# uta-smile/Adaptive-Graph-Convolutional-Network

Hardware: NVIDIA B200
Metric: sgc_ll_train_graphs_per_s (higher is better)
Workload: dtype f32

## Files before the change

adaptive-graph-convolutional-network_b200/_lib.py:

```python
import ctypes
import os

HERE = os.path.dirname(os.path.abspath(__file__))
LIB_PATH = os.path.join(HERE, "libagcn_sm100.so")

AGCN_OK = 0
VARIANT = {"SGC_LL": 0, "SGC_LL_Reslap": 1}
LAPLACIAN = {"reference_literal": 0, "paper": 1}
METRIC_GRAD = {"reference": 0, "full": 1}
ACT = {"linear": 0, "relu": 1}
LOSS = {"sigmoid_ce": 0, "softmax_ce": 1, "weighted_l2": 2}
ADJ_RULE = {"mean_distance": 0, "cutoff": 1}
NODE = {"sgcll": 0, "block_end": 1}
NOTIFY_FN = ctypes.CFUNCTYPE(None, ctypes.c_void_p, ctypes.c_int32, ctypes.c_void_p)
OUT_RES_L, OUT_RES_W, OUT_L_ALL, SAVE_FOR_BACKWARD = 1, 2, 4, 8


class AgcnError(RuntimeError):
    pass


class Desc(ctypes.Structure):
    _fields_ = [("F", ctypes.c_int32), ("Fo", ctypes.c_int32), ("K", ctypes.c_int32), ("variant", ctypes.c_int32),
                ("laplacian_mode", ctypes.c_int32), ("metric_grad", ctypes.c_int32), ("activation", ctypes.c_int32),
                ("flags", ctypes.c_uint32)]


class StackNode(ctypes.Structure):
    _fields_ = [("kind", ctypes.c_int32), ("desc", Desc), ("src", ctypes.c_int32)]


_P = ctypes.c_void_p
_SIGNATURES = {
    "agcn_version": (ctypes.c_int, []),
    "agcn_last_error": (ctypes.c_char_p, []),
    "agcn_launch_count": (ctypes.c_uint64, []),
    "agcn_plan_create": (ctypes.c_int, [_P, ctypes.c_int32, ctypes.c_int32, _P, ctypes.POINTER(_P)]),
    "agcn_plan_destroy": (ctypes.c_int, [_P]),
    "agcn_plan_total_nodes": (ctypes.c_int64, [_P]),
    "agcn_plan_total_lap": (ctypes.c_int64, [_P]),
    "agcn_plan_node_off_host": (_P, [_P]),
    "agcn_plan_lap_off_host": (_P, [_P]),
    "agcn_fused_tiles_host": (ctypes.c_int, [_P, ctypes.c_int32, _P, ctypes.c_int32, _P, ctypes.c_int32, _P, _P]),
    "agcn_fused_debug_set": (ctypes.c_int, [_P]),
    "agcn_fused_profile": (ctypes.c_int, [ctypes.c_int]),
    "agcn_fused_profile_read": (ctypes.c_int, [ctypes.POINTER(ctypes.c_float), ctypes.POINTER(ctypes.c_int)]),
    "agcn_profile_enable": (ctypes.c_int, [ctypes.c_int]),
    "agcn_profile_read": (ctypes.c_int, [ctypes.c_char_p, ctypes.c_size_t, ctypes.POINTER(ctypes.c_size_t)]),
    "agcn_profile_timeline": (ctypes.c_int, [ctypes.c_char_p, ctypes.c_size_t, ctypes.POINTER(ctypes.c_size_t)]),
    "agcn_probe_fp32_fma": (ctypes.c_int, [_P, ctypes.c_int32, _P]),
    "agcn_pack_nodes": (ctypes.c_int, [_P, _P, _P, ctypes.c_int32, _P]),
    "agcn_unpack_nodes": (ctypes.c_int, [_P, _P, _P, ctypes.c_int32, _P]),
    "agcn_pack_lap": (ctypes.c_int, [_P, _P, _P, _P]),
    "agcn_capture_begin": (ctypes.c_int, [_P]),
    "agcn_capture_end_launch": (ctypes.c_int, [_P, ctypes.POINTER(ctypes.c_void_p), ctypes.POINTER(ctypes.c_int32)]),
    "agcn_capture_abort": (ctypes.c_int, [_P]),
    "agcn_step_graph_destroy": (ctypes.c_int, [_P]),
    "agcn_unpack_lap": (ctypes.c_int, [_P, _P, _P, _P]),
    "agcn_debug_grouped_product": (ctypes.c_int, [_P, _P, _P, _P, ctypes.c_int32, ctypes.c_int32, ctypes.c_int32,
                                                  ctypes.c_float, ctypes.c_int32, _P]),
    "agcn_debug_grouped_timeline": (ctypes.c_int, [_P]),
    "agcn_pack_lap_csr": (ctypes.c_int, [_P, _P, _P, _P, _P, _P]),
    "agcn_point_laplacian_workspace_bytes": (ctypes.c_int, [_P, ctypes.POINTER(ctypes.c_size_t)]),
    "agcn_point_laplacian": (ctypes.c_int, [_P, _P, ctypes.c_int32, ctypes.c_int32, ctypes.c_float, _P, _P,
                                            ctypes.c_size_t, _P]),
    "agcn_graph_pool": (ctypes.c_int, [_P, _P, _P, _P, _P, ctypes.c_int32, _P]),
    "agcn_graph_pool_backward": (ctypes.c_int, [_P, _P, _P, _P, ctypes.c_int32, _P]),
    "agcn_sgcll_workspace_bytes": (ctypes.c_int, [ctypes.POINTER(Desc), _P, ctypes.POINTER(ctypes.c_size_t),
                                                  ctypes.POINTER(ctypes.c_size_t)]),
    "agcn_sgcll_forward": (ctypes.c_int, [ctypes.POINTER(Desc), _P] + [_P] * 14 + [ctypes.c_size_t, _P]),
    "agcn_sgcll_backward": (ctypes.c_int, [ctypes.POINTER(Desc), _P] + [_P] * 19 + [ctypes.c_size_t, _P]),
    "agcn_gemm_tn_scratch_bytes": (ctypes.c_size_t, [ctypes.c_int32] * 4),
    "agcn_gemm_tn": (ctypes.c_int, [_P, _P, _P, _P, ctypes.c_int32, ctypes.c_int32, ctypes.c_int32, ctypes.c_int32,
                                    _P, ctypes.c_int32, _P]),
    "agcn_node_gemm_scratch_bytes": (ctypes.c_size_t, [ctypes.c_int32, ctypes.c_int32]),
    "agcn_node_gemm": (ctypes.c_int, [_P, ctypes.c_int32, _P, ctypes.c_int32, ctypes.c_int32, _P, ctypes.c_int32,
                                      ctypes.c_int32, ctypes.c_int32, ctypes.c_int32, _P, _P, ctypes.c_int32,
                                      ctypes.c_int32, _P, _P]),
    "agcn_dropout": (ctypes.c_int, [_P, _P, ctypes.c_int64, ctypes.c_float, ctypes.c_uint64, _P]),
    "agcn_expand_labels": (ctypes.c_int, [_P, _P, ctypes.c_int32, ctypes.c_int32, _P, _P, _P]),
    "agcn_head_workspace_bytes": (ctypes.c_int, [_P, ctypes.c_int32, ctypes.c_int32, ctypes.c_int32,
                                                  ctypes.POINTER(ctypes.c_size_t)]),
    "agcn_head_loss_grad": (ctypes.c_int, [_P] * 8 + [ctypes.c_float, ctypes.c_int32, ctypes.c_int32, ctypes.c_int32] +
                            [_P] * 7 + [ctypes.c_size_t, _P]),
    "agcn_head_loss_grad_ex": (ctypes.c_int, [_P] * 8 + [ctypes.c_float, ctypes.c_int32, ctypes.c_int32, ctypes.c_int32,
                                                     ctypes.c_int32] + [_P] * 7 + [ctypes.c_size_t, _P]),
    "agcn_head_predict_workspace_bytes": (ctypes.c_int, [_P, ctypes.c_int32, ctypes.c_int32, ctypes.c_int32,
                                                          ctypes.POINTER(ctypes.c_size_t)]),
    "agcn_head_predict": (ctypes.c_int, [_P] * 8 + [ctypes.c_float, ctypes.c_int32, ctypes.c_int32, ctypes.c_int32,
                                                ctypes.c_int32] + [_P] * 3 + [ctypes.c_size_t, _P]),
    "agcn_stack_create": (ctypes.c_int, [_P, ctypes.c_int32, ctypes.c_int32, ctypes.c_int32, ctypes.c_int32, _P,
                                         ctypes.POINTER(_P)]),
    "agcn_stack_create_nodes": (ctypes.c_int, [_P, ctypes.c_int32, ctypes.c_int32, ctypes.c_int32, ctypes.c_int32, _P,
                                               ctypes.POINTER(_P)]),
    "agcn_stack_destroy": (ctypes.c_int, [_P]),
    "agcn_stack_workspace_bytes": (ctypes.c_int, [_P, _P, ctypes.POINTER(ctypes.c_size_t)]),
    "agcn_stack_loss_grad": (ctypes.c_int, [_P] * 6 + [ctypes.c_float] + [_P] * 4 + [ctypes.c_size_t, _P, _P, _P]),
    "agcn_stack_predict_workspace_bytes": (ctypes.c_int, [_P, _P, ctypes.POINTER(ctypes.c_size_t)]),
    "agcn_stack_predict": (ctypes.c_int, [_P] * 6 + [ctypes.c_float] + [_P] * 4 + [ctypes.c_size_t, _P]),
    "agcn_adam_step": (ctypes.c_int, [_P] * 5 + [ctypes.c_int64] + [ctypes.c_float] * 4 + [_P]),
    "agcn_sgcll_host_scratch_bytes": (ctypes.c_int, [ctypes.POINTER(Desc), _P, ctypes.POINTER(ctypes.c_size_t)]),
    "agcn_sgcll_forward_host": (ctypes.c_int, [ctypes.POINTER(Desc), _P] + [_P] * 8 + [ctypes.c_size_t, _P]),
}
EXPORTED_SYMBOLS = tuple(_SIGNATURES)

_lib = None


def lib():
    global _lib
    if _lib is None:
        if not os.path.exists(LIB_PATH):
            raise AgcnError("libagcn_sm100.so is missing: run `python %s` (no CPU fallback exists)"
                            % os.path.join(HERE, "build_ext.py"))
        handle = ctypes.CDLL(LIB_PATH)
        for name, (res, args) in _SIGNATURES.items():
            fn = getattr(handle, name)
            fn.restype, fn.argtypes = res, args
        _lib = handle
    return _lib


def check(rc):
    if rc != AGCN_OK:
        raise AgcnError("libagcn_sm100 error %d: %s" % (rc, lib().agcn_last_error().decode()))


def launch_count():
    return int(lib().agcn_launch_count())


def profile_enable(on):
    check(lib().agcn_profile_enable(1 if on else 0))


def profile_timeline():
    buf = ctypes.create_string_buffer(1 << 18)
    check(lib().agcn_profile_timeline(buf, len(buf), None))
    out = []
    for line in buf.value.decode().splitlines():
        name, t0, t1 = line.split("\t")
        out.append((name, float(t0), float(t1)))
    return out


def profile_read():
    buf = ctypes.create_string_buffer(1 << 16)
    check(lib().agcn_profile_read(buf, len(buf), None))
    out = {}
    for line in buf.value.decode().splitlines():
        name, n, ms = line.split("\t")
        out[name] = (int(n), float(ms))
    return out
```

adaptive-graph-convolutional-network_b200/csrc/agcn_capi.cu:

```cuda
#include <algorithm>

#include "agcn_internal.cuh"

using namespace agcn;

namespace {

inline size_t align256(size_t x) { return (x + 255) & ~(size_t)255; }

int node_gemm_tn(const GemmTNArgs& t, cudaStream_t st) {
  if (tc_gemm_tn_supported(t)) return tc_gemm_tn(t, st);
  return gemm_tn(t, st);
}

int node_gemm(const GemmArgs& g, float* tc_scratch, cudaStream_t st, bool presplit = false) {
  if (tc_gemm_supported(g)) {
    if (!presplit) {
      int rc = tc_gemm_split_b(g, tc_scratch, st);
      if (rc) return rc;
    }
    return tc_gemm(g, tc_scratch, st);
  }
  return gemm_rows(g, st);
}
// ... 65 lines not shown
  return s;
}

inline int64_t dl_stride(const agcn_plan* p) { return (p->LL + 63) & ~(int64_t)63; }
inline int dl_parts(const agcn_sgcll_desc* d, const agcn_plan* p) {
  if (d->K < 2) return 1;
  int parts = std::min(8, (d->F + 31) / 32);
  while (parts > 1 && (int64_t)parts * dl_stride(p) * 4 > ((int64_t)1 << 30)) --parts;
  return std::max(1, parts);
}

struct Work {
  float *XW, *dYp, *G, *V, *tn_part, *act_part, *dL, *dXW, *dalpha_part, *dbeta_part, *tcY, *tcM, *big, *ftY;
  size_t bytes;
};

Work carve_work(const agcn_sgcll_desc* d, const agcn_plan* p, void* base) {
  const Modes m = modes_of(d);
  Carver c(base);
  Work w{};
  w.XW = c.take((size_t)p->R * d->F);
  w.dYp = c.take((size_t)p->R * d->Fo);
  w.G = c.take((size_t)d->K * p->R * d->F);
  w.V = c.take((size_t)(d->K > 1 ? d->K - 1 : 0) * p->R * d->Fo);
  size_t tn = gemm_tn_partial_floats((int)p->R, d->F, d->Fo, d->K);
  if (m.full) tn = std::max(tn, gemm_tn_partial_floats((int)p->R, d->F, d->F, 1));
  {
    GemmTNArgs t;
    t.M = (int)p->R; t.Kd = d->F; t.N = d->Fo; t.S = d->K;
    tn = std::max(tn, tc_gemm_tn_partial_floats(t));
    t.N = d->F; t.S = 1;
    tn = std::max(tn, tc_gemm_tn_partial_floats(t));
  }
  w.tn_part = c.take(tn);
  w.act_part = c.take(act_bwd_partial_floats(p->R, d->Fo));
  w.dL = m.need_dL ? c.take((size_t)dl_parts(d, p) * dl_stride(p)) : nullptr;
  w.dXW = m.full ? c.take((size_t)p->R * d->F) : nullptr;
  w.dalpha_part = c.take((size_t)p->B);
  w.dbeta_part = c.take((size_t)p->B);
  w.tcY = c.take(tc_gemm_scratch_floats(d->Fo, d->F, d->K, 1));
  w.tcM = c.take(tc_gemm_scratch_floats(d->F, d->F, 1, 1));
  w.big = c.take(big_work_floats(p, m.full));
  w.ftY = c.take(fused_w_floats(d->Fo, d->F, d->K));
  w.bytes = c.off;
  return w;
}

int check_desc(const agcn_sgcll_desc* d, const agcn_plan* p) {
  AGCN_REQUIRE(d && p, "null desc or plan");
  AGCN_REQUIRE(d->F >= 1 && d->Fo >= 1 && d->K >= 1, "F, Fo, K must be >= 1");
  AGCN_REQUIRE(d->variant == AGCN_VARIANT_SGC_LL || d->variant == AGCN_VARIANT_SGC_LL_RESLAP, "unknown variant");
  AGCN_REQUIRE(d->laplacian_mode == AGCN_LAP_REFERENCE_LITERAL || d->laplacian_mode == AGCN_LAP_PAPER,
               "unknown laplacian_mode");
  AGCN_REQUIRE(d->metric_grad == AGCN_METRIC_GRAD_REFERENCE || d->metric_grad == AGCN_METRIC_GRAD_FULL,
               "unknown metric_grad");
  AGCN_REQUIRE(d->activation == AGCN_ACT_LINEAR || d->activation == AGCN_ACT_RELU, "unknown activation");
  AGCN_REQUIRE(p->R < (1ll << 31) / std::max(d->F, d->Fo), "batch too large for 32-bit row indexing");
  return AGCN_OK;
}

}

namespace {

int padded_features(const agcn_sgcll_desc* d, const agcn_plan* p) {
  const int F = d->F;
  if (F < 33 || F % 32 == 0) return F;
  if (!literal_shortcut(d->variant, d->laplacian_mode)) return F;
  if (d->flags & (AGCN_OUT_RES_L | AGCN_OUT_RES_W | AGCN_OUT_L_ALL)) return F;
  const int Fp = (F + 31) & ~31;
  if (!fused_fwd_supported(p, Fp, d->Fo, d->K)) return F;
  return Fp;
}

struct PadSaved {
  float *Xp, *Wp;
  void* inner;
  size_t bytes;
};
PadSaved carve_pad_saved(const agcn_sgcll_desc* d2, const agcn_plan* p, void* base) {
  Carver c(base);
  PadSaved s{};
  s.Xp = c.take((size_t)p->R * d2->F);
  s.Wp = c.take((size_t)d2->F * d2->K * d2->Fo);
  s.inner = base ? reinterpret_cast<char*>(base) + c.off : nullptr;
  s.bytes = c.off + carve_saved(d2, p, nullptr).bytes + 256;
  return s;
}
struct PadWork {
  float *dXp, *dWp, *dMp;
  void* inner;
  size_t inner_bytes, bytes;
};
PadWork carve_pad_work(const agcn_sgcll_desc* d2, const agcn_plan* p, void* base) {
  Carver c(base);
  PadWork w{};
  w.dXp = c.take((size_t)p->R * d2->F);
  w.dWp = c.take((size_t)d2->F * d2->K * d2->Fo);
  w.dMp = c.take((size_t)d2->F * d2->F);
  w.inner = base ? reinterpret_cast<char*>(base) + c.off : nullptr;
  w.inner_bytes = carve_work(d2, p, nullptr).bytes + 256;
  w.bytes = c.off + w.inner_bytes;
  return w;
}

__global__ void pad_cols_kernel(const float* __restrict__ src, int Fs, float* __restrict__ dst, int Fd, long long rows) {
  const long long total = rows * Fd;
  for (long long e = (long long)blockIdx.x * blockDim.x + threadIdx.x; e < total; e += (long long)gridDim.x * blockDim.x) {
    const long long r = e / Fd;
    const int c = (int)(e - r * Fd);
    dst[e] = c < Fs ? src[r * Fs + c] : 0.f;
  }
}
__global__ void unpad_cols_kernel(const float* __restrict__ src, int Fs, float* __restrict__ dst, int Fd, long long rows) {
  const long long total = rows * Fd;
  for (long long e = (long long)blockIdx.x * blockDim.x + threadIdx.x; e < total; e += (long long)gridDim.x * blockDim.x) {
    const long long r = e / Fd;
    const int c = (int)(e - r * Fd);
    dst[e] = src[r * Fs + c];
  }
}
__global__ void copy_then_zero_kernel(const float* __restrict__ src, float* __restrict__ dst, long long n_copy, long long n_total) {
  for (long long e = (long long)blockIdx.x * blockDim.x + threadIdx.x; e < n_total; e += (long long)gridDim.x * blockDim.x)
    dst[e] = e < n_copy ? src[e] : 0.f;
}
inline unsigned grid_for(long long total) { return (unsigned)std::max<long long>(1, std::min<long long>((total + 255) / 256, 1184)); }

int forward_impl(const agcn_sgcll_desc* desc, const agcn_plan* plan, const float* d_X, const float* d_Lint,
                 const float* d_Lprev, const float* d_M_L, const float* d_weight, const float* d_bias,
                 const float* d_alpha, const float* d_beta, float* d_Y, float* d_resL, float* d_resW, float* d_Lall,
                 void* d_saved, void* d_work, size_t work_bytes, void* stream);
int backward_impl(const agcn_sgcll_desc* desc, const agcn_plan* plan, const float* d_X, const float* d_Lint,
                  const float* d_Lprev, const float* d_M_L, const float* d_weight, const float* d_alpha,
                  const float* d_beta, const float* d_Y, const float* d_dY, const float* d_dLall_in, const void* d_saved,
                  float* d_dX, float* d_dM_L, float* d_dweight, float* d_dbias, float* d_dalpha, float* d_dbeta,
                  float* d_dLprev, void* d_work, size_t work_bytes, void* stream);

}

extern "C" {

int agcn_sgcll_workspace_bytes(const agcn_sgcll_desc* desc, const agcn_plan* plan, size_t* saved_bytes,
                               size_t* work_bytes) {
  AGCN_REQUIRE(desc && plan, "null desc or plan");
  const int Fp = padded_features(desc, plan);
  if (Fp != desc->F) {
    agcn_sgcll_desc d2 = *desc;
    d2.F = Fp;
    if (saved_bytes) *saved_bytes = carve_pad_saved(&d2, plan, nullptr).bytes + 256;
    if (work_bytes) *work_bytes = carve_pad_work(&d2, plan, nullptr).bytes + 256;
    return AGCN_OK;
  }
  if (saved_bytes) *saved_bytes = carve_saved(desc, plan, nullptr).bytes + 256;
  if (work_bytes) *work_bytes = carve_work(desc, plan, nullptr).bytes + 256;
  return AGCN_OK;
}

int agcn_sgcll_forward(const agcn_sgcll_desc* desc, const agcn_plan* plan, const float* d_X, const float* d_Lint,
                       const float* d_Lprev, const float* d_M_L, const float* d_weight, const float* d_bias,
                       const float* d_alpha, const float* d_beta, float* d_Y, float* d_resL, float* d_resW,
                       float* d_Lall, void* d_saved, void* d_work, size_t work_bytes, void* stream) {
  int rc = check_desc(desc, plan);
  if (rc) return rc;
  const int Fp = padded_features(desc, plan);
  if (Fp == desc->F)
    return forward_impl(desc, plan, d_X, d_Lint, d_Lprev, d_M_L, d_weight, d_bias, d_alpha, d_beta, d_Y, d_resL, d_resW,
                        d_Lall, d_saved, d_work, work_bytes, stream);
  AGCN_REQUIRE(d_X && d_weight && d_saved && d_work, "forward: null pointer");
  agcn_sgcll_desc d2 = *desc;
  d2.F = Fp;
  PadSaved ps = carve_pad_saved(&d2, plan, d_saved);
  PadWork pw = carve_pad_work(&d2, plan, d_work);
  if (pw.bytes > work_bytes) {
    set_error("forward: workspace too small");
    return AGCN_ERR_WORKSPACE;
  }
  cudaStream_t st = (cudaStream_t)stream;
  if ((rc = plan_use(plan, st))) return rc;
  pad_cols_kernel<<<grid_for((long long)plan->R * Fp), 256, 0, st>>>(d_X, desc->F, ps.Xp, Fp, plan->R);
  AGCN_LAUNCH_CHECK();
  {
    const long long n_copy = (long long)desc->F * desc->K * desc->Fo, n_total = (long long)Fp * desc->K * desc->Fo;
    copy_then_zero_kernel<<<grid_for(n_total), 256, 0, st>>>(d_weight, ps.Wp, n_copy, n_total);
    AGCN_LAUNCH_CHECK();
  }
  return forward_impl(&d2, plan, ps.Xp, d_Lint, d_Lprev, d_M_L, ps.Wp, d_bias, d_alpha, d_beta, d_Y, d_resL, d_resW, d_Lall,
                      ps.inner, pw.inner, pw.inner_bytes, stream);
}

int agcn_sgcll_backward(const agcn_sgcll_desc* desc, const agcn_plan* plan, const float* d_X, const float* d_Lint,
                        const float* d_Lprev, const float* d_M_L, const float* d_weight, const float* d_alpha,
                        const float* d_beta, const float* d_Y, const float* d_dY, const float* d_dLall_in,
                        const void* d_saved, float* d_dX, float* d_dM_L, float* d_dweight, float* d_dbias,
                        float* d_dalpha, float* d_dbeta, float* d_dLprev, void* d_work, size_t work_bytes,
                        void* stream) {
  int rc = check_desc(desc, plan);
  if (rc) return rc;
  const int Fp = padded_features(desc, plan);
  if (Fp == desc->F)
    return backward_impl(desc, plan, d_X, d_Lint, d_Lprev, d_M_L, d_weight, d_alpha, d_beta, d_Y, d_dY, d_dLall_in, d_saved,
                         d_dX, d_dM_L, d_dweight, d_dbias, d_dalpha, d_dbeta, d_dLprev, d_work, work_bytes, stream);
  AGCN_REQUIRE(d_saved && d_work && d_dM_L && d_dweight, "backward: null pointer");
  agcn_sgcll_desc d2 = *desc;
  d2.F = Fp;
  PadSaved ps = carve_pad_saved(&d2, plan, const_cast<void*>(d_saved));
  PadWork pw = carve_pad_work(&d2, plan, d_work);
  if (pw.bytes > work_bytes) {
    set_error("backward: workspace too small");
    return AGCN_ERR_WORKSPACE;
  }
  cudaStream_t st = (cudaStream_t)stream;
  rc = backward_impl(&d2, plan, ps.Xp, d_Lint, d_Lprev, d_M_L, ps.Wp, d_alpha, d_beta, d_Y, d_dY, d_dLall_in, ps.inner,
                     d_dX ? pw.dXp : nullptr, pw.dMp, pw.dWp, d_dbias, d_dalpha, d_dbeta, d_dLprev, pw.inner, pw.inner_bytes,
                     stream);
  if (rc) return rc;
  {
    const long long n = (long long)desc->F * desc->K * desc->Fo;
    copy_then_zero_kernel<<<grid_for(n), 256, 0, st>>>(pw.dWp, d_dweight, n, n);
    AGCN_LAUNCH_CHECK();
  }
  if ((rc = zero_async(d_dM_L, (size_t)desc->F * desc->F, st))) return rc;
  if (d_dX) {
    unpad_cols_kernel<<<grid_for((long long)plan->R * desc->F), 256, 0, st>>>(pw.dXp, Fp, d_dX, desc->F, plan->R);
    AGCN_LAUNCH_CHECK();
  }
  return AGCN_OK;
}

}

namespace {

int forward_impl(const agcn_sgcll_desc* desc, const agcn_plan* plan, const float* d_X, const float* d_Lint,
                       const float* d_Lprev, const float* d_M_L, const float* d_weight, const float* d_bias,
                       const float* d_alpha, const float* d_beta, float* d_Y, float* d_resL, float* d_resW,
                       float* d_Lall, void* d_saved, void* d_work, size_t work_bytes, void* stream) {
  int rc = check_desc(desc, plan);
  if (rc) return rc;
  AGCN_REQUIRE(d_X && d_Lint && d_M_L && d_weight && d_bias && d_alpha && d_Y && d_saved && d_work,
               "forward: null pointer");
  const Modes m = modes_of(desc);
  AGCN_REQUIRE(!m.reslap || d_beta, "forward: beta required for SGC_LL_Reslap");
  AGCN_REQUIRE(!(desc->flags & AGCN_OUT_RES_L) || d_resL, "forward: d_resL missing");
  AGCN_REQUIRE(!(desc->flags & AGCN_OUT_RES_W) || d_resW, "forward: d_resW missing");
  AGCN_REQUIRE(!(desc->flags & AGCN_OUT_L_ALL) || d_Lall, "forward: d_Lall missing");
  cudaStream_t st = (cudaStream_t)stream;
  if ((rc = plan_use(plan, st))) return rc;
  Saved sv = carve_saved(desc, plan, d_saved);
  Work wk = carve_work(desc, plan, d_work);
  if (wk.bytes > work_bytes) {
    set_error("forward: workspace too small");
    return AGCN_ERR_WORKSPACE;
  }
  const int F = desc->F, Fo = desc->Fo, K = desc->K;
  const int R = (int)plan->R;
  const bool want_resL = desc->flags & AGCN_OUT_RES_L, want_resW = desc->flags & AGCN_OUT_RES_W;
  const bool want_Lall = desc->flags & AGCN_OUT_L_ALL;
  const bool need_W = m.paper || want_resW;
  const bool need_build = !m.shortcut || want_resL || want_resW || want_Lall;
  float* XW = m.full ? sv.XW : wk.XW;

  const bool fuse_f = fused_fwd_supported(plan, F, Fo, K);
  const bool fuse_b = (desc->flags & AGCN_SAVE_FOR_BACKWARD) && !m.need_dL && fused_bwd_supported(plan, F, Fo, K);
  GemmArgs gy = y_gemm_args(desc, R, d_X, sv.T, d_weight, d_bias, d_Y);
  const bool y_tc = !fuse_f && tc_gemm_supported(gy);
  GemmArgs gg = g_gemm_args(desc, R, d_Y , d_weight, wk.G);
  const bool g_tc = !fuse_b && (desc->flags & AGCN_SAVE_FOR_BACKWARD) && tc_gemm_supported(gg);
  if (y_tc || g_tc || fuse_f || fuse_b) {
    AGCN_CUDA(cudaEventRecord(plan->ev_side_fork, st));
    AGCN_CUDA(cudaStreamWaitEvent(plan->side, plan->ev_side_fork, 0));
    if (fuse_f && (rc = fused_fwd_prep(d_weight, F, Fo, K, wk.ftY, plan->side))) return rc;
    if (y_tc && (rc = tc_gemm_split_b(gy, wk.tcY, plan->side))) return rc;
    if (fuse_b && (rc = fused_bwd_prep(d_weight, F, Fo, K, sv.ftG, plan->side))) return rc;
    if (g_tc && (rc = tc_gemm_split_b(gg, sv.tcG, plan->side))) return rc;
    AGCN_CUDA(cudaEventRecord(plan->ev_side_join, plan->side));
  }
  if (need_W) {
    GemmArgs g;
    g.M = R; g.N = F; g.Kd = F;
    g.A0 = d_X; g.lda0 = F;
    g.B = d_M_L; g.ldb = F;
    g.C = XW; g.ldc = F;
    if ((rc = node_gemm(g, wk.tcM, st))) return rc;
  }
  GraphArgs ga;
  ga.plan = plan; ga.F = F; ga.K = K;
  ga.variant = desc->variant; ga.lap_mode = desc->laplacian_mode; ga.metric_full = m.full;
  ga.X = d_X; ga.XW = XW; ga.Lint = d_Lint; ga.Lprev = m.reslap ? d_Lprev : nullptr;
  ga.alpha = d_alpha; ga.beta = d_beta;
  ga.T = sv.T;
  if (need_build) {
    ga.Lall = m.shortcut ? nullptr : sv.Lall;
    ga.Lall_out = want_Lall ? d_Lall : nullptr;
    ga.resL = want_resL ? d_resL : nullptr;
    ga.resW = want_resW ? d_resW : nullptr;
    ga.dist = sv.dist; ga.dis = sv.dis; ga.stats = sv.stats;
    ga.big_work = wk.big;
    if ((rc = graph_build_laplacian(ga, need_W, st))) return rc;
  }
  ga.Lall = m.shortcut ? nullptr : sv.Lall;
  if (fuse_f) {
    const float* Lf = m.shortcut ? d_Lint : sv.Lall;
    const int ident = m.shortcut ? 1 : 0;
    const bool other = cheb_tiles_has_mid(plan) || plan->large_tiles > 0;
    if (other) {
      AGCN_CUDA(cudaEventRecord(plan->ev_big_fork, st));
      AGCN_CUDA(cudaStreamWaitEvent(plan->big, plan->ev_big_fork, 0));
    }
    if ((rc = cheb_tiles_forward(plan, d_X, Lf, ident, F, K, sv.T, st, plan->big))) return rc;
    if (plan->large_tiles > 0 && (rc = graph_chebyshev_fwd(ga, plan->big, AGCN_SMALL_MAX))) return rc;
    if (other) {
      AGCN_CUDA(cudaEventRecord(plan->ev_big_join, plan->big));
      AGCN_CUDA(cudaStreamWaitEvent(st, plan->ev_big_join, 0));
    }
    AGCN_CUDA(cudaStreamWaitEvent(st, plan->ev_side_join, 0));
    return pre_forward(plan, -1, 0, d_X, sv.T, wk.ftY, d_bias, desc->activation, F, Fo, K, d_Y, st);
  }
  if ((rc = graph_chebyshev_fwd(ga, st))) return rc;
  if (y_tc || g_tc || fuse_b) AGCN_CUDA(cudaStreamWaitEvent(st, plan->ev_side_join, 0));
  if ((rc = node_gemm(gy, wk.tcY, st, true))) return rc;
  return AGCN_OK;
}

int backward_impl(const agcn_sgcll_desc* desc, const agcn_plan* plan, const float* d_X, const float* d_Lint,
                  const float* d_Lprev, const float* d_M_L, const float* d_weight, const float* d_alpha,
                  const float* d_beta, const float* d_Y, const float* d_dY, const float* d_dLall_in, const void* d_saved,
                  float* d_dX, float* d_dM_L, float* d_dweight, float* d_dbias, float* d_dalpha, float* d_dbeta,
                  float* d_dLprev, void* d_work, size_t work_bytes, void* stream) {
  int rc = check_desc(desc, plan);
  if (rc) return rc;
  AGCN_REQUIRE(d_X && d_Lint && d_M_L && d_weight && d_alpha && d_Y && d_dY && d_saved && d_work,
               "backward: null input pointer");
  AGCN_REQUIRE(d_dM_L && d_dweight && d_dbias && d_dalpha, "backward: null output pointer");
  const Modes m = modes_of(desc);
  AGCN_REQUIRE(!m.reslap || (d_beta && d_dbeta), "backward: beta / dbeta required for SGC_LL_Reslap");
  cudaStream_t st = (cudaStream_t)stream;
  if ((rc = plan_use(plan, st))) return rc;
  Saved sv = carve_saved(desc, plan, const_cast<void*>(d_saved));
  Work wk = carve_work(desc, plan, d_work);
  if (wk.bytes > work_bytes) {
    set_error("backward: workspace too small");
    return AGCN_ERR_WORKSPACE;
  }
  const int F = desc->F, Fo = desc->Fo, K = desc->K;
  const int R = (int)plan->R;
  const bool has_prev = m.reslap && d_Lprev;

  const bool fuse_b = (desc->flags & AGCN_SAVE_FOR_BACKWARD) && !m.need_dL && d_dX != nullptr &&
                      fused_bwd_supported(plan, F, Fo, K);
  const bool vfirst = fuse_b && plan->large_tiles == 0;
  const bool need_G = !fuse_b && (d_dX != nullptr || (m.need_dL && K >= 2));
  const float* dYp = (desc->activation == AGCN_ACT_RELU) ? wk.dYp : d_dY;
  const bool act_on_side = !vfirst && (fuse_b || (!need_G && !m.need_dL));
  if (!act_on_side && (rc = act_bwd_partials(d_dY, d_Y, wk.dYp, wk.act_part, R, Fo, desc->activation, st))) return rc;
  AGCN_CUDA(cudaEventRecord(plan->ev_side_fork, st));
  AGCN_CUDA(cudaStreamWaitEvent(plan->side, plan->ev_side_fork, 0));
  if (act_on_side && (rc = act_bwd_partials(d_dY, d_Y, wk.dYp, wk.act_part, R, Fo, desc->activation, plan->side)))
    return rc;
  if ((rc = act_bwd_reduce(wk.act_part, d_dbias, R, Fo, plan->side))) return rc;
  float* dXbuf = d_dX ? d_dX : wk.G;
  AGCN_REQUIRE(d_dX || !m.full, "backward: d_dX is required with metric_grad = full");
  if (need_G) {
    GemmArgs g = g_gemm_args(desc, R, dYp, d_weight, (K == 1) ? d_dX : wk.G);
    GemmArgs probe = g_gemm_args(desc, R, d_Y, d_weight, wk.G);
    const bool presplit = (desc->flags & AGCN_SAVE_FOR_BACKWARD) && tc_gemm_supported(probe);
    if ((rc = node_gemm(g, sv.tcG, st, presplit))) return rc;
  }
  GraphArgs ga;
  ga.plan = plan; ga.F = F; ga.K = K;
  ga.variant = desc->variant; ga.lap_mode = desc->laplacian_mode; ga.metric_full = m.full;
  ga.X = d_X; ga.XW = sv.XW; ga.Lint = d_Lint; ga.Lprev = has_prev ? d_Lprev : nullptr;
  ga.alpha = d_alpha; ga.beta = d_beta;
  ga.T = sv.T; ga.Lall = m.shortcut ? nullptr : sv.Lall;
  ga.dist = sv.dist; ga.dis = sv.dis; ga.stats = sv.stats;
  ga.G = wk.G; ga.dLall_in = d_dLall_in; ga.dX = dXbuf; ga.dL = wk.dL;
  ga.dl_parts = (m.need_dL && K >= 2) ? dl_parts(desc, plan) : 1;
  ga.dl_stride = dl_stride(plan);
  ga.dLprev = has_prev ? d_dLprev : nullptr;
  ga.dXW = wk.dXW; ga.dalpha_part = wk.dalpha_part; ga.dbeta_part = m.reslap ? wk.dbeta_part : nullptr;
  ga.big_work = wk.big;
  {
    GemmTNArgs t;
    t.M = R; t.Kd = F; t.N = Fo; t.S = K;
    t.A0 = d_X; t.lda0 = F;
    t.A1 = sv.T; t.lda1 = F; t.sliceA1 = (int64_t)R * F;
    t.D = dYp; t.ldd = Fo;
    t.out = d_dweight; t.partial = wk.tn_part;
    if ((rc = node_gemm_tn(t, plan->side))) return rc;
  }
  AGCN_CUDA(cudaEventRecord(plan->ev_side_join, plan->side));
  if (vfirst) {
    const float* Lf = m.shortcut ? d_Lint : sv.Lall;
    const int ident = m.shortcut ? 1 : 0;
    const bool other = cheb_tiles_has_mid(plan);
    if (other) {
      AGCN_CUDA(cudaEventRecord(plan->ev_big_fork, st));
      AGCN_CUDA(cudaStreamWaitEvent(plan->big, plan->ev_big_fork, 0));
    }
    if ((rc = cheb_tiles_forward(plan, dYp, Lf, ident, Fo, K, wk.V, st, plan->big, 1))) return rc;
    if (other) {
      AGCN_CUDA(cudaEventRecord(plan->ev_big_join, plan->big));
      AGCN_CUDA(cudaStreamWaitEvent(st, plan->ev_big_join, 0));
    }
    if ((rc = pre_forward(plan, -1, 0, dYp, wk.V, sv.ftG, nullptr, AGCN_ACT_LINEAR, Fo, F, K, d_dX, st))) return rc;
  } else if (fuse_b) {
    const float* Lf = m.shortcut ? d_Lint : sv.Lall;
    const int ident = m.shortcut ? 1 : 0;
    if ((rc = pre_backward(plan, -1, 0, d_dY, desc->activation == AGCN_ACT_RELU ? d_Y : nullptr, sv.ftG, F, Fo, K, wk.G, st)))
      return rc;
    const bool other = cheb_tiles_has_mid(plan) || plan->large_tiles > 0;
    if (other) {
      AGCN_CUDA(cudaEventRecord(plan->ev_big_fork, st));
      AGCN_CUDA(cudaStreamWaitEvent(plan->big, plan->ev_big_fork, 0));
    }
    if ((rc = cheb_tiles_backward(plan, wk.G, Lf, ident, F, K, d_dX, st, plan->big))) return rc;
    if (plan->large_tiles > 0 && (rc = graph_recurrence_bwd(ga, false, plan->big, AGCN_SMALL_MAX))) return rc;
    if (other) {
      AGCN_CUDA(cudaEventRecord(plan->ev_big_join, plan->big));
      AGCN_CUDA(cudaStreamWaitEvent(st, plan->ev_big_join, 0));
    }
  } else if (K >= 2) {
    if (need_G && (rc = graph_recurrence_bwd(ga, m.need_dL, st))) return rc;
  } else if (m.need_dL) {
    if (d_dLall_in)
      AGCN_CUDA(cudaMemcpyAsync(wk.dL, d_dLall_in, (size_t)plan->LL * sizeof(float), cudaMemcpyDeviceToDevice, st));
    else
      AGCN_CUDA(cudaMemsetAsync(wk.dL, 0, (size_t)plan->LL * sizeof(float), st));
  }
  AGCN_CUDA(cudaStreamWaitEvent(st, plan->ev_side_join, 0));
  if (m.need_dL) {
    if ((rc = graph_laplacian_bwd(ga, st))) return rc;
    if ((rc = reduce_scalar_parts(wk.dalpha_part, plan->B, d_dalpha, st))) return rc;
    if (m.reslap) {
      if ((rc = reduce_scalar_parts(wk.dbeta_part, plan->B, d_dbeta, st))) return rc;
    }
  } else {
    if ((rc = zero_async(d_dalpha, 1, st))) return rc;
  }
  if (m.full) {
    GemmTNArgs t;
    t.M = R; t.Kd = F; t.N = F; t.S = 1;
    t.A0 = d_X; t.lda0 = F;
    t.D = wk.dXW; t.ldd = F;
    t.out = d_dM_L; t.partial = wk.tn_part;
    if ((rc = node_gemm_tn(t, st))) return rc;
    GemmArgs g;
    g.M = R; g.N = F; g.Kd = F;
    g.A0 = wk.dXW; g.lda0 = F;
    g.B = d_M_L; g.ldb = F; g.transB = 1;
    g.C = d_dX; g.ldc = F; g.accumulate = 1;
    if ((rc = node_gemm(g, wk.tcM, st))) return rc;
  } else {
    if ((rc = zero_async(d_dM_L, (size_t)F * F, st))) return rc;
  }
  return AGCN_OK;
}

}

extern "C" {

size_t agcn_gemm_tn_scratch_bytes(int32_t M, int32_t Kd, int32_t N, int32_t S) {
  GemmTNArgs t;
  t.M = M; t.Kd = Kd; t.N = N; t.S = S;
  return 4 * std::max(gemm_tn_partial_floats(M, Kd, N, S), tc_gemm_tn_partial_floats(t)) + 256;
}

int agcn_gemm_tn(const float* d_A0, const float* d_A1, const float* d_D, float* d_out, int32_t M, int32_t Kd,
                 int32_t N, int32_t S, void* d_scratch, int32_t use_tensor_cores, void* stream) {
  AGCN_REQUIRE(d_A0 && d_D && d_out && d_scratch && M >= 1 && Kd >= 1 && N >= 1 && S >= 1, "gemm_tn: bad arguments");
  GemmTNArgs t;
  t.M = M; t.Kd = Kd; t.N = N; t.S = S;
  t.A0 = d_A0; t.lda0 = Kd;
  t.A1 = d_A1; t.lda1 = Kd; t.sliceA1 = (int64_t)M * Kd;
  t.D = d_D; t.ldd = N;
  t.out = d_out; t.partial = reinterpret_cast<float*>(d_scratch);
  if (use_tensor_cores) {
    if (!tc_gemm_tn_supported(t)) {
      set_error("gemm_tn: shape not supported by the tensor-core kernel");
      return AGCN_ERR_INVALID;
    }
    return tc_gemm_tn(t, (cudaStream_t)stream);
  }
  return gemm_tn(t, (cudaStream_t)stream);
}

size_t agcn_node_gemm_scratch_bytes(int32_t N, int32_t Kd) { return 4 * tc_gemm_scratch_floats(N, Kd, 1, 1) + 256; }

int agcn_node_gemm(const float* d_A, int32_t lda, const float* d_B, int32_t ldb, int32_t transB, float* d_C, int32_t ldc,
                   int32_t M, int32_t N, int32_t Kd, const float* d_bias, const float* d_scale, int32_t accumulate,
                   int32_t activation, void* d_scratch, void* stream) {
  AGCN_REQUIRE(d_A && d_B && d_C && d_scratch && M >= 1 && N >= 1 && Kd >= 1, "node_gemm: bad arguments");
  AGCN_REQUIRE(activation == AGCN_ACT_LINEAR || activation == AGCN_ACT_RELU, "node_gemm: unknown activation");
  GemmArgs g;
  g.M = M; g.N = N; g.Kd = Kd;
  g.A0 = d_A; g.lda0 = lda;
  g.B = d_B; g.ldb = ldb; g.transB = transB;
  g.C = d_C; g.ldc = ldc;
  g.bias = d_bias; g.scale = d_scale; g.accumulate = accumulate; g.act = activation;
  return node_gemm(g, reinterpret_cast<float*>(d_scratch), (cudaStream_t)stream);
}

int agcn_fused_profile(int enable) {
  fused_profile_enable(enable);
  return AGCN_OK;
}
int agcn_fused_profile_read(float* ms_sum, int* launches) { return fused_profile_read(ms_sum, launches); }

int agcn_fused_debug_set(void* d_buf) {
  fused_debug_set(d_buf);
  return AGCN_OK;
}

int agcn_sgcll_host_scratch_bytes(const agcn_sgcll_desc* desc, const agcn_plan* plan, size_t* bytes) {
  AGCN_REQUIRE(desc && plan && bytes, "null pointer");
  size_t saved = 0, work = 0;
  agcn_sgcll_workspace_bytes(desc, plan, &saved, &work);
  const size_t B = plan->B, N = plan->Nmax;
  size_t total = 0;
  total += align256(B * N * desc->F * 4) + align256(B * N * N * 4) + align256(B * N * desc->Fo * 4);
  total += align256((size_t)plan->R * desc->F * 4) + align256((size_t)plan->LL * 4) +
           align256((size_t)plan->R * desc->Fo * 4);
  total += align256(saved) + align256(work);
  *bytes = total;
  return AGCN_OK;
}

int agcn_sgcll_forward_host(const agcn_sgcll_desc* desc, const agcn_plan* plan, const float* h_X_padded,
                            const float* h_L_padded, const float* d_M_L, const float* d_weight, const float* d_bias,
                            const float* d_alpha, float* h_Y_padded, void* d_scratch, size_t scratch_bytes,
                            void* stream) {
  int rc = check_desc(desc, plan);
  if (rc) return rc;
  AGCN_REQUIRE(h_X_padded && h_L_padded && h_Y_padded && d_scratch, "forward_host: null pointer");
  AGCN_REQUIRE(desc->variant == AGCN_VARIANT_SGC_LL, "forward_host: SGC_LL only");
  AGCN_REQUIRE((desc->flags & (AGCN_OUT_RES_L | AGCN_OUT_RES_W | AGCN_OUT_L_ALL)) == 0,
               "forward_host: optional outputs are not supported");
  size_t need = 0, saved = 0, work = 0;
  agcn_sgcll_host_scratch_bytes(desc, plan, &need);
  if (need > scratch_bytes) {
    set_error("forward_host: scratch too small");
    return AGCN_ERR_WORKSPACE;
  }
  agcn_sgcll_workspace_bytes(desc, plan, &saved, &work);
  cudaStream_t st = (cudaStream_t)stream;
  const size_t B = plan->B, N = plan->Nmax;
  char* base = reinterpret_cast<char*>(d_scratch);
  size_t off = 0;
  auto take = [&](size_t bytes) { char* r = base + off; off += align256(bytes); return r; };
  float* dXpad = (float*)take(B * N * desc->F * 4);
  float* dLpad = (float*)take(B * N * N * 4);
  float* dYpad = (float*)take(B * N * desc->Fo * 4);
  float* dX = (float*)take((size_t)plan->R * desc->F * 4);
  float* dL = (float*)take((size_t)plan->LL * 4);
  float* dY = (float*)take((size_t)plan->R * desc->Fo * 4);
  void* dsaved = take(saved);
  void* dwork = take(work);
  auto device_view = [](const float* h) -> const float* {
    cudaPointerAttributes at;
    if (cudaPointerGetAttributes(&at, h) != cudaSuccess) {
      (void)cudaGetLastError();
      return nullptr;
    }
    if ((at.type == cudaMemoryTypeHost || at.type == cudaMemoryTypeManaged) && at.devicePointer)
      return reinterpret_cast<const float*>(at.devicePointer);
    return nullptr;
  };
  const float* xsrc = device_view(h_X_padded);
  const float* lsrc = device_view(h_L_padded);
  if (!xsrc) {
    AGCN_CUDA(cudaMemcpyAsync(dXpad, h_X_padded, B * N * desc->F * 4, cudaMemcpyHostToDevice, st));
    xsrc = dXpad;
  }
  if (!lsrc) {
    AGCN_CUDA(cudaMemcpyAsync(dLpad, h_L_padded, B * N * N * 4, cudaMemcpyHostToDevice, st));
    lsrc = dLpad;
  }
  if ((rc = agcn_pack_nodes(plan, xsrc, dX, desc->F, st))) return rc;
  if ((rc = agcn_pack_lap(plan, lsrc, dL, st))) return rc;
  if ((rc = agcn_sgcll_forward(desc, plan, dX, dL, nullptr, d_M_L, d_weight, d_bias, d_alpha, nullptr, dY, nullptr,
                               nullptr, nullptr, dsaved, dwork, work, st)))
    return rc;
  if ((rc = agcn_unpack_nodes(plan, dY, dYpad, desc->Fo, st))) return rc;
  AGCN_CUDA(cudaMemcpyAsync(h_Y_padded, dYpad, B * N * desc->Fo * 4, cudaMemcpyDeviceToHost, st));
  AGCN_CUDA(cudaStreamSynchronize(st));
  return AGCN_OK;
}

}
```

adaptive-graph-convolutional-network_b200/csrc/agcn_cheb_tile.cu:

```cuda
#include <algorithm>
#include <mutex>

#include "agcn_internal.cuh"

namespace agcn {
namespace ct {

constexpr int CH = 32;
constexpr int CPITCH = 144;

__device__ __forceinline__ uint32_t smem_u32(const void* p) { return (uint32_t)__cvta_generic_to_shared(p); }
__device__ __forceinline__ float4 lds128(uint32_t a) {
  float4 v;
  asm volatile("ld.shared.v4.f32 {%0,%1,%2,%3}, [%4];\n" : "=f"(v.x), "=f"(v.y), "=f"(v.z), "=f"(v.w) : "r"(a) : "memory");
  return v;
}
__device__ __forceinline__ float lds32(uint32_t a) {
  float v;
  asm volatile("ld.shared.f32 %0, [%1];\n" : "=f"(v) : "r"(a) : "memory");
  return v;
}
__device__ __forceinline__ void sts128(uint32_t a, float4 v) {
  asm volatile("st.shared.v4.f32 [%0], {%1,%2,%3,%4};\n" ::"r"(a), "f"(v.x), "f"(v.y), "f"(v.z), "f"(v.w) : "memory");
}
__device__ __forceinline__ void sts32(uint32_t a, float v) {
  asm volatile("st.shared.f32 [%0], %1;\n" ::"r"(a), "f"(v) : "memory");
}
__device__ __forceinline__ void cp_async4(uint32_t sdst, const float* gsrc) {
  asm volatile("cp.async.ca.shared.global [%0], [%1], 4;\n" ::"r"(sdst), "l"(gsrc) : "memory");
}
__device__ __forceinline__ void cp_async16(uint32_t sdst, const float* gsrc) {
  asm volatile("cp.async.cg.shared.global [%0], [%1], 16;\n" ::"r"(sdst), "l"(gsrc) : "memory");
}
__device__ __forceinline__ void cp_async_commit() { asm volatile("cp.async.commit_group;\n" ::: "memory"); }
__device__ __forceinline__ void cp_async_wait_all() { asm volatile("cp.async.wait_group 0;\n" ::: "memory"); }

struct CtArgs {
  const int4* tile_graphs;
  const int32_t* tile_gstart;
  const int32_t* order;
  const int32_t* n_nodes;
  const int32_t* node_off;
  const int64_t* lap_off;
  int order_start;
  int chunks;
  int cpc;
  int groups;
  int rows;
  int lfloats;
  const float* L;
  int add_identity;
  int transL;
  int F, K;
  const float* X;
  float* T;
  long long tslice;
  const float* G;
  long long gslice;
  float* dX;
  unsigned long long* dbg;
};

#define CT_STAMP(slot)                                                                  \
  do {                                                                                  \
    if (p.dbg && threadIdx.x == 0) {                                                    \
      unsigned long long t__;                                                           \
      asm volatile("mov.u64 %0, %%globaltimer;\n" : "=l"(t__));                         \
      p.dbg[(long long)blockIdx.x * 128 + (slot)] = t__;                                \
    }                                                                                   \
  } while (0)

struct Row {
  int grow;
  int n;
  int r0;
  int lbase;
  int i;
  int pitch;
};

__device__ __forceinline__ void copy_matrix(const float* __restrict__ src, uint32_t dst, int n, int pitch) {
  const int warp = threadIdx.x >> 5, lane = threadIdx.x & 31, nw = blockDim.x >> 5;
  for (int i = warp; i < n; i += nw) {
    const float* srow = src + (long long)i * n;
    const uint32_t drow = dst + 4 * (i * pitch);
    for (int j = lane; j < n; j += 32) cp_async4(drow + 4 * j, srow + j);
  }
}

template <bool TILE>
__device__ __forceinline__ Row prologue(const CtArgs& p, int tile, int r, uint32_t s_glist, uint32_t sL) {
  Row t;
  t.grow = -1; t.n = 0; t.r0 = 0; t.lbase = 0; t.i = 0; t.pitch = 1;
  const int tid = threadIdx.x, nthreads = blockDim.x;
  if (TILE) {
    if (tid < 32) {
      int gs = 0, ge = 0;
      if (tid == 0) {
        gs = __ldg(p.tile_gstart + tile);
        ge = __ldg(p.tile_gstart + tile + 1);
      }
      gs = __shfl_sync(0xffffffffu, gs, 0);
      ge = __shfl_sync(0xffffffffu, ge, 0);
      const int ng2 = 2 * (ge - gs);
      for (int e = tid; e < ng2; e += 32) {
        const int4 v = __ldg(p.tile_graphs + 2 * gs + e);
        asm volatile("st.shared.v4.s32 [%0], {%1,%2,%3,%4};\n" ::"r"(s_glist + 16 * e), "r"(v.x), "r"(v.y), "r"(v.z), "r"(v.w) : "memory");
      }
      if (tid == 0) asm volatile("st.shared.s32 [%0], %1;\n" ::"r"(s_glist + 128 * 32), "r"(ge - gs) : "memory");
    }
    __syncthreads();
    int ng;
    asm volatile("ld.shared.s32 %0, [%1];\n" : "=r"(ng) : "r"(s_glist + 128 * 32) : "memory");
    for (int e = 0; e < ng; ++e) {
      int gx, gy, gz, gw, noff, lo, hi, pad;
      asm volatile("ld.shared.v4.s32 {%0,%1,%2,%3}, [%4];\n" : "=r"(gx), "=r"(gy), "=r"(gz), "=r"(gw) : "r"(s_glist + 32 * e) : "memory");
      asm volatile("ld.shared.v4.s32 {%0,%1,%2,%3}, [%4];\n" : "=r"(noff), "=r"(lo), "=r"(hi), "=r"(pad) : "r"(s_glist + 32 * e + 16) : "memory");
      if (r >= gy && r < gy + gz) {
        t.grow = noff + (r - gy);
        t.n = gz; t.r0 = gy; t.lbase = gw; t.i = r - gy; t.pitch = gz | 1;
      }
      const long long loff = (long long)(((unsigned long long)(unsigned)hi << 32) | (unsigned)lo);
      copy_matrix(p.L + loff, sL + 4 * gw, gz, gz | 1);
    }
  } else {
    const int g = p.order[p.order_start + tile];
    const int n = p.n_nodes[g], pitch = n | 1;
    if (r < n) {
      t.grow = p.node_off[g] + r;
      t.n = n; t.i = r; t.pitch = pitch;
    }
    copy_matrix(p.L + p.lap_off[g], sL, n, pitch);
  }
  cp_async_commit();
  return t;
}

template <int MW>
struct Mask {
  uint32_t w[MW];
};

template <int MW>
__device__ __forceinline__ Mask<MW> nonzero_mask(uint32_t laddr, int lstride_bytes, int n) {
  Mask<MW> m;
#pragma unroll
  for (int k = 0; k < MW; ++k) {
    uint32_t bits = 0;
    const int j0 = 32 * k;
    if (j0 < n) {
      const int cnt = min(32, n - j0);
      uint32_t a = laddr + (uint32_t)(j0 * lstride_bytes);
      int j = 0;
      for (; j + 8 <= cnt; j += 8) {
        uint32_t b8 = 0;
#pragma unroll
        for (int u = 0; u < 8; ++u) b8 |= (lds32(a + (uint32_t)(u * lstride_bytes)) != 0.f) ? (1u << u) : 0u;
        bits |= b8 << j;
        a += 8 * lstride_bytes;
      }
      for (; j < cnt; ++j) {
        bits |= (lds32(a) != 0.f) ? (1u << j) : 0u;
        a += lstride_bytes;
      }
    }
    m.w[k] = bits;
  }
  return m;
}
template <int MW>
__device__ __forceinline__ bool prefer_masked(const Mask<MW>& m, int n) {
  int nnz = 0;
#pragma unroll
  for (int k = 0; k < MW; ++k) nnz += __popc(m.w[k]);
  const unsigned dense_cost = __reduce_max_sync(0xffffffffu, (unsigned)(n * 3));
  const unsigned masked_cost = __reduce_max_sync(0xffffffffu, (unsigned)(nnz * 4));
  return masked_cost < dense_cost;
}

__device__ __forceinline__ void fma_row(float a, const float4 b[4], float acc[16]) {
#pragma unroll
  for (int g = 0; g < 4; ++g) {
    acc[4 * g] = fmaf(a, b[g].x, acc[4 * g]);
    acc[4 * g + 1] = fmaf(a, b[g].y, acc[4 * g + 1]);
    acc[4 * g + 2] = fmaf(a, b[g].z, acc[4 * g + 2]);
    acc[4 * g + 3] = fmaf(a, b[g].w, acc[4 * g + 3]);
  }
}
__device__ __forceinline__ void lap_times_rows(uint32_t laddr, int lstride_bytes, uint32_t src, int r0, int n, int h,
                                               float acc[16]) {
  uint32_t ta = src + (uint32_t)(r0 * CPITCH + h * 64);
  uint32_t la = laddr;
  int j = 0;
  for (; j < n; ++j) {
    const float a = lds32(la);
    float4 b[4];
#pragma unroll
    for (int g = 0; g < 4; ++g) b[g] = lds128(ta + 16 * g);
    fma_row(a, b, acc);
    la += lstride_bytes;
    ta += CPITCH;
  }
}
template <int MW>
__device__ __forceinline__ void lap_times_rows_masked(uint32_t laddr, int lstride_bytes, uint32_t src, int r0,
                                                      const Mask<MW>& m, int h, float acc[16]) {
#pragma unroll
  for (int k = 0; k < MW; ++k) {
    uint32_t bits = m.w[k];
    const uint32_t tbase = src + (uint32_t)((r0 + 32 * k) * CPITCH + h * 64);
    const uint32_t lbase = laddr + (uint32_t)(32 * k * lstride_bytes);
    while (bits) {
      const int j = __ffs((int)bits) - 1;
      bits &= bits - 1;
      const float a = lds32(lbase + (uint32_t)(j * lstride_bytes));
      float4 b[4];
#pragma unroll
      for (int g = 0; g < 4; ++g) b[g] = lds128(tbase + (uint32_t)(j * CPITCH + 16 * g));
      fma_row(a, b, acc);
    }
  }
}

__device__ __forceinline__ uint32_t seg_addr(uint32_t buf, int row, int h) { return buf + (uint32_t)(row * CPITCH + h * 64); }
__device__ __forceinline__ void read_seg(uint32_t buf, int row, int h, float v[16]) {
#pragma unroll
  for (int g = 0; g < 4; ++g) {
    const float4 x = lds128(seg_addr(buf, row, h) + 16 * g);
    v[4 * g] = x.x; v[4 * g + 1] = x.y; v[4 * g + 2] = x.z; v[4 * g + 3] = x.w;
  }
}
__device__ __forceinline__ void write_seg(uint32_t buf, int row, int h, const float v[16]) {
#pragma unroll
  for (int g = 0; g < 4; ++g)
    sts128(seg_addr(buf, row, h) + 16 * g, make_float4(v[4 * g], v[4 * g + 1], v[4 * g + 2], v[4 * g + 3]));
}
__device__ __forceinline__ void load_seg(const float* __restrict__ M, int F, int grow, int col0, bool vec, float v[16]) {
  if (grow < 0) {
#pragma unroll
    for (int u = 0; u < 16; ++u) v[u] = 0.f;
    return;
  }
  const float* src = M + (long long)grow * F + col0;
  if (vec) {
#pragma unroll
    for (int g = 0; g < 4; ++g) {
      float4 x = make_float4(0.f, 0.f, 0.f, 0.f);
      if (col0 + 4 * g < F) x = __ldg(reinterpret_cast<const float4*>(src) + g);
      v[4 * g] = x.x; v[4 * g + 1] = x.y; v[4 * g + 2] = x.z; v[4 * g + 3] = x.w;
    }
  } else {
#pragma unroll
    for (int u = 0; u < 16; ++u) v[u] = (col0 + u < F) ? __ldg(src + u) : 0.f;
  }
}
__device__ __forceinline__ void store_seg(float* __restrict__ M, int F, int grow, int col0, bool vec, const float v[16]) {
  if (grow < 0) return;
  float* dst = M + (long long)grow * F + col0;
  if (vec) {
#pragma unroll
    for (int g = 0; g < 4; ++g)
      if (col0 + 4 * g < F)
        reinterpret_cast<float4*>(dst)[g] = make_float4(v[4 * g], v[4 * g + 1], v[4 * g + 2], v[4 * g + 3]);
  } else {
#pragma unroll
    for (int u = 0; u < 16; ++u)
      if (col0 + u < F) dst[u] = v[u];
  }
}

template <bool TILE, int MW>
__global__ void __launch_bounds__(TILE ? 256 : 320, TILE ? 3 : 1) cheb_tile_fwd_kernel(CtArgs p) {
  extern __shared__ __align__(16) uint8_t smem[];
  const uint32_t sbase = smem_u32(smem);
  const int rows = p.rows;
  const uint32_t buf0 = sbase, buf1 = sbase + (uint32_t)(rows * CPITCH), sL = buf1 + (uint32_t)(rows * CPITCH),
                 s_glist = sL + 4u * (uint32_t)p.lfloats;
  const int tile = blockIdx.x / p.groups, grp = blockIdx.x - tile * p.groups;
  const int warp = threadIdx.x >> 5, lane = threadIdx.x & 31, wpr = rows >> 5;
  const int h = warp / wpr, r = (warp - h * wpr) * 32 + lane;
  const int F = p.F, K = p.K;
  CT_STAMP(100);
  const Row me = prologue<TILE>(p, tile, r, s_glist, sL);
  CT_STAMP(101);
  const bool vec = ((F & 3) == 0) && ((reinterpret_cast<uintptr_t>(p.X) & 15) == 0) &&
                   ((reinterpret_cast<uintptr_t>(p.T) & 15) == 0) && ((p.tslice & 3) == 0);
  const uint32_t lrow = p.transL ? sL + 4 * (me.lbase + me.i) : sL + 4 * (me.lbase + me.i * me.pitch);
  const int lstep = p.transL ? 4 * me.pitch : 4;
  Mask<MW> mask;
  bool masked = false;
  const int c_beg = grp * p.cpc, c_end = min(p.chunks, c_beg + p.cpc);
  for (int c = c_beg; c < c_end; ++c) {
    const int col0 = c * CH + 16 * h;
    {
      const uint32_t d = seg_addr(buf0, r, h);
      const float* src = p.X + (long long)(me.grow < 0 ? 0 : me.grow) * F + col0;
      if (vec) {
#pragma unroll
        for (int g = 0; g < 4; ++g) {
          if (me.grow >= 0 && col0 + 4 * g < F)
            cp_async16(d + 16 * g, src + 4 * g);
          else
            sts128(d + 16 * g, make_float4(0.f, 0.f, 0.f, 0.f));
        }
      } else {
#pragma unroll
        for (int u = 0; u < 16; ++u) {
          if (me.grow >= 0 && col0 + u < F)
            cp_async4(d + 4 * u, src + u);
          else
            sts32(d + 4 * u, 0.f);
        }
      }
      cp_async_commit();
    }
    if (c == c_beg) CT_STAMP(102);
    cp_async_wait_all();
    __syncthreads();
    if (c == c_beg) {
      CT_STAMP(103);
      mask = nonzero_mask<MW>(lrow, lstep, me.n);
      masked = prefer_masked<MW>(mask, me.n);
      CT_STAMP(104);
    }
    float tm1[16], tm2[16];
    read_seg(buf0, r, h, tm1);
#pragma unroll
    for (int u = 0; u < 16; ++u) tm2[u] = 0.f;
    uint32_t src = buf0, dst = buf1;
    for (int s = 1; s < K; ++s) {
      float t[16];
#pragma unroll
      for (int u = 0; u < 16; ++u) t[u] = p.add_identity ? tm1[u] : 0.f;
      if (masked)
        lap_times_rows_masked<MW>(lrow, lstep, src, me.r0, mask, h, t);
      else
        lap_times_rows(lrow, lstep, src, me.r0, me.n, h, t);
      if (s >= 2) {
#pragma unroll
        for (int u = 0; u < 16; ++u) t[u] = 2.f * t[u] - tm2[u];
      }
      store_seg(p.T + (long long)(s - 1) * p.tslice, F, me.grow, col0, vec, t);
      if (s + 1 < K) {
        write_seg(dst, r, h, t);
        __syncthreads();
        const uint32_t tmp = src; src = dst; dst = tmp;
      }
#pragma unroll
      for (int u = 0; u < 16; ++u) { tm2[u] = tm1[u]; tm1[u] = t[u]; }
      if (c == c_beg) CT_STAMP(104 + s);
    }
    if (c + 1 < c_end) __syncthreads();
  }
}

template <bool TILE, int MW>
__global__ void __launch_bounds__(TILE ? 256 : 320, TILE ? 3 : 1) cheb_tile_bwd_kernel(CtArgs p) {
  extern __shared__ __align__(16) uint8_t smem[];
  const uint32_t sbase = smem_u32(smem);
  const int rows = p.rows;
  const uint32_t buf0 = sbase, buf1 = sbase + (uint32_t)(rows * CPITCH), sL = buf1 + (uint32_t)(rows * CPITCH),
                 s_glist = sL + 4u * (uint32_t)p.lfloats;
  const int tile = blockIdx.x / p.groups, grp = blockIdx.x - tile * p.groups;
  const int warp = threadIdx.x >> 5, lane = threadIdx.x & 31, wpr = rows >> 5;
  const int h = warp / wpr, r = (warp - h * wpr) * 32 + lane;
  const int F = p.F, K = p.K;
  const Row me = prologue<TILE>(p, tile, r, s_glist, sL);
  const bool vec = ((F & 3) == 0) && ((reinterpret_cast<uintptr_t>(p.G) & 15) == 0) &&
                   ((reinterpret_cast<uintptr_t>(p.dX) & 15) == 0) && ((p.gslice & 3) == 0);
  cp_async_wait_all();
  __syncthreads();
  const uint32_t lcol = sL + 4 * (me.lbase + me.i);
  const Mask<MW> mask = nonzero_mask<MW>(lcol, 4 * me.pitch, me.n);
  const bool masked = prefer_masked<MW>(mask, me.n);
  const uint32_t ub[2] = {buf0, buf1};
  const int c_beg = grp * p.cpc, c_end = min(p.chunks, c_beg + p.cpc);
  for (int c = c_beg; c < c_end; ++c) {
    const int col0 = c * CH + 16 * h;
    float u1[16], u2[16];
    load_seg(p.G + (long long)(K - 1) * p.gslice, F, me.grow, col0, vec, u1);
#pragma unroll
    for (int u = 0; u < 16; ++u) u2[u] = 0.f;
    int cur = 0;
    for (int j = K - 2; j >= 0; --j) {
      write_seg(ub[cur], r, h, u1);
      __syncthreads();
      float acc[16];
#pragma unroll
      for (int u = 0; u < 16; ++u) acc[u] = p.add_identity ? u1[u] : 0.f;
      if (masked)
        lap_times_rows_masked<MW>(lcol, 4 * me.pitch, ub[cur], me.r0, mask, h, acc);
      else
        lap_times_rows(lcol, 4 * me.pitch, ub[cur], me.r0, me.n, h, acc);
      const float cmul = (j + 1 >= 2) ? 2.f : 1.f;
#pragma unroll
      for (int u = 0; u < 16; ++u) acc[u] = cmul * acc[u] - u2[u];
      float g[16];
      load_seg(p.G + (long long)j * p.gslice, F, me.grow, col0, vec, g);
#pragma unroll
      for (int u = 0; u < 16; ++u) {
        const float o = g[u] + acc[u];
        u2[u] = u1[u];
        u1[u] = o;
      }
      cur ^= 1;
    }
    store_seg(p.dX, F, me.grow, col0, vec, u1);
    if (c + 1 < c_end) __syncthreads();
  }
}

static unsigned long long* g_dbg = nullptr;

static size_t smem_bytes(int rows, int lfloats, bool tile) {
  return (size_t)2 * rows * CPITCH + (size_t)lfloats * 4 + (tile ? 128 * 32 + 16 : 0) + 64;
}

template <typename Kern>
static int opt_in(Kern k, size_t bytes) {
  cudaError_t e = cudaFuncSetAttribute(k, cudaFuncAttributeMaxDynamicSharedMemorySize, (int)bytes);
  if (e != cudaSuccess) return cuda_fail(e, "cudaFuncSetAttribute(cheb_tile)", __FILE__, __LINE__);
  return AGCN_OK;
}

static CtArgs base_args(const agcn_plan* plan, const float* L, int add_identity, int F, int K) {
  CtArgs a{};
  a.order = plan->d_order; a.n_nodes = plan->d_n; a.node_off = plan->d_node_off; a.lap_off = plan->d_lap_off;
  a.chunks = (F + CH - 1) / CH;
  a.L = L; a.add_identity = add_identity; a.F = F; a.K = K;
  a.dbg = g_dbg;
  return a;
}

static const Bucket* mid_bucket(const agcn_plan* plan) {
  for (const Bucket& b : plan->buckets)
    if (b.limit > AGCN_FUSE_MAX_N && b.max_n <= plan->cheb_small_max) return &b;
  return nullptr;
}

static int launch(const agcn_plan* plan, CtArgs a, bool forward, cudaStream_t st_small, cudaStream_t st_mid) {
  static std::once_flag once;
  static int once_rc = AGCN_OK;
  const size_t smem_tile = smem_bytes(128, AGCN_FUSE_LCAP, true);
  const int mid_rows = (AGCN_SMALL_MAX + 31) / 32 * 32;
  const size_t smem_mid = smem_bytes(mid_rows, AGCN_SMALL_MAX * (AGCN_SMALL_MAX | 1), false);
  std::call_once(once, [&] {
    int rc;
    if ((rc = opt_in(cheb_tile_fwd_kernel<true, 2>, smem_tile))) once_rc = rc;
    if ((rc = opt_in(cheb_tile_bwd_kernel<true, 2>, smem_tile))) once_rc = rc;
    if ((rc = opt_in(cheb_tile_fwd_kernel<false, 5>, smem_mid))) once_rc = rc;
    if ((rc = opt_in(cheb_tile_bwd_kernel<false, 5>, smem_mid))) once_rc = rc;
  });
  if (once_rc) return once_rc;
  if (const Bucket* b = mid_bucket(plan)) {
    CtArgs t = a;
    t.tile_graphs = nullptr;
    t.order_start = b->start;
    t.rows = mid_rows;
    t.lfloats = AGCN_SMALL_MAX * (AGCN_SMALL_MAX | 1);
    t.cpc = 1;
    t.groups = t.chunks;
    const unsigned grid = (unsigned)(b->count * t.chunks);
    {
      ProfScope prof(forward ? "ct::cheb_tile_fwd_kernel(mid)" : "ct::cheb_tile_bwd_kernel(mid)", st_mid);
      if (forward)
        cheb_tile_fwd_kernel<false, 5><<<grid, 2 * mid_rows, smem_mid, st_mid>>>(t);
      else
        cheb_tile_bwd_kernel<false, 5><<<grid, 2 * mid_rows, smem_mid, st_mid>>>(t);
    }
    AGCN_LAUNCH_CHECK();
  }
  if (plan->ft_small_tiles > 0) {
    CtArgs t = a;
    t.tile_graphs = reinterpret_cast<const int4*>(plan->d_ft_entries);
    t.tile_gstart = plan->d_ft_gstart;
    t.rows = 128;
    t.lfloats = AGCN_FUSE_LCAP;
    int sms = 148, dev = 0;
    if (cudaGetDevice(&dev) == cudaSuccess) cudaDeviceGetAttribute(&sms, cudaDevAttrMultiProcessorCount, dev);
    t.cpc = 1;
    while (t.cpc < t.chunks && plan->ft_small_tiles * ((t.chunks + t.cpc - 1) / t.cpc) > 3 * sms) ++t.cpc;
    t.groups = (t.chunks + t.cpc - 1) / t.cpc;
    const unsigned grid = (unsigned)(plan->ft_small_tiles * t.groups);
    ProfScope prof(forward ? "ct::cheb_tile_fwd_kernel" : "ct::cheb_tile_bwd_kernel", st_small);
    if (forward)
      cheb_tile_fwd_kernel<true, 2><<<grid, 256, smem_tile, st_small>>>(t);
    else
      cheb_tile_bwd_kernel<true, 2><<<grid, 256, smem_tile, st_small>>>(t);
  }
  if (plan->ft_small_tiles > 0) AGCN_LAUNCH_CHECK();
  return AGCN_OK;
}

}

void cheb_debug_set(void* d_buf) { ct::g_dbg = reinterpret_cast<unsigned long long*>(d_buf); }

bool cheb_tiles_has_mid(const agcn_plan* plan) { return ct::mid_bucket(plan) != nullptr; }

int cheb_tiles_forward(const agcn_plan* plan, const float* X, const float* L, int add_identity, int F, int K, float* T,
                       cudaStream_t st_small, cudaStream_t st_mid, int transL) {
  if (K < 2) return AGCN_OK;
  ct::CtArgs a = ct::base_args(plan, L, add_identity, F, K);
  a.transL = transL;
  a.X = X; a.T = T; a.tslice = (long long)plan->R * F;
  return ct::launch(plan, a, true, st_small, st_mid);
}

int cheb_tiles_backward(const agcn_plan* plan, const float* G, const float* L, int add_identity, int F, int K, float* dX,
                        cudaStream_t st_small, cudaStream_t st_mid) {
  if (K < 2) return AGCN_OK;
  ct::CtArgs a = ct::base_args(plan, L, add_identity, F, K);
  a.G = G; a.gslice = (long long)plan->R * F; a.dX = dX;
  return ct::launch(plan, a, false, st_small, st_mid);
}

}
```

adaptive-graph-convolutional-network_b200/csrc/agcn_internal.cuh:

```cuda
#pragma once
#include <cuda_runtime.h>
#include <stdint.h>

#include <atomic>
#include <string>
#include <vector>

#include "agcn_sgcll.h"

#define AGCN_SMALL_MAX 144
#define AGCN_CHEB_SMALL_MAX 144
#define AGCN_FUSE_MAX_N 64
#define AGCN_FUSE_LCAP 8320
#define AGCN_MID_TILED_MIN 32
#define AGCN_DEGREE_FLOOR 8.271806125530277e-25f

namespace agcn {

#ifdef __CUDACC__
__device__ __forceinline__ float tf32_rn(float x) {
  uint32_t r;
  asm("cvt.rna.tf32.f32 %0, %1;\n" : "=r"(r) : "f"(x));
  return __uint_as_float(r);
}

__device__ __forceinline__ void mbar_wait_shared(uint32_t addr, uint32_t parity) {
  uint32_t done = 0, spins = 0;
  unsigned long long t0 = 0;
  while (true) {
    asm volatile(
        "{\n.reg .pred p;\nmbarrier.try_wait.parity.shared::cta.b64 p, [%1], %2;\nselp.u32 %0, 1, 0, p;\n}\n"
        : "=r"(done)
        : "r"(addr), "r"(parity)
        : "memory");
    if (done) break;
    if ((++spins & 0xFFFFu) == 0) {
      unsigned long long t;
      asm volatile("mov.u64 %0, %%globaltimer;\n" : "=l"(t));
      if (t0 == 0) t0 = t;
      else if (t - t0 > 10000000000ull) __trap();
    }
  }
}
#endif

struct Bucket {
  int start;
  int count;
  int max_n;
  int limit;
};

#ifdef AGCN_AB_SWITCHES
#include <cstdlib>
inline const char* ab_env(const char* name) { return getenv(name); }
#else
inline const char* ab_env(const char*) { return nullptr; }
#endif

void set_error(const std::string& msg);
int cuda_fail(cudaError_t e, const char* what, const char* file, int line);
extern std::atomic<uint64_t> g_launches;

#define AGCN_CUDA(call)                                                        \
  do {                                                                         \
    cudaError_t e__ = (call);                                                  \
    if (e__ != cudaSuccess) return agcn::cuda_fail(e__, #call, __FILE__, __LINE__); \
  } while (0)

#define AGCN_LAUNCH_CHECK()                                                    \
  do {                                                                         \
    agcn::g_launches.fetch_add(1, std::memory_order_relaxed);                  \
    cudaError_t e__ = cudaGetLastError();                                      \
    if (e__ != cudaSuccess) return agcn::cuda_fail(e__, "kernel launch", __FILE__, __LINE__); \
  } while (0)

#define AGCN_REQUIRE(cond, msg)                                                \
  do {                                                                         \
    if (!(cond)) {                                                             \
      agcn::set_error(std::string("invalid argument: ") + msg);               \
      return AGCN_ERR_INVALID;                                                 \
    }                                                                          \
  } while (0)

}

struct agcn_plan {
  int32_t B = 0, Nmax = 0, max_n = 0;
  int32_t uniform_n = 0;
  int32_t cheb_small_max = AGCN_CHEB_SMALL_MAX;
  int64_t R = 0;
  int64_t LL = 0;
  std::vector<int32_t> n, node_off, order;
  std::vector<int64_t> lap_off;
  std::vector<agcn::Bucket> buckets;
  int large_count = 0;
  std::vector<int32_t> tile_graph, tile_row;
  int large_tiles = 0;
  int big_tiles = 0;
  std::vector<int32_t> big_tile_start;
  void* d_block = nullptr;
  int32_t* d_n = nullptr;
  int32_t* d_node_off = nullptr;
  int32_t* d_order = nullptr;
  int64_t* d_lap_off = nullptr;
  int32_t* d_tile_graph = nullptr;
  int32_t* d_tile_row = nullptr;
  int32_t* d_big_tile_start = nullptr;
  int ft_tiles = 0;
  int ft_small_tiles = 0;
  std::vector<int32_t> ft_gstart, ft_entries;
  int32_t* d_ft_gstart = nullptr;
  int32_t* d_ft_entries = nullptr;
  cudaStream_t aux[3] = {nullptr, nullptr, nullptr};
  cudaEvent_t ev_fork = nullptr;
  cudaEvent_t ev_join[3] = {nullptr, nullptr, nullptr};
  cudaStream_t side = nullptr;
  cudaEvent_t ev_side_fork = nullptr, ev_side_join = nullptr;
  cudaStream_t big = nullptr;
  cudaEvent_t ev_big_fork = nullptr, ev_big_join = nullptr;
  cudaEvent_t ev_ready = nullptr;
  cudaStream_t create_stream = nullptr, last_stream = nullptr;
  bool ready_done = false;
  int res_device = -1;
  void* staging_host = nullptr;
  size_t staging_bytes = 0;
  cudaEvent_t staging_done = nullptr;
};

namespace agcn {

struct GemmArgs {
  int M = 0, N = 0, Kd = 0;
  int S = 1;
  int Z = 1;
  const float* A0 = nullptr;
  int lda0 = 0;
  const float* A1 = nullptr;
  int lda1 = 0;
  int64_t sliceA1 = 0;
  const float* B = nullptr;
  int ldb = 0;
  int64_t sliceB = 0;
  int transB = 0;
  float* C = nullptr;
  int ldc = 0;
  int64_t sliceC = 0;
  const float* bias = nullptr;
  const float* scale = nullptr;
  int act = AGCN_ACT_LINEAR;
  int accumulate = 0;
  const float* bce_y = nullptr;
  const float* bce_w = nullptr;
  int bce_ld = 0;
  float bce_scale = 1.f;
  float* loss_part = nullptr;
  int prob = 0;
  int l2 = 0;
  float* split_k_partial = nullptr;
};
int tc_gemm_loss_parts(const GemmArgs& a);
int gemm_rows(const GemmArgs& a, cudaStream_t st);
bool tc_gemm_supported(const GemmArgs& a);
size_t tc_gemm_scratch_floats(int N, int Kd, int S, int Z);
int tc_gemm_split_b(const GemmArgs& a, float* scratch, cudaStream_t st);
int tc_gemm(const GemmArgs& a, const float* scratch, cudaStream_t st);

struct GemmTNArgs {
  int M = 0;
  int Kd = 0;
  int N = 0;
  int S = 1;
  const float* A0 = nullptr;
  int lda0 = 0;
  const float* A1 = nullptr;
  int lda1 = 0;
  int64_t sliceA1 = 0;
  const float* D = nullptr;
  int ldd = 0;
  float* out = nullptr;
  float* partial = nullptr;
};
size_t gemm_tn_partial_floats(int M, int Kd, int N, int S);
int gemm_tn(const GemmTNArgs& a, cudaStream_t st);
bool tc_gemm_tn_supported(const GemmTNArgs& a);
size_t tc_gemm_tn_partial_floats(const GemmTNArgs& a);
int tc_gemm_tn(const GemmTNArgs& a, cudaStream_t st);

size_t act_bwd_partial_floats(int64_t R, int Fo);
int act_bwd_partials(const float* dY, const float* Y, float* dYp, float* partial, int64_t R, int Fo, int act,
                     cudaStream_t st);
int act_bwd_reduce(const float* partial, float* dbias, int64_t R, int Fo, cudaStream_t st);

struct GraphArgs {
  const agcn_plan* plan = nullptr;
  int F = 0, K = 0;
  int variant = 0, lap_mode = 0, metric_full = 0;
  const float* X = nullptr;
  const float* XW = nullptr;
  const float* Lint = nullptr;
  const float* Lprev = nullptr;
  const float* alpha = nullptr;
  const float* beta = nullptr;
  float* T = nullptr;
  float* Lall = nullptr;
  float* Lall_out = nullptr;
  float* resL = nullptr;
  float* resW = nullptr;
  float* dist = nullptr;
  float* dis = nullptr;
  float* stats = nullptr;
  const float* G = nullptr;
  const float* dLall_in = nullptr;
  float* dX = nullptr;
  float* dL = nullptr;
  int dl_parts = 1;
  int64_t dl_stride = 0;
  float* dLprev = nullptr;
  float* dXW = nullptr;
  float* dalpha_part = nullptr;
  float* dbeta_part = nullptr;
  float* big_work = nullptr;
};
bool literal_shortcut(int variant, int lap_mode);
int graph_build_laplacian(const GraphArgs& a, bool need_W, cudaStream_t st);
int graph_chebyshev_fwd(const GraphArgs& a, cudaStream_t st, int above_n = 0);
int graph_recurrence_bwd(const GraphArgs& a, bool need_dL, cudaStream_t st, int above_n = 0);
int graph_laplacian_bwd(const GraphArgs& a, cudaStream_t st);
int reduce_scalar_parts(const float* parts, int B, float* out, cudaStream_t st);
int large_chebyshev_fwd(const GraphArgs& a, cudaStream_t st);
int large_recurrence_bwd(const GraphArgs& a, float* G, bool big_only, cudaStream_t st);
size_t big_work_floats(const agcn_plan* plan, bool full);
int big_build_laplacian(const GraphArgs& a, bool need_W, float* big_work, cudaStream_t st);
int big_dL(const GraphArgs& a, const float* U, cudaStream_t st);
int big_laplacian_bwd(const GraphArgs& a, float* big_work, cudaStream_t st);

struct GroupedArgs {
  const int32_t* n_nodes;
  const int32_t* node_off;
  const int64_t* lap_off;
  const int32_t* tile_graph;
  const int32_t* tile_row;
  const float* L;
  int add_identity, transL;
  const float* In;
  const float* Sub;
  const float* Add;
  float* Out;
  float* Out2;
  float cmul;
  int F;
  const float* RowScale;
  const float* ScaleIn;
  unsigned long long* dbg;
  int force_uniform;
};
int grouped_launch(const agcn_plan* plan, int tiles, const GroupedArgs& g, cudaStream_t st);
int grouped_simt(int tiles, const GroupedArgs& g, cudaStream_t st);
bool grouped_tc_supported(const GroupedArgs& g);
int grouped_tc(const agcn_plan* plan, int tiles, const GroupedArgs& g, cudaStream_t st);
bool pair_tc_supported(const agcn_plan* plan, int F);
int pair_tc_similarity(const agcn_plan* plan, const float* XW, int F, float* norms, float* dist, float* resW, float* rowpart,
                       int ncb, cudaStream_t st);
int pair_tc_dL(const agcn_plan* plan, const float* U, const float* X, const float* T, int F, int K, const float* dL_in,
               float* dL, cudaStream_t st);
bool grouped_thin_supported(const GroupedArgs& g);
int grouped_thin(int tiles, const GroupedArgs& g, cudaStream_t st);

void fused_profile_enable(int on);
int fused_profile_read(float* ms_sum, int* launches);
void prof_enable(int on);
void fused_debug_set(void* d_buf);
bool fused_fwd_supported(const agcn_plan* plan, int F, int Fo, int K);
bool fused_bwd_supported(const agcn_plan* plan, int F, int Fo, int K);
size_t fused_w_floats(int Nv, int Kv, int Z);
int fused_fwd_prep(const float* weight, int F, int Fo, int K, float* scratch, cudaStream_t st);
int fused_bwd_prep(const float* weight, int F, int Fo, int K, float* scratch, cudaStream_t st);

int pre_forward(const agcn_plan* plan, int tile0, int ntiles, const float* X, const float* T, const float* wsplit,
                const float* bias, int act, int F, int Fo, int K, float* Y, cudaStream_t st);
int pre_backward(const agcn_plan* plan, int tile0, int ntiles, const float* dY, const float* Y, const float* wsplit, int F,
                 int Fo, int K, float* G, cudaStream_t st);

bool cheb_tiles_has_mid(const agcn_plan* plan);
int cheb_tiles_forward(const agcn_plan* plan, const float* X, const float* L, int add_identity, int F, int K, float* T,
                       cudaStream_t st_small, cudaStream_t st_mid, int transL = 0);
int cheb_tiles_backward(const agcn_plan* plan, const float* G, const float* L, int add_identity, int F, int K, float* dX,
                        cudaStream_t st_small, cudaStream_t st_mid);

class ProfScope {
 public:
  ProfScope(const char* name, cudaStream_t st);
  ~ProfScope();
  ProfScope(const ProfScope&) = delete;
  ProfScope& operator=(const ProfScope&) = delete;

 private:
  const char* name_;
  cudaStream_t st_;
  cudaEvent_t e0_;
};

int zero_async(float* dst, size_t floats, cudaStream_t st);
int plan_use(const agcn_plan* plan, cudaStream_t st);
int fork_streams(const agcn_plan* plan, cudaStream_t main, int n_aux);
int join_streams(const agcn_plan* plan, cudaStream_t main, int n_aux);

}
```

adaptive-graph-convolutional-network_b200/csrc/agcn_plan.cu:

```cuda
#include <algorithm>
#include <cstdlib>
#include <cstring>
#include <mutex>
#include <numeric>

#include "agcn_internal.cuh"

namespace agcn {

static thread_local std::string t_error;
std::atomic<uint64_t> g_launches{0};

void set_error(const std::string& msg) { t_error = msg; }

int cuda_fail(cudaError_t e, const char* what, const char* file, int line) {
  t_error = std::string(what) + " failed: " + cudaGetErrorString(e) + " (" + file + ":" + std::to_string(line) + ")";
  return (e == cudaErrorNoDevice || e == cudaErrorNoKernelImageForDevice || e == cudaErrorInsufficientDriver)
             ? AGCN_ERR_NO_DEVICE
             : AGCN_ERR_CUDA;
}

int fork_streams(const agcn_plan* plan, cudaStream_t main, int n_aux) {
  if (n_aux <= 0) return AGCN_OK;
  AGCN_CUDA(cudaEventRecord(plan->ev_fork, main));
// ... 125 lines not shown
      const int nl = len ? (int)((s0 - a0 + len + 31) >> 5) : 0;
      for (int l = 0; __any_sync(0xffffffffu, l < nl); l += PACK_U) {
        float4 v[PACK_U];
#pragma unroll
        for (int u = 0; u < PACK_U; ++u) v[u] = load_line(a0, l + u, l + u < nl);
#pragma unroll
        for (int u = 0; u < PACK_U; ++u) store_line(a0, l + u, s0, len, d0, v[u], l + u < nl);
      }
    }
  }
}

__global__ void __launch_bounds__(1024) pack_rows_kernel(const float* __restrict__ padded, float* __restrict__ packed,
                                                        const int32_t* __restrict__ n_nodes,
                                                        const int32_t* __restrict__ node_off,
                                                        const int64_t* __restrict__ lap_off, int B, int Nmax, int F,
                                                        int R, int lap) {
  const int lane = threadIdx.x & 31;
  const int warps = (gridDim.x * blockDim.x) >> 5;
  for (int r = (blockIdx.x * blockDim.x + threadIdx.x) >> 5; r < R; r += warps) {
    const int g = graph_of_row(node_off, B, r);
    const int i = r - node_off[g];
    const float* __restrict__ src;
    float* __restrict__ dst;
    int len;
    if (lap) {
      const int n = n_nodes[g];
      src = padded + ((int64_t)g * Nmax + i) * Nmax;
      dst = packed + lap_off[g] + (int64_t)i * n;
      len = n;
    } else {
      src = padded + ((int64_t)g * Nmax + i) * F;
      dst = packed + (int64_t)r * F;
      len = F;
    }
    for (int c = lane; c < len; c += 32) dst[c] = __ldg(src + c);
  }
}

constexpr int PACK_CTAS = 2, PACK_THREADS = 1024;
static void pack_shape(int64_t warp_items, unsigned* ctas, unsigned* threads) {
  static const int c = ab_env("AGCN_PACK_CTAS") ? atoi(ab_env("AGCN_PACK_CTAS")) : PACK_CTAS;
  static const int t = ab_env("AGCN_PACK_THREADS") ? atoi(ab_env("AGCN_PACK_THREADS")) : PACK_THREADS;
  *threads = (unsigned)t;
  *ctas = (unsigned)std::max<int64_t>(1, std::min<int64_t>((std::max<int64_t>(1, warp_items) * 32 + t - 1) / t, c));
}

static void launch_pack(const agcn_plan* plan, const float* padded, float* packed, int F, int lap, cudaStream_t st) {
  unsigned ctas, threads;
  if ((reinterpret_cast<uintptr_t>(padded) & 15) != 0) {
    pack_shape(plan->R, &ctas, &threads);
    pack_rows_kernel<<<ctas, threads, 0, st>>>(padded, packed, plan->d_n, plan->d_node_off, plan->d_lap_off, plan->B,
                                              plan->Nmax, F, (int)plan->R, lap);
  } else if (lap) {
    pack_shape((plan->R + 3) / 4, &ctas, &threads);
    pack_lines_kernel<true><<<ctas, threads, 0, st>>>(padded, packed, plan->d_n, plan->d_node_off, plan->d_lap_off, plan->B,
                                                     plan->Nmax, F, (int)plan->R,
                                                     (int64_t)plan->B * plan->Nmax * plan->Nmax);
  } else {
    pack_shape(plan->B, &ctas, &threads);
    pack_lines_kernel<false><<<ctas, threads, 0, st>>>(padded, packed, plan->d_n, plan->d_node_off, plan->d_lap_off, plan->B,
                                                      plan->Nmax, F, (int)plan->R, (int64_t)plan->B * plan->Nmax * F);
  }
}

static void build_fused_tiles(const std::vector<int32_t>& n, const std::vector<int32_t>& order,
                              std::vector<int32_t>* gstart, std::vector<int32_t>* entries, int* n_small_tiles) {
  const int B = (int)n.size();
  gstart->clear();
  entries->clear();
  auto push = [&](int g, int a, int b, int c) {
    entries->push_back(g); entries->push_back(a); entries->push_back(b); entries->push_back(c);
  };
  int i = 0;
  while (i < B && n[order[i]] > AGCN_FUSE_MAX_N) ++i;
  const int n_big = i;
  struct Open { int rows, lused; std::vector<int32_t> e; };
  std::vector<Open> open;
  size_t first_open = 0;
  const int min_n = n[order[B - 1]];
  for (; i < B; ++i) {
    const int g = order[i], ng = n[g], need = ng * (ng | 1);
    size_t t = first_open;
    for (; t < open.size(); ++t)
      if (open[t].rows + ng <= 128 && open[t].lused + need <= AGCN_FUSE_LCAP) break;
    if (t == open.size()) open.push_back(Open{0, 0, {}});
    Open& o = open[t];
    o.e.push_back(g); o.e.push_back(o.rows); o.e.push_back(ng); o.e.push_back(o.lused);
    o.rows += ng;
    o.lused += need;
    while (first_open < open.size() && open[first_open].rows + min_n > 128) ++first_open;
  }
  for (const Open& o : open) {
    gstart->push_back((int32_t)(entries->size() / 4));
    entries->insert(entries->end(), o.e.begin(), o.e.end());
  }
  if (n_small_tiles) *n_small_tiles = (int)gstart->size();
  for (int b = 0; b < n_big; ++b) {
    const int g = order[b];
    for (int r = 0; r < n[g]; r += 128) {
      gstart->push_back((int32_t)(entries->size() / 4));
      push(g, r, std::min(128, n[g] - r), -1);
    }
  }
  gstart->push_back((int32_t)(entries->size() / 4));
}


__global__ void upload_tables_kernel(const int4* __restrict__ src, int4* __restrict__ dst, size_t n16) {
  for (size_t i = (size_t)blockIdx.x * blockDim.x + threadIdx.x; i < n16; i += (size_t)gridDim.x * blockDim.x)
    dst[i] = src[i];
}

__global__ void zero_fill_kernel(float* __restrict__ dst, size_t n) {
  for (size_t i = (size_t)blockIdx.x * blockDim.x + threadIdx.x; i < n; i += (size_t)gridDim.x * blockDim.x) dst[i] = 0.f;
}
int zero_async(float* dst, size_t floats, cudaStream_t st) {
  if (floats == 0) return AGCN_OK;
  zero_fill_kernel<<<(unsigned)std::min<size_t>((floats + 255) / 256, 592), 256, 0, st>>>(dst, floats);
  AGCN_LAUNCH_CHECK();
  return AGCN_OK;
}

struct PlanRes {
  cudaStream_t aux[3] = {nullptr, nullptr, nullptr}, side = nullptr, big = nullptr;
  cudaEvent_t ev_fork = nullptr, ev_join[3] = {nullptr, nullptr, nullptr}, ev_side_fork = nullptr, ev_side_join = nullptr,
              ev_big_fork = nullptr, ev_big_join = nullptr, ev_ready = nullptr;
  int device = -1;
};
struct Staging {
  void* host = nullptr;
  size_t bytes = 0;
  cudaEvent_t done = nullptr;
  int device = -1;
};
static std::mutex g_pool_mu;
static std::vector<PlanRes> g_res_pool;
static std::vector<Staging> g_staging_pool;

static cudaError_t acquire_res(PlanRes* out) {
  int dev = 0;
  cudaError_t e = cudaGetDevice(&dev);
  if (e != cudaSuccess) return e;
  {
    std::lock_guard<std::mutex> lock(g_pool_mu);
    for (size_t i = 0; i < g_res_pool.size(); ++i)
      if (g_res_pool[i].device == dev) {
        *out = g_res_pool[i];
        g_res_pool.erase(g_res_pool.begin() + i);
        return cudaSuccess;
      }
  }
  PlanRes r;
  r.device = dev;
  for (int i = 0; i < 3 && e == cudaSuccess; ++i) {
    e = cudaStreamCreateWithFlags(&r.aux[i], cudaStreamNonBlocking);
    if (e == cudaSuccess) e = cudaEventCreateWithFlags(&r.ev_join[i], cudaEventDisableTiming);
  }
  if (e == cudaSuccess) e = cudaEventCreateWithFlags(&r.ev_fork, cudaEventDisableTiming);
  if (e == cudaSuccess) e = cudaStreamCreateWithFlags(&r.side, cudaStreamNonBlocking);
  if (e == cudaSuccess) e = cudaEventCreateWithFlags(&r.ev_side_fork, cudaEventDisableTiming);
  if (e == cudaSuccess) e = cudaEventCreateWithFlags(&r.ev_side_join, cudaEventDisableTiming);
  if (e == cudaSuccess) {
    int lo = 0, hi = 0;
    if (cudaDeviceGetStreamPriorityRange(&lo, &hi) != cudaSuccess) { lo = hi = 0; (void)cudaGetLastError(); }
    e = cudaStreamCreateWithPriority(&r.big, cudaStreamNonBlocking, hi);
  }
  if (e == cudaSuccess) e = cudaEventCreateWithFlags(&r.ev_big_fork, cudaEventDisableTiming);
  if (e == cudaSuccess) e = cudaEventCreateWithFlags(&r.ev_big_join, cudaEventDisableTiming);
  if (e == cudaSuccess) e = cudaEventCreateWithFlags(&r.ev_ready, cudaEventDisableTiming);
  *out = r;
  return e;
}

static void release_res(const PlanRes& r) {
  std::lock_guard<std::mutex> lock(g_pool_mu);
  g_res_pool.push_back(r);
}

static cudaError_t acquire_staging(size_t bytes, Staging* out) {
  int dev = 0;
  cudaError_t e = cudaGetDevice(&dev);
  if (e != cudaSuccess) return e;
  {
    std::lock_guard<std::mutex> lock(g_pool_mu);
    for (size_t i = 0; i < g_staging_pool.size(); ++i) {
      Staging& s = g_staging_pool[i];
      if (s.device != dev || s.bytes < bytes) continue;
      const cudaError_t q = cudaEventQuery(s.done);
      if (q == cudaSuccess) {
        *out = s;
        g_staging_pool.erase(g_staging_pool.begin() + i);
        return cudaSuccess;
      }
      (void)cudaGetLastError();
    }
  }
  Staging s;
  s.device = dev;
  s.bytes = std::max<size_t>((bytes + 65535) & ~(size_t)65535, (size_t)1 << 18);
  e = cudaMallocHost(&s.host, s.bytes);
  if (e == cudaSuccess) e = cudaEventCreateWithFlags(&s.done, cudaEventDisableTiming);
  *out = s;
  return e;
}

static void release_staging(const Staging& s) {
  if (!s.host) return;
  std::lock_guard<std::mutex> lock(g_pool_mu);
  g_staging_pool.push_back(s);
}

int plan_use(const agcn_plan* plan, cudaStream_t st) {
  agcn_plan* p = const_cast<agcn_plan*>(plan);
  if (!p->ready_done && st != p->create_stream) {
    cudaStreamCaptureStatus cs = cudaStreamCaptureStatusNone;
    AGCN_CUDA(cudaStreamIsCapturing(st, &cs));
    if (cs == cudaStreamCaptureStatusNone) {
      const cudaError_t q = cudaEventQuery(p->ev_ready);
      if (q == cudaSuccess) {
        p->ready_done = true;
      } else {
        (void)cudaGetLastError();
        AGCN_CUDA(cudaStreamWaitEvent(st, p->ev_ready, 0));
      }
    }
  }
  p->last_stream = st;
  return AGCN_OK;
}

}

using namespace agcn;

extern "C" {

int agcn_version(void) { return 100; }
const char* agcn_last_error(void) { return t_error.c_str(); }
uint64_t agcn_launch_count(void) { return g_launches.load(); }

int agcn_plan_create(const int32_t* n_nodes_host, int32_t B, int32_t Nmax, void* stream, agcn_plan** out) {
  AGCN_REQUIRE(n_nodes_host && out, "null pointer");
  AGCN_REQUIRE(B >= 1 && Nmax >= 1, "B and Nmax must be positive");
  agcn_plan* p = new agcn_plan();
  p->B = B;
  p->Nmax = Nmax;
  p->n.assign(n_nodes_host, n_nodes_host + B);
  p->node_off.resize(B + 1);
  p->lap_off.resize(B + 1);
  p->node_off[0] = 0;
  p->lap_off[0] = 0;
  for (int g = 0; g < B; ++g) {
    const int n = p->n[g];
    if (n < 1 || n > Nmax) {
      delete p;
      set_error("invalid argument: n_nodes[g] must be in [1, Nmax]");
      return AGCN_ERR_INVALID;
    }
    p->node_off[g + 1] = p->node_off[g] + n;
    p->lap_off[g + 1] = p->lap_off[g] + (int64_t)n * n;
    p->max_n = std::max(p->max_n, n);
  }
  p->R = p->node_off[B];
  p->LL = p->lap_off[B];
  p->uniform_n = p->max_n;
  for (int g = 0; g < B; ++g)
    if (p->n[g] != p->max_n) p->uniform_n = 0;
  p->order.resize(B);
  std::iota(p->order.begin(), p->order.end(), 0);
  std::stable_sort(p->order.begin(), p->order.end(), [&](int a, int b) { return p->n[a] > p->n[b]; });
  int pos = 0;
  while (pos < B && p->n[p->order[pos]] > AGCN_SMALL_MAX) ++pos;
  p->large_count = pos;
  {
    int mid = 0;
    for (int i = pos; i < B && p->n[p->order[i]] > AGCN_FUSE_MAX_N; ++i) ++mid;
    if (mid >= AGCN_MID_TILED_MIN) p->cheb_small_max = AGCN_FUSE_MAX_N;
  }
  if (const char* e = ab_env("AGCN_CHEB_SMALL_MAX")) p->cheb_small_max = std::min(AGCN_SMALL_MAX, std::max(16, atoi(e)));
  for (int i = 0; i < B && p->n[p->order[i]] > p->cheb_small_max; ++i) {
    const int g = p->order[i];
    if (i <= p->large_count) p->big_tile_start.push_back((int32_t)p->tile_graph.size());
    if (i == p->large_count) p->big_tiles = (int)p->tile_graph.size();
    for (int r = 0; r < p->n[g]; r += 64) {
      p->tile_graph.push_back(g);
      p->tile_row.push_back(r);
    }
  }
  p->large_tiles = (int)p->tile_graph.size();
  if ((int)p->big_tile_start.size() <= p->large_count) {
    p->big_tile_start.push_back(p->large_tiles);
    p->big_tiles = p->large_tiles;
  }
  static const int limits[] = {AGCN_SMALL_MAX, AGCN_FUSE_MAX_N, 32, 16};
  for (int b = 0; b < 4 && pos < B; ++b) {
    const int lo = (b + 1 < 4) ? limits[b + 1] : 0;
    const int start = pos;
    while (pos < B && p->n[p->order[pos]] > lo) ++pos;
    if (pos > start) p->buckets.push_back(Bucket{start, pos - start, p->n[p->order[start]], limits[b]});
  }
  build_fused_tiles(p->n, p->order, &p->ft_gstart, &p->ft_entries, &p->ft_small_tiles);
  p->ft_tiles = (int)p->ft_gstart.size() - 1;
  const size_t T = (size_t)p->large_tiles;
  const size_t NB = p->big_tile_start.size();
  const size_t n32 = (size_t)B + (B + 1) + B + 2 * T + NB + p->ft_gstart.size();
  const size_t off64 = (n32 * 4 + 15) / 16 * 16;
  const size_t off_ft = (off64 + (size_t)(B + 1) * 8 + 15) / 16 * 16;
  const size_t bytes = off_ft + p->ft_entries.size() * 8;
  cudaStream_t st = (cudaStream_t)stream;
  PlanRes res;
  Staging stg;
  cudaError_t e = acquire_res(&res);
  if (e == cudaSuccess) e = acquire_staging(bytes, &stg);
  if (e != cudaSuccess) {
    int rc = cuda_fail(e, "agcn_plan_create (resources)", __FILE__, __LINE__);
    delete p;
    return rc;
  }
  char* host = reinterpret_cast<char*>(stg.host);
  std::memset(host, 0, bytes);
  int32_t* h32 = reinterpret_cast<int32_t*>(host);
  std::memcpy(h32, p->n.data(), (size_t)B * 4);
  std::memcpy(h32 + B, p->node_off.data(), (size_t)(B + 1) * 4);
  std::memcpy(h32 + 2 * B + 1, p->order.data(), (size_t)B * 4);
  if (T) {
    std::memcpy(h32 + 3 * B + 1, p->tile_graph.data(), T * 4);
    std::memcpy(h32 + 3 * B + 1 + T, p->tile_row.data(), T * 4);
  }
  std::memcpy(h32 + 3 * B + 1 + 2 * T, p->big_tile_start.data(), NB * 4);
  std::memcpy(h32 + 3 * B + 1 + 2 * T + NB, p->ft_gstart.data(), p->ft_gstart.size() * 4);
  std::memcpy(host + off64, p->lap_off.data(), (size_t)(B + 1) * 8);
  {
    int32_t* de = reinterpret_cast<int32_t*>(host + off_ft);
    for (size_t en = 0; en < p->ft_entries.size() / 4; ++en) {
      const int32_t* src = &p->ft_entries[4 * en];
      const int64_t lo = p->lap_off[src[0]];
      de[8 * en + 0] = src[0]; de[8 * en + 1] = src[1]; de[8 * en + 2] = src[2]; de[8 * en + 3] = src[3];
      de[8 * en + 4] = p->node_off[src[0]];
      de[8 * en + 5] = (int32_t)(uint32_t)(lo & 0xffffffffll);
      de[8 * en + 6] = (int32_t)(uint32_t)((uint64_t)lo >> 32);
      de[8 * en + 7] = 0;
    }
  }
  for (int i = 0; i < 3; ++i) { p->aux[i] = res.aux[i]; p->ev_join[i] = res.ev_join[i]; }
  p->ev_fork = res.ev_fork; p->side = res.side; p->ev_side_fork = res.ev_side_fork; p->ev_side_join = res.ev_side_join;
  p->big = res.big; p->ev_big_fork = res.ev_big_fork; p->ev_big_join = res.ev_big_join; p->ev_ready = res.ev_ready;
  p->res_device = res.device;
  p->staging_host = stg.host; p->staging_bytes = stg.bytes; p->staging_done = stg.done;
  p->create_stream = st;
  p->last_stream = st;
  const size_t n16 = (bytes + 15) / 16;
  e = cudaMallocAsync(&p->d_block, n16 * 16, st);
  if (e == cudaSuccess) {
    upload_tables_kernel<<<(unsigned)std::min<size_t>((n16 + 255) / 256, 64), 256, 0, st>>>(
        reinterpret_cast<const int4*>(host), reinterpret_cast<int4*>(p->d_block), n16);
    g_launches.fetch_add(1, std::memory_order_relaxed);
    e = cudaGetLastError();
  }
  if (e == cudaSuccess) e = cudaEventRecord(stg.done, st);
  if (e == cudaSuccess) e = cudaEventRecord(p->ev_ready, st);
  if (e != cudaSuccess) {
    int rc = cuda_fail(e, "agcn_plan_create", __FILE__, __LINE__);
    agcn_plan_destroy(p);
    return rc;
  }
  int32_t* d32 = reinterpret_cast<int32_t*>(p->d_block);
  p->d_n = d32;
  p->d_node_off = d32 + B;
  p->d_order = d32 + 2 * B + 1;
  p->d_tile_graph = d32 + 3 * B + 1;
  p->d_tile_row = d32 + 3 * B + 1 + T;
  p->d_big_tile_start = d32 + 3 * B + 1 + 2 * T;
  p->d_ft_gstart = d32 + 3 * B + 1 + 2 * T + NB;
  p->d_lap_off = reinterpret_cast<int64_t*>(reinterpret_cast<char*>(p->d_block) + off64);
  p->d_ft_entries = reinterpret_cast<int32_t*>(reinterpret_cast<char*>(p->d_block) + off_ft);
  *out = p;
  return AGCN_OK;
}

int agcn_fused_tiles_host(const int32_t* n_nodes_host, int32_t B, int32_t* gstart_out, int32_t gstart_cap,
                          int32_t* entries_out, int32_t entries_cap, int32_t* tiles_out, int32_t* n_entries_out) {
  AGCN_REQUIRE(n_nodes_host && B >= 1 && tiles_out && n_entries_out, "fused_tiles_host: bad arguments");
  std::vector<int32_t> n(n_nodes_host, n_nodes_host + B), order(B), gs, en;
  for (int g = 0; g < B; ++g) AGCN_REQUIRE(n[g] >= 1, "n_nodes[g] must be >= 1");
  std::iota(order.begin(), order.end(), 0);
  std::stable_sort(order.begin(), order.end(), [&](int a, int b) { return n[a] > n[b]; });
  build_fused_tiles(n, order, &gs, &en, nullptr);
  *tiles_out = (int32_t)gs.size() - 1;
  *n_entries_out = (int32_t)(en.size() / 4);
  if (gstart_out && entries_out) {
    AGCN_REQUIRE(gstart_cap >= (int32_t)gs.size() && entries_cap >= (int32_t)en.size(), "fused_tiles_host: buffers too small");
    std::memcpy(gstart_out, gs.data(), gs.size() * 4);
    std::memcpy(entries_out, en.data(), en.size() * 4);
  }
  return AGCN_OK;
}

int agcn_plan_destroy(agcn_plan* p) {
  if (!p) return AGCN_OK;
  if (p->d_block) cudaFreeAsync(p->d_block, p->last_stream);
  if (p->ev_ready) {
    PlanRes r;
    for (int i = 0; i < 3; ++i) { r.aux[i] = p->aux[i]; r.ev_join[i] = p->ev_join[i]; }
    r.ev_fork = p->ev_fork; r.side = p->side; r.ev_side_fork = p->ev_side_fork; r.ev_side_join = p->ev_side_join;
    r.big = p->big; r.ev_big_fork = p->ev_big_fork; r.ev_big_join = p->ev_big_join; r.ev_ready = p->ev_ready;
    r.device = p->res_device;
    release_res(r);
  }
  if (p->staging_host) {
    Staging sg;
    sg.host = p->staging_host; sg.bytes = p->staging_bytes; sg.done = p->staging_done; sg.device = p->res_device;
    release_staging(sg);
  }
  delete p;
  return AGCN_OK;
}

int64_t agcn_plan_total_nodes(const agcn_plan* p) { return p ? p->R : -1; }
int64_t agcn_plan_total_lap(const agcn_plan* p) { return p ? p->LL : -1; }
const int32_t* agcn_plan_node_off_host(const agcn_plan* p) { return p ? p->node_off.data() : nullptr; }
const int64_t* agcn_plan_lap_off_host(const agcn_plan* p) { return p ? p->lap_off.data() : nullptr; }

static int pack_nodes_impl(const agcn_plan* plan, const float* padded, float* packed, int32_t F, void* stream,
                           int to_padded) {
  AGCN_REQUIRE(plan && padded && packed && F >= 1, "null pointer or F < 1");
  if (int rc = plan_use(plan, (cudaStream_t)stream)) return rc;
  if (!to_padded) {
    launch_pack(plan, padded, packed, F, 0, (cudaStream_t)stream);
    AGCN_LAUNCH_CHECK();
    return AGCN_OK;
  }
  const int64_t rows = (int64_t)plan->B * plan->Nmax;
  const int wpb = 8;
  pack_nodes_kernel<<<(unsigned)((rows + wpb - 1) / wpb), wpb * 32, 0, (cudaStream_t)stream>>>(
      padded, packed, plan->d_n, plan->d_node_off, plan->B, plan->Nmax, F, to_padded);
  AGCN_LAUNCH_CHECK();
  return AGCN_OK;
}

int agcn_pack_nodes(const agcn_plan* plan, const float* d_padded, float* d_packed, int32_t F, void* stream) {
  return pack_nodes_impl(plan, d_padded, d_packed, F, stream, 0);
}
int agcn_unpack_nodes(const agcn_plan* plan, const float* d_packed, float* d_padded, int32_t F, void* stream) {
  return pack_nodes_impl(plan, d_padded, const_cast<float*>(d_packed), F, stream, 1);
}

static int pack_lap_impl(const agcn_plan* plan, const float* padded, float* packed, void* stream, int to_padded) {
  AGCN_REQUIRE(plan && padded && packed, "null pointer");
  if (int rc = plan_use(plan, (cudaStream_t)stream)) return rc;
  if (!to_padded) {
    launch_pack(plan, padded, packed, 0, 1, (cudaStream_t)stream);
    AGCN_LAUNCH_CHECK();
    return AGCN_OK;
  }
  const int64_t rows = (int64_t)plan->B * plan->Nmax;
  const int wpb = 8;
  pack_lap_kernel<<<(unsigned)((rows + wpb - 1) / wpb), wpb * 32, 0, (cudaStream_t)stream>>>(
      padded, packed, plan->d_n, plan->d_lap_off, plan->B, plan->Nmax, to_padded);
  AGCN_LAUNCH_CHECK();
  return AGCN_OK;
}

int agcn_pack_lap(const agcn_plan* plan, const float* d_padded, float* d_packed, void* stream) {
  return pack_lap_impl(plan, d_padded, d_packed, stream, 0);
}
int agcn_unpack_lap(const agcn_plan* plan, const float* d_packed, float* d_padded, void* stream) {
  return pack_lap_impl(plan, d_padded, const_cast<float*>(d_packed), stream, 1);
}

}
```

adaptive-graph-convolutional-network_b200/csrc/agcn_pre_tile.cu:

```cuda
#include <cuda.h>

#include <algorithm>
#include <mutex>

#include "agcn_internal.cuh"

namespace agcn {
namespace pt {

constexpr int TM = 128;
constexpr int CH = 32;
constexpr int UMMA_K = 8;
constexpr int A_BYTES = TM * CH * 4;
constexpr int WORKERS = 256;
constexpr int THREADS = 64 + WORKERS;
constexpr int SLOTS = 3;

__device__ __forceinline__ uint32_t smem_u32(const void* p) { return (uint32_t)__cvta_generic_to_shared(p); }
__device__ __forceinline__ void mbar_init(uint64_t* bar, uint32_t count) {
  asm volatile("mbarrier.init.shared::cta.b64 [%0], %1;\n" ::"r"(smem_u32(bar)), "r"(count) : "memory");
}
__device__ __forceinline__ void mbar_expect_tx(uint64_t* bar, uint32_t bytes) {
  asm volatile("mbarrier.arrive.expect_tx.shared::cta.b64 _, [%0], %1;\n" ::"r"(smem_u32(bar)), "r"(bytes) : "memory");
}
__device__ __forceinline__ void mbar_arrive(uint64_t* bar) {
  asm volatile("mbarrier.arrive.shared::cta.b64 _, [%0];\n" ::"r"(smem_u32(bar)) : "memory");
}
__device__ __forceinline__ void mbar_wait(uint64_t* bar, uint32_t parity) { mbar_wait_shared(smem_u32(bar), parity); }
__device__ __forceinline__ void tma_load_2d(uint32_t dst, const CUtensorMap* map, uint64_t* bar, int c0, int c1) {
  asm volatile(
      "cp.async.bulk.tensor.2d.shared::cluster.global.mbarrier::complete_tx::bytes [%0], [%1, {%3, %4}], [%2];\n" ::"r"(dst),
      "l"(reinterpret_cast<uint64_t>(map)), "r"(smem_u32(bar)), "r"(c0), "r"(c1)
      : "memory");
}
__device__ __forceinline__ void tc_fence_before() { asm volatile("tcgen05.fence::before_thread_sync;\n" ::: "memory"); }
__device__ __forceinline__ void tc_fence_after() { asm volatile("tcgen05.fence::after_thread_sync;\n" ::: "memory"); }

__device__ __forceinline__ uint64_t make_desc(uint32_t saddr) {
  uint64_t d = 0;
  d |= (uint64_t)((saddr & 0x3FFFF) >> 4);
  d |= (uint64_t)1 << 16;
  d |= (uint64_t)(1024 >> 4) << 32;
  d |= (uint64_t)1 << 46;
  d |= (uint64_t)2 << 61;
  return d;
}
__device__ __forceinline__ void umma_ss(uint32_t tmem_d, uint64_t adesc, uint64_t bdesc, uint32_t idesc, uint32_t acc) {
  asm volatile(
      "{\n.reg .pred p;\nsetp.ne.b32 p, %4, 0;\ntcgen05.mma.cta_group::1.kind::tf32 [%0], %1, %2, %3, p;\n}\n" ::"r"(tmem_d),
      "l"(adesc), "l"(bdesc), "r"(idesc), "r"(acc)
      : "memory");
}
__device__ __forceinline__ void umma_commit(uint64_t* bar) {
  asm volatile("tcgen05.commit.cta_group::1.mbarrier::arrive::one.shared::cluster.b64 [%0];\n" ::"r"(smem_u32(bar))
               : "memory");
}
__device__ __forceinline__ void tmem_ld16(uint32_t taddr, float v[16]) {
  uint32_t u[16];
  asm volatile(
      "tcgen05.ld.sync.aligned.32x32b.x16.b32 {%0,%1,%2,%3,%4,%5,%6,%7,%8,%9,%10,%11,%12,%13,%14,%15}, [%16];\n"
      : "=r"(u[0]), "=r"(u[1]), "=r"(u[2]), "=r"(u[3]), "=r"(u[4]), "=r"(u[5]), "=r"(u[6]), "=r"(u[7]), "=r"(u[8]),
        "=r"(u[9]), "=r"(u[10]), "=r"(u[11]), "=r"(u[12]), "=r"(u[13]), "=r"(u[14]), "=r"(u[15])
      : "r"(taddr));
  asm volatile("tcgen05.wait::ld.sync.aligned;\n" ::: "memory");
#pragma unroll
  for (int i = 0; i < 16; ++i) v[i] = __uint_as_float(u[i]);
}
__device__ __forceinline__ void sts128(uint32_t a, float4 v) {
  asm volatile("st.shared.v4.f32 [%0], {%1,%2,%3,%4};\n" ::"r"(a), "f"(v.x), "f"(v.y), "f"(v.z), "f"(v.w) : "memory");
}
__device__ __forceinline__ int ldsi32(uint32_t a) {
  int v;
  asm volatile("ld.shared.s32 %0, [%1];\n" : "=r"(v) : "r"(a) : "memory");
  return v;
}
__device__ __forceinline__ void worker_sync() { asm volatile("bar.sync 1, 256;\n" ::: "memory"); }

__device__ __forceinline__ void write_rows_operand(uint32_t a_hi, uint32_t a_lo, int row, int h, const float v[16]) {
#pragma unroll
  for (int g = 0; g < 4; ++g) {
    float4 hi, lo;
    hi.x = tf32_rn(v[4 * g]);     hi.y = tf32_rn(v[4 * g + 1]);
    hi.z = tf32_rn(v[4 * g + 2]); hi.w = tf32_rn(v[4 * g + 3]);
    lo.x = tf32_rn(v[4 * g] - hi.x);     lo.y = tf32_rn(v[4 * g + 1] - hi.y);
    lo.z = tf32_rn(v[4 * g + 2] - hi.z); lo.w = tf32_rn(v[4 * g + 3] - hi.w);
    const uint32_t off = (uint32_t)(row * 128 + (((4 * h + g) ^ (row & 7)) << 4));
    sts128(a_hi + off, hi);
    sts128(a_lo + off, lo);
  }
}

struct SmemPlan {
  int w_bytes;
  int slot_bytes;
  int off_bars;
  int total;
};
__host__ __device__ inline SmemPlan smem_plan(int N) {
  SmemPlan s;
  s.w_bytes = N * 128;
  s.slot_bytes = 2 * A_BYTES + 2 * s.w_bytes;
  s.off_bars = SLOTS * s.slot_bytes;
  s.total = s.off_bars + 256 + 1024;
  return s;
}

struct PreArgs {
  const int4* tile_graphs;
  const int32_t* tile_gstart;
  int tile0;
  int R;
  int Fin;
  int Fout;
  int K;
  int N;
  int nchunks;
  int tmem_cols;
  int acc_stride;
  const float* In;
  const float* Mask;
  const float* T;
  long long t_slice;
  const float* bias;
  int act;
  float* Out;
  long long out_slice;
  int forward;
};

__global__ void __launch_bounds__(THREADS, 1)
pre_tile_kernel(const __grid_constant__ CUtensorMap tmBhi, const __grid_constant__ CUtensorMap tmBlo, PreArgs p) {
  extern __shared__ uint8_t smem_raw[];
  uint8_t* base = reinterpret_cast<uint8_t*>((reinterpret_cast<uintptr_t>(smem_raw) + 1023) & ~(uintptr_t)1023);
  const uint32_t sbase = smem_u32(base);
  const SmemPlan sp = smem_plan(p.N);
  uint64_t* bars = reinterpret_cast<uint64_t*>(base + sp.off_bars);
  uint64_t* full_bar = bars;
  uint64_t* ops_bar = bars + SLOTS;
  uint64_t* done_bar = bars + 2 * SLOTS;
  uint64_t* out_bar = bars + 3 * SLOTS;
  uint64_t* outfree_bar = bars + 3 * SLOTS + 1;
  uint32_t* tmem_slot = reinterpret_cast<uint32_t*>(bars + 3 * SLOTS + 2);

  const int warp = threadIdx.x >> 5, lane = threadIdx.x & 31;
  const int tile = p.tile0 + blockIdx.x;
  const int K = p.K, N = p.N, nc = p.nchunks, Fin = p.Fin, Fout = p.Fout;
  const int passes = p.forward ? 1 : K;
  const int per_pass = p.forward ? nc * K : nc;

  if (threadIdx.x == 0) {
    for (int s = 0; s < SLOTS; ++s) {
      mbar_init(&full_bar[s], 1);
      mbar_init(&ops_bar[s], WORKERS / 32);
      mbar_init(&done_bar[s], 1);
    }
    mbar_init(out_bar, 1);
    mbar_init(outfree_bar, WORKERS / 32);
    asm volatile("fence.mbarrier_init.release.cluster;\n" ::: "memory");
  }
  if (warp == 1) {
    const uint32_t s = smem_u32(tmem_slot);
    switch (p.tmem_cols) {
      case 32: asm volatile("tcgen05.alloc.cta_group::1.sync.aligned.shared::cta.b32 [%0], 32;\n" ::"r"(s) : "memory"); break;
      case 64: asm volatile("tcgen05.alloc.cta_group::1.sync.aligned.shared::cta.b32 [%0], 64;\n" ::"r"(s) : "memory"); break;
      case 128: asm volatile("tcgen05.alloc.cta_group::1.sync.aligned.shared::cta.b32 [%0], 128;\n" ::"r"(s) : "memory"); break;
      default: asm volatile("tcgen05.alloc.cta_group::1.sync.aligned.shared::cta.b32 [%0], 256;\n" ::"r"(s) : "memory"); break;
    }
    asm volatile("tcgen05.relinquish_alloc_permit.cta_group::1.sync.aligned;\n" ::: "memory");
  }
  tc_fence_before();
  __syncthreads();
  tc_fence_after();
  const uint32_t tmem_base = *tmem_slot;

  if (warp == 0) {
    if (lane == 0) {
      int t_all = 0;
      for (int z = 0; z < passes; ++z)
        for (int t = 0; t < per_pass; ++t, ++t_all) {
          const int slot = t_all % SLOTS, u = t_all / SLOTS;
          if (u > 0) mbar_wait(&done_bar[slot], (uint32_t)((u - 1) & 1));
          const int cc = p.forward ? t / K : t, sl = p.forward ? t % K : z;
          const uint32_t dst = sbase + slot * sp.slot_bytes + 2 * A_BYTES;
          mbar_expect_tx(&full_bar[slot], 2 * sp.w_bytes);
          tma_load_2d(dst, &tmBhi, &full_bar[slot], cc * CH, sl * N);
          tma_load_2d(dst + sp.w_bytes, &tmBlo, &full_bar[slot], cc * CH, sl * N);
        }
    }
  } else if (warp == 1) {
    if (lane == 0) {
      const uint32_t idesc = (1u << 4) | (2u << 7) | (2u << 10) | ((uint32_t)(N >> 3) << 17) | ((uint32_t)(TM >> 4) << 24);
      int t_all = 0;
      for (int z = 0; z < passes; ++z) {
        if (z > 1) {
          mbar_wait(outfree_bar, (uint32_t)((z - 2) & 1));
          tc_fence_after();
        }
        const uint32_t acc = tmem_base + (uint32_t)((z & 1) * p.acc_stride);
        for (int t = 0; t < per_pass; ++t, ++t_all) {
          const int slot = t_all % SLOTS, u = t_all / SLOTS;
          mbar_wait(&full_bar[slot], (uint32_t)(u & 1));
          mbar_wait(&ops_bar[slot], (uint32_t)(u & 1));
          tc_fence_after();
          const uint32_t sa = sbase + slot * sp.slot_bytes, sa_lo = sa + A_BYTES;
          const uint32_t sw = sa + 2 * A_BYTES, sw_lo = sw + sp.w_bytes;
#pragma unroll
          for (int k = 0; k < CH / UMMA_K; ++k) {
            const uint32_t koff = k * UMMA_K * 4;
            const uint64_t a_hi = make_desc(sa + koff), a_lo = make_desc(sa_lo + koff);
            const uint64_t b_hi = make_desc(sw + koff), b_lo = make_desc(sw_lo + koff);
            umma_ss(acc, a_lo, b_hi, idesc, (t | k) != 0);
            umma_ss(acc, a_hi, b_lo, idesc, 1);
            umma_ss(acc, a_hi, b_hi, idesc, 1);
          }
          umma_commit(&done_bar[slot]);
        }
        umma_commit(out_bar);
      }
    }
  } else {
    const int q = warp & 3;
    const int h = (warp - 2) >> 2;
    const int r = q * 32 + lane;
    int grow = -1;
    if (p.tile_graphs) {
      const int4 e0 = __ldg(p.tile_graphs + 2 * p.tile_gstart[tile]);
      const int4 e1 = __ldg(p.tile_graphs + 2 * p.tile_gstart[tile] + 1);
      if (r < e0.z) grow = e1.x + e0.y + r;
    } else if (tile * TM + r < p.R) {
      grow = tile * TM + r;
    }
    const bool vecIn = ((Fin & 3) == 0) && ((reinterpret_cast<uintptr_t>(p.In) & 15) == 0) &&
                       (!p.Mask || (reinterpret_cast<uintptr_t>(p.Mask) & 15) == 0) &&
                       (!p.T || (((reinterpret_cast<uintptr_t>(p.T) & 15) == 0) && ((p.t_slice & 3) == 0)));
    auto load_item = [&](int cc, int sl, float v[16], float m[16]) {
      const int c0 = cc * CH + 16 * h;
      const float* src = (p.forward && sl > 0) ? p.T + (long long)(sl - 1) * p.t_slice : p.In;
      const float* msk = p.forward ? nullptr : p.Mask;
#pragma unroll
      for (int g = 0; g < 4; ++g) {
        const int col = c0 + 4 * g;
        float4 x = make_float4(0.f, 0.f, 0.f, 0.f), y = make_float4(1.f, 1.f, 1.f, 1.f);
        if (grow >= 0 && col < Fin) {
          const long long o = (long long)grow * Fin + col;
          if (vecIn) {
            x = __ldg(reinterpret_cast<const float4*>(src + o));
            if (msk) y = __ldg(reinterpret_cast<const float4*>(msk + o));
          } else {
            float t[4] = {0.f, 0.f, 0.f, 0.f}, ty[4] = {1.f, 1.f, 1.f, 1.f};
#pragma unroll
            for (int e = 0; e < 4; ++e)
              if (col + e < Fin) {
                t[e] = __ldg(src + o + e);
                if (msk) ty[e] = __ldg(msk + o + e);
              }
            x = make_float4(t[0], t[1], t[2], t[3]);
            y = make_float4(ty[0], ty[1], ty[2], ty[3]);
          }
        }
        v[4 * g] = x.x; v[4 * g + 1] = x.y; v[4 * g + 2] = x.z; v[4 * g + 3] = x.w;
        m[4 * g] = y.x; m[4 * g + 1] = y.y; m[4 * g + 2] = y.z; m[4 * g + 3] = y.w;
      }
    };
    auto coords = [&](int z, int t, int& cc, int& sl) {
      cc = p.forward ? t / K : t;
      sl = p.forward ? t % K : z;
    };
    auto drain_out = [&](float* dstm, uint32_t acc_col) {
      const bool vecO = ((Fout & 3) == 0) && ((reinterpret_cast<uintptr_t>(dstm) & 15) == 0);
      for (int c0 = 16 * h; c0 < N && c0 < Fout; c0 += 32) {
        float v[16];
        tmem_ld16(tmem_base + ((uint32_t)(q * 32) << 16) + acc_col + (uint32_t)c0, v);
        if (grow < 0) continue;
        if (p.forward) {
#pragma unroll
          for (int u = 0; u < 16; ++u) {
            float o = v[u] + ((p.bias && c0 + u < Fout) ? __ldg(p.bias + c0 + u) : 0.f);
            if (p.act == AGCN_ACT_RELU) o = fmaxf(o, 0.f);
            v[u] = o;
          }
        }
        float* dst = dstm + (long long)grow * Fout + c0;
#pragma unroll
        for (int g = 0; g < 4; ++g) {
          if (c0 + 4 * g >= Fout) continue;
          if (vecO && c0 + 4 * g + 3 < Fout) {
            *reinterpret_cast<float4*>(dst + 4 * g) = make_float4(v[4 * g], v[4 * g + 1], v[4 * g + 2], v[4 * g + 3]);
          } else {
#pragma unroll
            for (int e = 0; e < 4; ++e)
              if (c0 + 4 * g + e < Fout) dst[4 * g + e] = v[4 * g + e];
          }
        }
      }
    };

    const int total = passes * per_pass;
    auto fetch = [&](int idx, float (&buf)[16], float (&mk)[16]) {
      if (idx >= total) return;
      const int z = idx / per_pass, t = idx - z * per_pass;
      int cc, sl;
      coords(z, t, cc, sl);
      load_item(cc, sl, buf, mk);
    };
    auto process = [&](int idx, float (&buf)[16], float (&mk)[16]) {
      if (idx >= total) return;
      float v[16];
#pragma unroll
      for (int e = 0; e < 16; ++e) v[e] = (mk[e] > 0.f) ? buf[e] : 0.f;
      fetch(idx + 2, buf, mk);
      const int slot = idx % SLOTS, u = idx / SLOTS;
      if (u > 0) {
        if (lane == 0) mbar_wait(&done_bar[slot], (uint32_t)((u - 1) & 1));
        __syncwarp();
      }
      const uint32_t st = sbase + slot * sp.slot_bytes;
      write_rows_operand(st, st + A_BYTES, r, h, v);
      asm volatile("fence.proxy.async.shared::cta;\n" ::: "memory");
      __syncwarp();
      if (lane == 0) mbar_arrive(&ops_bar[slot]);
      const int z = idx / per_pass;
      if (idx - z * per_pass == per_pass - 1) {
        for (int zd = (z > 0 ? z - 1 : z); zd <= z; ++zd) {
          if (zd == z && z != passes - 1) break;
          if (lane == 0) mbar_wait(out_bar, (uint32_t)(zd & 1));
          __syncwarp();
          tc_fence_after();
          drain_out(p.forward ? p.Out : p.Out + (long long)zd * p.out_slice, (uint32_t)((zd & 1) * p.acc_stride));
          tc_fence_before();
          __syncwarp();
          if (lane == 0 && zd + 2 < passes) mbar_arrive(outfree_bar);
        }
      }
    };
    float b0[16], m0[16], b1[16], m1[16];
    fetch(0, b0, m0);
    fetch(1, b1, m1);
    for (int idx = 0; idx < total; idx += 2) {
      process(idx, b0, m0);
      process(idx + 1, b1, m1);
    }
  }
  tc_fence_before();
  __syncthreads();
  if (warp == 1) {
    switch (p.tmem_cols) {
      case 32: asm volatile("tcgen05.dealloc.cta_group::1.sync.aligned.b32 %0, 32;\n" ::"r"(tmem_base) : "memory"); break;
      case 64: asm volatile("tcgen05.dealloc.cta_group::1.sync.aligned.b32 %0, 64;\n" ::"r"(tmem_base) : "memory"); break;
      case 128: asm volatile("tcgen05.dealloc.cta_group::1.sync.aligned.b32 %0, 128;\n" ::"r"(tmem_base) : "memory"); break;
      default: asm volatile("tcgen05.dealloc.cta_group::1.sync.aligned.b32 %0, 256;\n" ::"r"(tmem_base) : "memory"); break;
    }
  }
}

constexpr int RG_THREADS = 96 + WORKERS;

struct RowsArgs {
  int R, Fin, Fout, K, N, nchunks;
  int NS, NA, NB;
  int acc_stride, tmem_cols;
  int full_tiles;
  int a_col0;
  int has_mask;
  const float* bias;
  int act;
  float* Out;
  long long out_slice;
  unsigned long long* dbg;
};

#define RG_STAMP(slot)                                                                  \
  do {                                                                                  \
    if (p.dbg) {                                                                        \
      unsigned long long t__;                                                           \
      asm volatile("mov.u64 %0, %%globaltimer;\n" : "=l"(t__));                         \
      p.dbg[(long long)blockIdx.x * 128 + (slot)] = t__;                                \
    }                                                                                   \
  } while (0)

__device__ __forceinline__ void umma_ts(uint32_t tmem_d, uint32_t tmem_a, uint64_t bdesc, uint32_t idesc, uint32_t acc) {
  asm volatile(
      "{\n.reg .pred p;\nsetp.ne.b32 p, %4, 0;\ntcgen05.mma.cta_group::1.kind::tf32 [%0], [%1], %2, %3, p;\n}\n" ::"r"(tmem_d),
      "r"(tmem_a), "l"(bdesc), "r"(idesc), "r"(acc)
      : "memory");
}
__device__ __forceinline__ void tmem_st16(uint32_t taddr, const float v[16]) {
  asm volatile(
      "tcgen05.st.sync.aligned.32x32b.x16.b32 [%0], {%1,%2,%3,%4,%5,%6,%7,%8,%9,%10,%11,%12,%13,%14,%15,%16};\n" ::"r"(taddr),
      "r"(__float_as_uint(v[0])), "r"(__float_as_uint(v[1])), "r"(__float_as_uint(v[2])), "r"(__float_as_uint(v[3])),
      "r"(__float_as_uint(v[4])), "r"(__float_as_uint(v[5])), "r"(__float_as_uint(v[6])), "r"(__float_as_uint(v[7])),
      "r"(__float_as_uint(v[8])), "r"(__float_as_uint(v[9])), "r"(__float_as_uint(v[10])), "r"(__float_as_uint(v[11])),
      "r"(__float_as_uint(v[12])), "r"(__float_as_uint(v[13])), "r"(__float_as_uint(v[14])), "r"(__float_as_uint(v[15]))
      : "memory");
}
__device__ __forceinline__ void tmem_st_wait() { asm volatile("tcgen05.wait::st.sync.aligned;\n" ::: "memory"); }

__device__ __forceinline__ float4 lds128(uint32_t a) {
  float4 v;
  asm volatile("ld.shared.v4.f32 {%0,%1,%2,%3}, [%4];\n" : "=f"(v.x), "=f"(v.y), "=f"(v.z), "=f"(v.w) : "r"(a) : "memory");
  return v;
}

template <bool FWD>
__global__ void __launch_bounds__(RG_THREADS, FWD ? 2 : 1)
rows_gemm_kernel(const __grid_constant__ CUtensorMap tmBhi, const __grid_constant__ CUtensorMap tmBlo,
                 const __grid_constant__ CUtensorMap tmIn, const __grid_constant__ CUtensorMap tmAux, RowsArgs p) {
  extern __shared__ uint8_t smem_raw[];
  uint8_t* base = reinterpret_cast<uint8_t*>((reinterpret_cast<uintptr_t>(smem_raw) + 1023) & ~(uintptr_t)1023);
  const uint32_t sbase = smem_u32(base);
  const int NS = p.NS, NA = p.NA, NB = p.NB, N = p.N, K = p.K, nc = p.nchunks;
  const int w_bytes = N * 128;
  const int stage_bytes = (!FWD && p.has_mask) ? 2 * A_BYTES : A_BYTES;
  const uint32_t b_ring = sbase, s_ring = b_ring + (uint32_t)(NB * 2 * w_bytes);
  uint64_t* bars = reinterpret_cast<uint64_t*>(base + NB * 2 * w_bytes + NS * stage_bytes);
  uint64_t* a_full = bars;
  uint64_t* a_empty = bars + 4;
  uint64_t* b_full = bars + 8;
  uint64_t* b_empty = bars + 12;
  uint64_t* s_full = bars + 16;
  uint64_t* s_empty = bars + 20;
  uint64_t* out_bar = bars + 24;
  uint32_t* tmem_slot = reinterpret_cast<uint32_t*>(bars + 25);

  const int warp = threadIdx.x >> 5, lane = threadIdx.x & 31;
  const bool split = !FWD && (int)blockIdx.x >= p.full_tiles;
  const int tile = split ? p.full_tiles + ((int)blockIdx.x - p.full_tiles) / K : (int)blockIdx.x;
  const int z0 = split ? ((int)blockIdx.x - p.full_tiles) % K : 0;
  const int items = FWD ? nc * K : nc;
  const int nb = FWD ? 1 : (split ? 1 : K);

  if (threadIdx.x == 0) {
    RG_STAMP(0);
    for (int s = 0; s < 4; ++s) {
      mbar_init(&a_full[s], WORKERS / 32);
      mbar_init(&a_empty[s], 1);
      mbar_init(&b_full[s], 1);
      mbar_init(&b_empty[s], 1);
      mbar_init(&s_full[s], 1);
      mbar_init(&s_empty[s], WORKERS / 32);
    }
    mbar_init(out_bar, 1);
    asm volatile("fence.mbarrier_init.release.cluster;\n" ::: "memory");
  }
  if (warp == 1) {
    const uint32_t s = smem_u32(tmem_slot);
    switch (p.tmem_cols) {
      case 32: asm volatile("tcgen05.alloc.cta_group::1.sync.aligned.shared::cta.b32 [%0], 32;\n" ::"r"(s) : "memory"); break;
      case 64: asm volatile("tcgen05.alloc.cta_group::1.sync.aligned.shared::cta.b32 [%0], 64;\n" ::"r"(s) : "memory"); break;
      case 128: asm volatile("tcgen05.alloc.cta_group::1.sync.aligned.shared::cta.b32 [%0], 128;\n" ::"r"(s) : "memory"); break;
      case 256: asm volatile("tcgen05.alloc.cta_group::1.sync.aligned.shared::cta.b32 [%0], 256;\n" ::"r"(s) : "memory"); break;
      default: asm volatile("tcgen05.alloc.cta_group::1.sync.aligned.shared::cta.b32 [%0], 512;\n" ::"r"(s) : "memory"); break;
    }
    asm volatile("tcgen05.relinquish_alloc_permit.cta_group::1.sync.aligned;\n" ::: "memory");
  }
  tc_fence_before();
  __syncthreads();
  tc_fence_after();
  const uint32_t tmem_base = *tmem_slot;
  if (threadIdx.x == 0) RG_STAMP(1);

  if (warp == 0) {
    if (lane == 0) {
      int bi = 0, cc = 0, sl = 0;
      for (int i = 0; i < items; ++i) {
        for (int j = 0; j < nb; ++j, ++bi) {
          const int slot = bi % NB, u = bi / NB;
          if (u > 0) mbar_wait(&b_empty[slot], (uint32_t)((u - 1) & 1));
          const uint32_t dst = b_ring + (uint32_t)(slot * 2 * w_bytes);
          const int z = FWD ? sl : z0 + j;
          mbar_expect_tx(&b_full[slot], 2 * w_bytes);
          tma_load_2d(dst, &tmBhi, &b_full[slot], cc * CH, z * N);
          tma_load_2d(dst + w_bytes, &tmBlo, &b_full[slot], cc * CH, z * N);
        }
        if (FWD) {
          if (++sl == K) { sl = 0; ++cc; }
        } else {
          ++cc;
        }
      }
    }
  } else if (warp == 2) {
    if (lane == 0) {
      int cc = 0, sl = 0;
      for (int i = 0; i < items; ++i) {
        const int slot = i % NS, u = i / NS;
        if (u > 0) mbar_wait(&s_empty[slot], (uint32_t)((u - 1) & 1));
        const uint32_t dst = s_ring + (uint32_t)(slot * stage_bytes);
        mbar_expect_tx(&s_full[slot], stage_bytes);
        if (FWD) {
          if (sl == 0)
            tma_load_2d(dst, &tmIn, &s_full[slot], cc * CH, tile * TM);
          else
            tma_load_2d(dst, &tmAux, &s_full[slot], cc * CH, (sl - 1) * p.R + tile * TM);
          if (++sl == K) { sl = 0; ++cc; }
        } else {
          tma_load_2d(dst, &tmIn, &s_full[slot], cc * CH, tile * TM);
          if (p.has_mask) tma_load_2d(dst + A_BYTES, &tmAux, &s_full[slot], cc * CH, tile * TM);
          ++cc;
        }
      }
    }
  } else if (warp == 1) {
    if (lane == 0) {
      const uint32_t idesc = (1u << 4) | (2u << 7) | (2u << 10) | ((uint32_t)(N >> 3) << 17) | ((uint32_t)(TM >> 4) << 24);
      int bi = 0;
      for (int i = 0; i < items; ++i) {
        const int aslot = i % NA;
        mbar_wait(&a_full[aslot], (uint32_t)((i / NA) & 1));
        if (i < 12) RG_STAMP(40 + 3 * i);
        tc_fence_after();
        const uint32_t ta_hi = tmem_base + (uint32_t)(p.a_col0 + aslot * 2 * CH), ta_lo = ta_hi + CH;
        for (int j = 0; j < nb; ++j, ++bi) {
          const int slot = bi % NB;
          mbar_wait(&b_full[slot], (uint32_t)((bi / NB) & 1));
          if (i < 12 && j == 0) RG_STAMP(41 + 3 * i);
          tc_fence_after();
          const uint32_t sw = b_ring + (uint32_t)(slot * 2 * w_bytes), sw_lo = sw + w_bytes;
          const uint32_t acc = tmem_base + (uint32_t)(FWD ? 0 : (z0 + j) * p.acc_stride);
#pragma unroll
          for (int k = 0; k < CH / UMMA_K; ++k) {
            const uint32_t koff = k * UMMA_K * 4;
            const uint64_t b_hi = make_desc(sw + koff), b_lo = make_desc(sw_lo + koff);
            umma_ts(acc, ta_lo + k * UMMA_K, b_hi, idesc, (i | k) != 0);
            umma_ts(acc, ta_hi + k * UMMA_K, b_lo, idesc, 1);
            umma_ts(acc, ta_hi + k * UMMA_K, b_hi, idesc, 1);
          }
          umma_commit(&b_empty[slot]);
        }
        umma_commit(&a_empty[aslot]);
        if (i < 12) RG_STAMP(42 + 3 * i);
      }
      umma_commit(out_bar);
    }
  } else {
    const int wi = warp - 3, q = warp & 3, h = wi >> 2, r = q * 32 + lane;
    const long long grow = (long long)tile * TM + r;
    const bool valid = grow < p.R;
    uint32_t soff[4];
#pragma unroll
    for (int g = 0; g < 4; ++g) soff[g] = (uint32_t)(r * 128 + (((4 * h + g) ^ (r & 7)) << 4));
    const bool masked = !FWD && p.has_mask;
    for (int i = 0; i < items; ++i) {
      const int sslot = i % NS, aslot = i % NA;
      if (lane == 0) {
        mbar_wait(&s_full[sslot], (uint32_t)((i / NS) & 1));
        if (wi == 0 && i < 12) RG_STAMP(4 + 3 * i);
        if (i >= NA) mbar_wait(&a_empty[aslot], (uint32_t)((i / NA - 1) & 1));
        if (wi == 0 && i < 12) RG_STAMP(5 + 3 * i);
      }
      __syncwarp();
      const uint32_t st = s_ring + (uint32_t)(sslot * stage_bytes);
      float4 x[4];
#pragma unroll
      for (int g = 0; g < 4; ++g) x[g] = lds128(st + soff[g]);
      if (masked) {
#pragma unroll
        for (int g = 0; g < 4; ++g) {
          const float4 m = lds128(st + A_BYTES + soff[g]);
          x[g].x = m.x > 0.f ? x[g].x : 0.f; x[g].y = m.y > 0.f ? x[g].y : 0.f;
          x[g].z = m.z > 0.f ? x[g].z : 0.f; x[g].w = m.w > 0.f ? x[g].w : 0.f;
        }
      }
      float hi[16], lo[16];
#pragma unroll
      for (int g = 0; g < 4; ++g) {
        hi[4 * g] = tf32_rn(x[g].x); hi[4 * g + 1] = tf32_rn(x[g].y);
        hi[4 * g + 2] = tf32_rn(x[g].z); hi[4 * g + 3] = tf32_rn(x[g].w);
        lo[4 * g] = tf32_rn(x[g].x - hi[4 * g]); lo[4 * g + 1] = tf32_rn(x[g].y - hi[4 * g + 1]);
        lo[4 * g + 2] = tf32_rn(x[g].z - hi[4 * g + 2]); lo[4 * g + 3] = tf32_rn(x[g].w - hi[4 * g + 3]);
      }
      const uint32_t ta = tmem_base + ((uint32_t)(q * 32) << 16) + (uint32_t)(p.a_col0 + aslot * 2 * CH + 16 * h);
      tmem_st16(ta, hi);
      tmem_st16(ta + CH, lo);
      tmem_st_wait();
      tc_fence_before();
      __syncwarp();
      if (lane == 0) {
        mbar_arrive(&s_empty[sslot]);
        mbar_arrive(&a_full[aslot]);
        if (wi == 0 && i < 12) RG_STAMP(6 + 3 * i);
      }
    }
    if (lane == 0) mbar_wait(out_bar, 0);
    if (wi == 0 && lane == 0) RG_STAMP(2);
    __syncwarp();
    tc_fence_after();
    const int Fout = p.Fout;
    const int zbeg = FWD ? 0 : z0, zend = FWD ? 1 : (split ? z0 + 1 : K);
    for (int z = zbeg; z < zend; ++z) {
      float* dstm = p.Out + (long long)z * p.out_slice;
      const bool vecO = ((Fout & 3) == 0) && ((reinterpret_cast<uintptr_t>(dstm) & 15) == 0);
      for (int c0 = 16 * h; c0 < N && c0 < Fout; c0 += 32) {
        float v[16];
        tmem_ld16(tmem_base + ((uint32_t)(q * 32) << 16) + (uint32_t)(z * p.acc_stride + c0), v);
        if (!valid) continue;
        if (FWD) {
#pragma unroll
          for (int u = 0; u < 16; ++u) {
            float o = v[u] + ((p.bias && c0 + u < Fout) ? __ldg(p.bias + c0 + u) : 0.f);
            if (p.act == AGCN_ACT_RELU) o = fmaxf(o, 0.f);
            v[u] = o;
          }
        }
        float* dst = dstm + grow * Fout + c0;
#pragma unroll
        for (int g = 0; g < 4; ++g) {
          if (c0 + 4 * g >= Fout) continue;
          if (vecO && c0 + 4 * g + 3 < Fout) {
            *reinterpret_cast<float4*>(dst + 4 * g) = make_float4(v[4 * g], v[4 * g + 1], v[4 * g + 2], v[4 * g + 3]);
          } else {
#pragma unroll
            for (int e = 0; e < 4; ++e)
              if (c0 + 4 * g + e < Fout) dst[4 * g + e] = v[4 * g + e];
          }
        }
      }
    }
  }
  tc_fence_before();
  __syncthreads();
  if (threadIdx.x == 0) RG_STAMP(3);
  if (warp == 1) {
    switch (p.tmem_cols) {
      case 32: asm volatile("tcgen05.dealloc.cta_group::1.sync.aligned.b32 %0, 32;\n" ::"r"(tmem_base) : "memory"); break;
      case 64: asm volatile("tcgen05.dealloc.cta_group::1.sync.aligned.b32 %0, 64;\n" ::"r"(tmem_base) : "memory"); break;
      case 128: asm volatile("tcgen05.dealloc.cta_group::1.sync.aligned.b32 %0, 128;\n" ::"r"(tmem_base) : "memory"); break;
      case 256: asm volatile("tcgen05.dealloc.cta_group::1.sync.aligned.b32 %0, 256;\n" ::"r"(tmem_base) : "memory"); break;
      default: asm volatile("tcgen05.dealloc.cta_group::1.sync.aligned.b32 %0, 512;\n" ::"r"(tmem_base) : "memory"); break;
    }
  }
}

typedef CUresult (*EncodeTiledFn)(CUtensorMap*, CUtensorMapDataType, cuuint32_t, void*, const cuuint64_t*,
                                  const cuuint64_t*, const cuuint32_t*, const cuuint32_t*, CUtensorMapInterleave,
                                  CUtensorMapSwizzle, CUtensorMapL2promotion, CUtensorMapFloatOOBfill);

static EncodeTiledFn encode_fn() {
  static EncodeTiledFn fn = nullptr;
  static std::once_flag once;
  std::call_once(once, [] {
    void* p = nullptr;
    cudaDriverEntryPointQueryResult q;
    if (cudaGetDriverEntryPoint("cuTensorMapEncodeTiled", &p, cudaEnableDefault, &q) == cudaSuccess &&
        q == cudaDriverEntryPointSuccess)
      fn = reinterpret_cast<EncodeTiledFn>(p);
  });
  return fn;
}

static int make_map(CUtensorMap* map, const float* ptr, uint64_t rows, uint64_t cols, uint32_t box_rows) {
  EncodeTiledFn fn = encode_fn();
  if (!fn) {
    set_error("cuTensorMapEncodeTiled is not available from the driver");
    return AGCN_ERR_CUDA;
  }
  cuuint64_t gdim[2] = {cols, rows};
  cuuint64_t gstride[1] = {cols * sizeof(float)};
  cuuint32_t box[2] = {(cuuint32_t)CH, box_rows};
  cuuint32_t estr[2] = {1, 1};
  CUresult r = fn(map, CU_TENSOR_MAP_DATA_TYPE_FLOAT32, 2, const_cast<float*>(ptr), gdim, gstride, box, estr,
                  CU_TENSOR_MAP_INTERLEAVE_NONE, CU_TENSOR_MAP_SWIZZLE_128B, CU_TENSOR_MAP_L2_PROMOTION_L2_256B,
                  CU_TENSOR_MAP_FLOAT_OOB_FILL_NONE);
  if (r != CUDA_SUCCESS) {
    set_error("cuTensorMapEncodeTiled failed with code " + std::to_string((int)r));
    return AGCN_ERR_CUDA;
  }
  return AGCN_OK;
}


static int pad16(int x) { return (x + 15) & ~15; }
static int pad32(int x) { return (x + 31) & ~31; }

static void* g_rows_dbg = nullptr;
static void* rows_debug_buffer() { return g_rows_dbg; }

static bool rows_fast(const PreArgs& a) {
  auto al = [](const void* q) { return (reinterpret_cast<uintptr_t>(q) & 15) == 0; };
  if (a.Fin % CH != 0 || !al(a.In) || (a.Mask && !al(a.Mask)) || (a.T && (!al(a.T) || (a.t_slice & 3)))) return false;
  const int stride = a.N <= 32 ? 32 : (a.N <= 64 ? 64 : 128);
  return a.N <= 128 && (a.forward ? stride : a.K * stride) + 2 * CH <= 512;
}

static int launch_rows(const agcn_plan* plan, const PreArgs& a, const CUtensorMap& mhi, const CUtensorMap& mlo, const char* name,
                       cudaStream_t st) {
  RowsArgs r{};
  r.R = (int)plan->R; r.Fin = a.Fin; r.Fout = a.Fout; r.K = a.K; r.N = a.N; r.nchunks = a.Fin / CH;
  r.acc_stride = a.N <= 32 ? 32 : (a.N <= 64 ? 64 : 128);
  r.a_col0 = a.forward ? r.acc_stride : a.K * r.acc_stride;
  const int tmem_budget = a.forward ? 256 : 512;
  r.NA = std::max(1, std::min(3, (tmem_budget - r.a_col0) / (2 * CH)));
  int cols = r.a_col0 + r.NA * 2 * CH, tm = 32;
  while (tm < cols) tm <<= 1;
  r.tmem_cols = tm;
  r.has_mask = (!a.forward && a.Mask) ? 1 : 0;
  r.bias = a.bias; r.act = a.act; r.Out = a.Out; r.out_slice = a.out_slice;
  r.dbg = reinterpret_cast<unsigned long long*>(rows_debug_buffer());
  CUtensorMap min, maux;
  int rc;
  if ((rc = make_map(&min, a.In, (uint64_t)plan->R, (uint64_t)a.Fin, (uint32_t)TM))) return rc;
  if (a.forward) {
    const float* aux = (a.K > 1) ? a.T : a.In;
    const uint64_t rows = (a.K > 1) ? (uint64_t)(a.K - 1) * plan->R : (uint64_t)plan->R;
    if ((rc = make_map(&maux, aux, rows, (uint64_t)a.Fin, (uint32_t)TM))) return rc;
  } else {
    if ((rc = make_map(&maux, a.Mask ? a.Mask : a.In, (uint64_t)plan->R, (uint64_t)a.Fin, (uint32_t)TM))) return rc;
  }
  const int w2 = 2 * a.N * 128, budget = (a.forward ? 112 : 227) * 1024 - 1024 - 256;
  const int stage_bytes = r.has_mask ? 2 * A_BYTES : A_BYTES;
  r.NS = a.forward ? 2 : std::min(4, 65536 / stage_bytes);
  r.NB = std::max(1, std::min(4, (budget - r.NS * stage_bytes) / w2));
  const int smem = r.NB * w2 + r.NS * stage_bytes + 256 + 1024;
  int ntiles = (int)((plan->R + TM - 1) / TM);
  r.full_tiles = ntiles;
  if (!a.forward && a.K > 1) {
    int sms = 148;
    int dev = 0;
    if (cudaGetDevice(&dev) == cudaSuccess) cudaDeviceGetAttribute(&sms, cudaDevAttrMultiProcessorCount, dev);
    const int rem = ntiles % sms;
    if (ntiles > sms && rem > 0 && rem * a.K <= sms) {
      r.full_tiles = ntiles - rem;
      ntiles = r.full_tiles + rem * a.K;
    }
  }
  static std::once_flag once;
  std::call_once(once, [] {
    cudaFuncSetAttribute(rows_gemm_kernel<true>, cudaFuncAttributeMaxDynamicSharedMemorySize, 227 * 1024);
    cudaFuncSetAttribute(rows_gemm_kernel<false>, cudaFuncAttributeMaxDynamicSharedMemorySize, 227 * 1024);
  });
  {
    ProfScope prof(name, st);
    if (a.forward)
      rows_gemm_kernel<true><<<ntiles, RG_THREADS, smem, st>>>(mhi, mlo, min, maux, r);
    else
      rows_gemm_kernel<false><<<ntiles, RG_THREADS, smem, st>>>(mhi, mlo, min, maux, r);
  }
  AGCN_LAUNCH_CHECK();
  return AGCN_OK;
}

static int launch(const agcn_plan* plan, int tile0, int ntiles, PreArgs& a, const float* wsplit, int Kp, const char* name,
                  cudaStream_t st) {
  const long long half = (long long)a.K * a.N * Kp;
  CUtensorMap mhi, mlo;
  int rc;
  if ((rc = make_map(&mhi, wsplit, (uint64_t)a.K * a.N, (uint64_t)Kp, (uint32_t)a.N))) return rc;
  if ((rc = make_map(&mlo, wsplit + half, (uint64_t)a.K * a.N, (uint64_t)Kp, (uint32_t)a.N))) return rc;
  if (tile0 < 0 && rows_fast(a)) return launch_rows(plan, a, mhi, mlo, a.forward ? "pt::rows_gemm_kernel(fwd)" : "pt::rows_gemm_kernel(bwd)", st);
  if (tile0 >= 0) {
    a.tile_graphs = reinterpret_cast<const int4*>(plan->d_ft_entries);
    a.tile_gstart = plan->d_ft_gstart;
    a.tile0 = tile0;
  } else {
    a.tile_graphs = nullptr;
    a.tile_gstart = nullptr;
    a.tile0 = 0;
    a.R = (int)plan->R;
    ntiles = (int)((plan->R + TM - 1) / TM);
  }
  a.nchunks = Kp / CH;
  a.acc_stride = a.N <= 32 ? 32 : (a.N <= 64 ? 64 : 128);
  a.tmem_cols = a.forward ? a.acc_stride : 2 * a.acc_stride;
  const SmemPlan sp = smem_plan(a.N);
  static std::once_flag once;
  std::call_once(once, [] {
    cudaFuncSetAttribute(pre_tile_kernel, cudaFuncAttributeMaxDynamicSharedMemorySize, 227 * 1024);
  });
  {
    ProfScope prof(name, st);
    pre_tile_kernel<<<ntiles, THREADS, sp.total, st>>>(mhi, mlo, a);
  }
  AGCN_LAUNCH_CHECK();
  return AGCN_OK;
}

}

void rows_debug_set(void* d_buf) { pt::g_rows_dbg = d_buf; }

int pre_forward(const agcn_plan* plan, int tile0, int ntiles, const float* X, const float* T, const float* wsplit,
                const float* bias, int act, int F, int Fo, int K, float* Y, cudaStream_t st) {
  if (ntiles <= 0 && tile0 >= 0) return AGCN_OK;
  pt::PreArgs a{};
  a.Fin = F; a.Fout = Fo; a.K = K; a.N = pt::pad16(Fo);
  a.In = X; a.Mask = nullptr; a.T = T; a.t_slice = (long long)plan->R * F;
  a.bias = bias; a.act = act; a.Out = Y; a.out_slice = 0; a.forward = 1;
  return pt::launch(plan, tile0, ntiles, a, wsplit, pt::pad32(F), "pt::pre_tile_kernel(fwd)", st);
}

int pre_backward(const agcn_plan* plan, int tile0, int ntiles, const float* dY, const float* Y, const float* wsplit, int F,
                 int Fo, int K, float* G, cudaStream_t st) {
  if (ntiles <= 0 && tile0 >= 0) return AGCN_OK;
  pt::PreArgs a{};
  a.Fin = Fo; a.Fout = F; a.K = K; a.N = pt::pad16(F);
  a.In = dY; a.Mask = Y; a.T = nullptr; a.t_slice = 0;
  a.bias = nullptr; a.act = AGCN_ACT_LINEAR; a.Out = G; a.out_slice = (long long)plan->R * F; a.forward = 0;
  return pt::launch(plan, tile0, ntiles, a, wsplit, pt::pad32(Fo), "pt::pre_tile_kernel(bwd)", st);
}

}
```

include/agcn_sgcll.h:

```cpp
#ifndef AGCN_SGCLL_H_
#define AGCN_SGCLL_H_

#include <stdint.h>
#include <stddef.h>

#ifdef __cplusplus
extern "C" {
#endif

#define AGCN_OK 0
#define AGCN_ERR_INVALID (-1)
#define AGCN_ERR_CUDA (-2)
#define AGCN_ERR_WORKSPACE (-3)
#define AGCN_ERR_NO_DEVICE (-4)

#define AGCN_VARIANT_SGC_LL 0
#define AGCN_VARIANT_SGC_LL_RESLAP 1
#define AGCN_LAP_REFERENCE_LITERAL 0
#define AGCN_LAP_PAPER 1
#define AGCN_METRIC_GRAD_REFERENCE 0
#define AGCN_METRIC_GRAD_FULL 1
#define AGCN_ACT_LINEAR 0
#define AGCN_ACT_RELU 1

#define AGCN_OUT_RES_L 1u
#define AGCN_OUT_RES_W 2u
#define AGCN_OUT_L_ALL 4u
#define AGCN_SAVE_FOR_BACKWARD 8u

typedef struct agcn_plan agcn_plan;

typedef struct agcn_sgcll_desc {
  int32_t F;
  int32_t Fo;
  int32_t K;
  int32_t variant;
  int32_t laplacian_mode;
  int32_t metric_grad;
  int32_t activation;
  uint32_t flags;
} agcn_sgcll_desc;

int agcn_version(void);
const char* agcn_last_error(void);
uint64_t agcn_launch_count(void);

int agcn_plan_create(const int32_t* n_nodes_host, int32_t B, int32_t Nmax, void* stream, agcn_plan** out);
int agcn_plan_destroy(agcn_plan* plan);
int64_t agcn_plan_total_nodes(const agcn_plan* plan);
int64_t agcn_plan_total_lap(const agcn_plan* plan);
const int32_t* agcn_plan_node_off_host(const agcn_plan* plan);
const int64_t* agcn_plan_lap_off_host(const agcn_plan* plan);

int agcn_fused_tiles_host(const int32_t* n_nodes_host, int32_t B, int32_t* gstart_out, int32_t gstart_cap,
                          int32_t* entries_out, int32_t entries_cap, int32_t* tiles_out, int32_t* n_entries_out);

int agcn_fused_profile(int enable);
int agcn_fused_profile_read(float* ms_sum, int* launches);

int agcn_profile_enable(int enable);
int agcn_profile_read(char* buf, size_t cap, size_t* needed);
int agcn_profile_timeline(char* buf, size_t cap, size_t* needed);
int agcn_probe_fp32_fma(float* d_sink, int32_t iters, void* stream);

int agcn_fused_debug_set(void* d_buf);

int agcn_debug_grouped_product(const agcn_plan* plan, const float* d_L , const float* d_In ,
                               float* d_Out , int32_t F, int32_t transL, int32_t add_identity, float cmul,
                               int32_t impl, void* stream);

int agcn_debug_grouped_timeline(void* d_buf);

int agcn_pack_nodes(const agcn_plan* plan, const float* d_padded , float* d_packed ,
                    int32_t F, void* stream);
int agcn_unpack_nodes(const agcn_plan* plan, const float* d_packed, float* d_padded, int32_t F, void* stream);
int agcn_pack_lap(const agcn_plan* plan, const float* d_padded , float* d_packed, void* stream);
int agcn_unpack_lap(const agcn_plan* plan, const float* d_packed, float* d_padded, void* stream);
int agcn_pack_lap_csr(const agcn_plan* plan, const int32_t* d_indptr, const int32_t* d_indices, const float* d_values,
                      float* d_packed, void* stream);

#define AGCN_ADJ_MEAN_DISTANCE 0
#define AGCN_ADJ_CUTOFF 1
int agcn_point_laplacian_workspace_bytes(const agcn_plan* plan, size_t* bytes);
int agcn_point_laplacian(const agcn_plan* plan, const float* d_points, int32_t F, int32_t rule, float sparse_ratio,
                         float* d_L, void* d_work, size_t work_bytes, void* stream);

int agcn_graph_pool(const agcn_plan* plan, const float* d_X , const float* d_L , float* d_Y,
                    int32_t* d_argmax, int32_t F, void* stream);
int agcn_graph_pool_backward(const agcn_plan* plan, const float* d_dY, const int32_t* d_argmax, float* d_dX, int32_t F,
                             void* stream);

int agcn_sgcll_workspace_bytes(const agcn_sgcll_desc* desc, const agcn_plan* plan, size_t* saved_bytes,
                               size_t* work_bytes);

int agcn_sgcll_forward(const agcn_sgcll_desc* desc, const agcn_plan* plan, const float* d_X, const float* d_Lint,
                       const float* d_Lprev, const float* d_M_L, const float* d_weight, const float* d_bias,
                       const float* d_alpha, const float* d_beta, float* d_Y, float* d_resL, float* d_resW,
                       float* d_Lall, void* d_saved, void* d_work, size_t work_bytes, void* stream);

int agcn_sgcll_backward(const agcn_sgcll_desc* desc, const agcn_plan* plan, const float* d_X, const float* d_Lint,
                        const float* d_Lprev, const float* d_M_L, const float* d_weight, const float* d_alpha,
                        const float* d_beta, const float* d_Y, const float* d_dY, const float* d_dLall_in,
                        const void* d_saved, float* d_dX, float* d_dM_L, float* d_dweight, float* d_dbias,
                        float* d_dalpha, float* d_dbeta, float* d_dLprev, void* d_work, size_t work_bytes,
                        void* stream);

size_t agcn_gemm_tn_scratch_bytes(int32_t M, int32_t Kd, int32_t N, int32_t S);
int agcn_gemm_tn(const float* d_A0, const float* d_A1, const float* d_D, float* d_out, int32_t M, int32_t Kd,
                 int32_t N, int32_t S, void* d_scratch, int32_t use_tensor_cores, void* stream);

size_t agcn_node_gemm_scratch_bytes(int32_t N, int32_t Kd);
int agcn_node_gemm(const float* d_A, int32_t lda, const float* d_B, int32_t ldb, int32_t transB, float* d_C, int32_t ldc,
                   int32_t M, int32_t N, int32_t Kd, const float* d_bias, const float* d_scale, int32_t accumulate,
                   int32_t activation, void* d_scratch, void* stream);

int agcn_dropout(const float* d_X, float* d_Y, int64_t n, float p, uint64_t seed, void* stream);

int agcn_expand_labels(const uint8_t* y, const float* w, int32_t B, int32_t n_tasks, float* d_targets, float* d_weights,
                       void* stream);

#define AGCN_LOSS_SIGMOID_CE 0
#define AGCN_LOSS_SOFTMAX_CE 1
#define AGCN_LOSS_WEIGHTED_L2 2
int agcn_head_workspace_bytes(const agcn_plan* plan, int32_t Fh, int32_t Fm, int32_t Nt, size_t* bytes);
int agcn_head_loss_grad(const agcn_plan* plan, const float* d_H, const float* d_dense_W, const float* d_dense_b,
                        const float* d_head_W, const float* d_head_b, const float* d_targets, const float* d_weights,
                        float scale, int32_t Fh, int32_t Fm, int32_t Nt, float* d_loss, float* d_dH,
                        float* d_ddense_W, float* d_ddense_b, float* d_dhead_W, float* d_dhead_b, void* d_work,
                        size_t work_bytes, void* stream);

int agcn_head_loss_grad_ex(const agcn_plan* plan, const float* d_H, const float* d_dense_W, const float* d_dense_b,
                           const float* d_head_W, const float* d_head_b, const float* d_targets, const float* d_weights,
                           float scale, int32_t loss_kind, int32_t Fh, int32_t Fm, int32_t Nt, float* d_loss,
                           float* d_dH, float* d_ddense_W, float* d_ddense_b, float* d_dhead_W, float* d_dhead_b,
                           void* d_work, size_t work_bytes, void* stream);

int agcn_head_predict_workspace_bytes(const agcn_plan* plan, int32_t Fh, int32_t Fm, int32_t Nt, size_t* bytes);
int agcn_head_predict(const agcn_plan* plan, const float* d_H, const float* d_dense_W, const float* d_dense_b,
                      const float* d_head_W, const float* d_head_b, const float* d_targets, const float* d_weights,
                      float scale, int32_t loss_kind, int32_t Fh, int32_t Fm, int32_t Nt, float* d_probs, float* d_loss,
                      void* d_work, size_t work_bytes, void* stream);

typedef struct agcn_stack agcn_stack;
typedef void (*agcn_stack_notify_fn)(void* user, int32_t stage, void* stream);
int agcn_stack_create(const agcn_sgcll_desc* layer_descs, int32_t n_layers, int32_t Fm, int32_t Nt, int32_t loss_kind,
                      const int64_t* param_offsets, agcn_stack** out);
int agcn_stack_destroy(agcn_stack* stack);
int agcn_stack_workspace_bytes(const agcn_stack* stack, const agcn_plan* plan, size_t* bytes);
int agcn_stack_loss_grad(const agcn_stack* stack, const agcn_plan* plan, const float* d_X, const float* d_Lint,
                         const float* d_targets, const float* d_weights, float scale, const float* d_params,
                         float* d_grads, float* d_loss, void* d_work, size_t work_bytes, agcn_stack_notify_fn notify,
                         void* notify_user, void* stream);
int agcn_stack_predict_workspace_bytes(const agcn_stack* stack, const agcn_plan* plan, size_t* bytes);
int agcn_stack_predict(const agcn_stack* stack, const agcn_plan* plan, const float* d_X, const float* d_Lint,
                       const float* d_targets, const float* d_weights, float scale, const float* d_params,
                       float* d_probs, float* d_loss, void* d_work, size_t work_bytes, void* stream);

#define AGCN_NODE_SGCLL 0
#define AGCN_NODE_BLOCK_END 1
typedef struct agcn_stack_node {
  int32_t kind;
  agcn_sgcll_desc desc;
  int32_t src;
} agcn_stack_node;
int agcn_stack_create_nodes(const agcn_stack_node* nodes, int32_t n_nodes, int32_t Fm, int32_t Nt, int32_t loss_kind,
                            const int64_t* param_offsets, agcn_stack** out);

int agcn_adam_step(float* d_params, const float* d_grads, float* d_m, float* d_v, int32_t* d_step, int64_t n, float lr,
                   float beta1, float beta2, float eps, void* stream);

typedef struct agcn_step_graph agcn_step_graph;
int agcn_capture_begin(void* stream);
int agcn_capture_end_launch(void* stream, agcn_step_graph** graph ,
                            int32_t* how);
int agcn_capture_abort(void* stream);
int agcn_step_graph_destroy(agcn_step_graph* graph);

int agcn_sgcll_host_scratch_bytes(const agcn_sgcll_desc* desc, const agcn_plan* plan, size_t* bytes);
int agcn_sgcll_forward_host(const agcn_sgcll_desc* desc, const agcn_plan* plan, const float* h_X_padded,
                            const float* h_L_padded, const float* d_M_L, const float* d_weight, const float* d_bias,
                            const float* d_alpha, float* h_Y_padded, void* d_scratch, size_t scratch_bytes,
                            void* stream);

#ifdef __cplusplus
}
#endif
#endif
```

Baseline: 1.647 million.

## Fuse Chebyshev recursion and weight contraction into a single row-tile kernel

```diff
diff --git a/adaptive-graph-convolutional-network_b200/_lib.py b/adaptive-graph-convolutional-network_b200/_lib.py
--- a/adaptive-graph-convolutional-network_b200/_lib.py
+++ b/adaptive-graph-convolutional-network_b200/_lib.py
@@ -43,6 +43,7 @@
     "agcn_plan_lap_off_host": (_P, [_P]),
     "agcn_fused_tiles_host": (ctypes.c_int, [_P, ctypes.c_int32, _P, ctypes.c_int32, _P, ctypes.c_int32, _P, _P]),
     "agcn_fused_debug_set": (ctypes.c_int, [_P]),
+    "agcn_fused_layer": (ctypes.c_int, [ctypes.c_int]),
     "agcn_fused_profile": (ctypes.c_int, [ctypes.c_int]),
     "agcn_fused_profile_read": (ctypes.c_int, [ctypes.POINTER(ctypes.c_float), ctypes.POINTER(ctypes.c_int)]),
     "agcn_profile_enable": (ctypes.c_int, [ctypes.c_int]),
diff --git a/adaptive-graph-convolutional-network_b200/csrc/agcn_capi.cu b/adaptive-graph-convolutional-network_b200/csrc/agcn_capi.cu
--- a/adaptive-graph-convolutional-network_b200/csrc/agcn_capi.cu
+++ b/adaptive-graph-convolutional-network_b200/csrc/agcn_capi.cu
@@ -391,6 +391,24 @@
   if (fuse_f) {
     const float* Lf = m.shortcut ? d_Lint : sv.Lall;
     const int ident = m.shortcut ? 1 : 0;
+    const bool mid = cheb_tiles_has_mid(plan);
+    float* Tsave = ((desc->flags & AGCN_SAVE_FOR_BACKWARD) || mid) ? sv.T : nullptr;
+    if (cheb_rows_supported(plan, F, Fo, K, d_X, Tsave)) {
+      if (mid) {
+        AGCN_CUDA(cudaEventRecord(plan->ev_big_fork, st));
+        AGCN_CUDA(cudaStreamWaitEvent(plan->big, plan->ev_big_fork, 0));
+        if ((rc = cheb_mid_forward(plan, d_X, Lf, ident, F, K, sv.T, plan->big, 0))) return rc;
+        AGCN_CUDA(cudaEventRecord(plan->ev_big_join, plan->big));
+      }
+      AGCN_CUDA(cudaStreamWaitEvent(st, plan->ev_side_join, 0));
+      if ((rc = cheb_rows_forward(plan, d_X, Lf, ident, 0, Tsave, wk.ftY, d_bias, desc->activation, F, Fo, K, d_Y, st)))
+        return rc;
+      if (mid) {
+        AGCN_CUDA(cudaStreamWaitEvent(st, plan->ev_big_join, 0));
+        if ((rc = rows_forward_wide(plan, d_X, sv.T, wk.ftY, d_bias, desc->activation, F, Fo, K, d_Y, st))) return rc;
+      }
+      return AGCN_OK;
+    }
     const bool other = cheb_tiles_has_mid(plan) || plan->large_tiles > 0;
     if (other) {
       AGCN_CUDA(cudaEventRecord(plan->ev_big_fork, st));
@@ -478,7 +496,25 @@
     if ((rc = node_gemm_tn(t, plan->side))) return rc;
   }
   AGCN_CUDA(cudaEventRecord(plan->ev_side_join, plan->side));
-  if (vfirst) {
+  const bool mid_b = cheb_tiles_has_mid(plan);
+  if (vfirst && cheb_rows_supported(plan, Fo, F, K, dYp, mid_b ? wk.V : nullptr)) {
+    const float* Lf = m.shortcut ? d_Lint : sv.Lall;
+    const int ident = m.shortcut ? 1 : 0;
+    if (mid_b) {
+      AGCN_CUDA(cudaEventRecord(plan->ev_big_fork, st));
+      AGCN_CUDA(cudaStreamWaitEvent(plan->big, plan->ev_big_fork, 0));
+      if ((rc = cheb_mid_forward(plan, dYp, Lf, ident, Fo, K, wk.V, plan->big, 1))) return rc;
+      AGCN_CUDA(cudaEventRecord(plan->ev_big_join, plan->big));
+    }
+    if ((rc = cheb_rows_forward(plan, dYp, Lf, ident, 1, mid_b ? wk.V : nullptr, sv.ftG, nullptr, AGCN_ACT_LINEAR,
+                                Fo, F, K, d_dX, st)))
+      return rc;
+    if (mid_b) {
+      AGCN_CUDA(cudaStreamWaitEvent(st, plan->ev_big_join, 0));
+      if ((rc = rows_forward_wide(plan, dYp, wk.V, sv.ftG, nullptr, AGCN_ACT_LINEAR, Fo, F, K, d_dX, st)))
+        return rc;
+    }
+  } else if (vfirst) {
     const float* Lf = m.shortcut ? d_Lint : sv.Lall;
     const int ident = m.shortcut ? 1 : 0;
     const bool other = cheb_tiles_has_mid(plan);
@@ -595,6 +631,11 @@
   return AGCN_OK;
 }
 int agcn_fused_profile_read(float* ms_sum, int* launches) { return fused_profile_read(ms_sum, launches); }
+
+int agcn_fused_layer(int enable) {
+  cheb_rows_enable(enable);
+  return AGCN_OK;
+}
 
 int agcn_fused_debug_set(void* d_buf) {
   fused_debug_set(d_buf);
diff --git a/adaptive-graph-convolutional-network_b200/csrc/agcn_cheb_rows.cuh b/adaptive-graph-convolutional-network_b200/csrc/agcn_cheb_rows.cuh
--- /dev/null
+++ b/adaptive-graph-convolutional-network_b200/csrc/agcn_cheb_rows.cuh
@@ -0,0 +1,179 @@
+#pragma once
+#include "agcn_internal.cuh"
+
+namespace agcn {
+namespace ct {
+
+constexpr int CH = 32;
+constexpr int CPITCH = 144;
+
+__device__ __forceinline__ uint32_t smem_u32(const void* p) { return (uint32_t)__cvta_generic_to_shared(p); }
+__device__ __forceinline__ float4 lds128(uint32_t a) {
+  float4 v;
+  asm volatile("ld.shared.v4.f32 {%0,%1,%2,%3}, [%4];\n" : "=f"(v.x), "=f"(v.y), "=f"(v.z), "=f"(v.w) : "r"(a) : "memory");
+  return v;
+}
+__device__ __forceinline__ float lds32(uint32_t a) {
+  float v;
+  asm volatile("ld.shared.f32 %0, [%1];\n" : "=f"(v) : "r"(a) : "memory");
+  return v;
+}
+__device__ __forceinline__ void sts128(uint32_t a, float4 v) {
+  asm volatile("st.shared.v4.f32 [%0], {%1,%2,%3,%4};\n" ::"r"(a), "f"(v.x), "f"(v.y), "f"(v.z), "f"(v.w) : "memory");
+}
+__device__ __forceinline__ void sts32(uint32_t a, float v) {
+  asm volatile("st.shared.f32 [%0], %1;\n" ::"r"(a), "f"(v) : "memory");
+}
+__device__ __forceinline__ void cp_async4(uint32_t sdst, const float* gsrc) {
+  asm volatile("cp.async.ca.shared.global [%0], [%1], 4;\n" ::"r"(sdst), "l"(gsrc) : "memory");
+}
+__device__ __forceinline__ void cp_async16(uint32_t sdst, const float* gsrc) {
+  asm volatile("cp.async.cg.shared.global [%0], [%1], 16;\n" ::"r"(sdst), "l"(gsrc) : "memory");
+}
+__device__ __forceinline__ void cp_async_commit() { asm volatile("cp.async.commit_group;\n" ::: "memory"); }
+__device__ __forceinline__ void cp_async_wait_all() { asm volatile("cp.async.wait_group 0;\n" ::: "memory"); }
+
+__device__ __forceinline__ void copy_matrix(const float* __restrict__ src, uint32_t dst, int n, int pitch, int w0, int nw) {
+  const int warp = (threadIdx.x >> 5) - w0, lane = threadIdx.x & 31;
+  for (int i = warp; i < n; i += nw) {
+    const float* srow = src + (long long)i * n;
+    const uint32_t drow = dst + 4 * (i * pitch);
+    for (int j = lane; j < n; j += 32) cp_async4(drow + 4 * j, srow + j);
+  }
+}
+
+template <int MW>
+struct Mask {
+  uint32_t w[MW];
+};
+
+template <int MW>
+__device__ __forceinline__ Mask<MW> nonzero_mask(uint32_t laddr, int lstride_bytes, int n) {
+  Mask<MW> m;
+#pragma unroll
+  for (int k = 0; k < MW; ++k) {
+    uint32_t bits = 0;
+    const int j0 = 32 * k;
+    if (j0 < n) {
+      const int cnt = min(32, n - j0);
+      uint32_t a = laddr + (uint32_t)(j0 * lstride_bytes);
+      int j = 0;
+      for (; j + 8 <= cnt; j += 8) {
+        uint32_t b8 = 0;
+#pragma unroll
+        for (int u = 0; u < 8; ++u) b8 |= (lds32(a + (uint32_t)(u * lstride_bytes)) != 0.f) ? (1u << u) : 0u;
+        bits |= b8 << j;
+        a += 8 * lstride_bytes;
+      }
+      for (; j < cnt; ++j) {
+        bits |= (lds32(a) != 0.f) ? (1u << j) : 0u;
+        a += lstride_bytes;
+      }
+    }
+    m.w[k] = bits;
+  }
+  return m;
+}
+template <int MW>
+__device__ __forceinline__ bool prefer_masked(const Mask<MW>& m, int n) {
+  int nnz = 0;
+#pragma unroll
+  for (int k = 0; k < MW; ++k) nnz += __popc(m.w[k]);
+  const unsigned dense_cost = __reduce_max_sync(0xffffffffu, (unsigned)(n * 3));
+  const unsigned masked_cost = __reduce_max_sync(0xffffffffu, (unsigned)(nnz * 4));
+  return masked_cost < dense_cost;
+}
+
+__device__ __forceinline__ void fma_row(float a, const float4 b[4], float acc[16]) {
+#pragma unroll
+  for (int g = 0; g < 4; ++g) {
+    acc[4 * g] = fmaf(a, b[g].x, acc[4 * g]);
+    acc[4 * g + 1] = fmaf(a, b[g].y, acc[4 * g + 1]);
+    acc[4 * g + 2] = fmaf(a, b[g].z, acc[4 * g + 2]);
+    acc[4 * g + 3] = fmaf(a, b[g].w, acc[4 * g + 3]);
+  }
+}
+__device__ __forceinline__ void lap_times_rows(uint32_t laddr, int lstride_bytes, uint32_t src, int r0, int n, int h,
+                                               float acc[16]) {
+  uint32_t ta = src + (uint32_t)(r0 * CPITCH + h * 64);
+  uint32_t la = laddr;
+  int j = 0;
+  for (; j < n; ++j) {
+    const float a = lds32(la);
+    float4 b[4];
+#pragma unroll
+    for (int g = 0; g < 4; ++g) b[g] = lds128(ta + 16 * g);
+    fma_row(a, b, acc);
+    la += lstride_bytes;
+    ta += CPITCH;
+  }
+}
+template <int MW>
+__device__ __forceinline__ void lap_times_rows_masked(uint32_t laddr, int lstride_bytes, uint32_t src, int r0,
+                                                      const Mask<MW>& m, int h, float acc[16]) {
+#pragma unroll
+  for (int k = 0; k < MW; ++k) {
+    uint32_t bits = m.w[k];
+    const uint32_t tbase = src + (uint32_t)((r0 + 32 * k) * CPITCH + h * 64);
+    const uint32_t lbase = laddr + (uint32_t)(32 * k * lstride_bytes);
+    while (bits) {
+      const int j = __ffs((int)bits) - 1;
+      bits &= bits - 1;
+      const float a = lds32(lbase + (uint32_t)(j * lstride_bytes));
+      float4 b[4];
+#pragma unroll
+      for (int g = 0; g < 4; ++g) b[g] = lds128(tbase + (uint32_t)(j * CPITCH + 16 * g));
+      fma_row(a, b, acc);
+    }
+  }
+}
+
+__device__ __forceinline__ uint32_t seg_addr(uint32_t buf, int row, int h) { return buf + (uint32_t)(row * CPITCH + h * 64); }
+__device__ __forceinline__ void read_seg(uint32_t buf, int row, int h, float v[16]) {
+#pragma unroll
+  for (int g = 0; g < 4; ++g) {
+    const float4 x = lds128(seg_addr(buf, row, h) + 16 * g);
+    v[4 * g] = x.x; v[4 * g + 1] = x.y; v[4 * g + 2] = x.z; v[4 * g + 3] = x.w;
+  }
+}
+__device__ __forceinline__ void write_seg(uint32_t buf, int row, int h, const float v[16]) {
+#pragma unroll
+  for (int g = 0; g < 4; ++g)
+    sts128(seg_addr(buf, row, h) + 16 * g, make_float4(v[4 * g], v[4 * g + 1], v[4 * g + 2], v[4 * g + 3]));
+}
+__device__ __forceinline__ void load_seg(const float* __restrict__ M, int F, int grow, int col0, bool vec, float v[16]) {
+  if (grow < 0) {
+#pragma unroll
+    for (int u = 0; u < 16; ++u) v[u] = 0.f;
+    return;
+  }
+  const float* src = M + (long long)grow * F + col0;
+  if (vec) {
+#pragma unroll
+    for (int g = 0; g < 4; ++g) {
+      float4 x = make_float4(0.f, 0.f, 0.f, 0.f);
+      if (col0 + 4 * g < F) x = __ldg(reinterpret_cast<const float4*>(src) + g);
+      v[4 * g] = x.x; v[4 * g + 1] = x.y; v[4 * g + 2] = x.z; v[4 * g + 3] = x.w;
+    }
+  } else {
+#pragma unroll
+    for (int u = 0; u < 16; ++u) v[u] = (col0 + u < F) ? __ldg(src + u) : 0.f;
+  }
+}
+__device__ __forceinline__ void store_seg(float* __restrict__ M, int F, int grow, int col0, bool vec, const float v[16]) {
+  if (grow < 0) return;
+  float* dst = M + (long long)grow * F + col0;
+  if (vec) {
+#pragma unroll
+    for (int g = 0; g < 4; ++g)
+      if (col0 + 4 * g < F)
+        reinterpret_cast<float4*>(dst)[g] = make_float4(v[4 * g], v[4 * g + 1], v[4 * g + 2], v[4 * g + 3]);
+  } else {
+#pragma unroll
+    for (int u = 0; u < 16; ++u)
+      if (col0 + u < F) dst[u] = v[u];
+  }
+}
+
+}
+}
diff --git a/adaptive-graph-convolutional-network_b200/csrc/agcn_cheb_tile.cu b/adaptive-graph-convolutional-network_b200/csrc/agcn_cheb_tile.cu
--- a/adaptive-graph-convolutional-network_b200/csrc/agcn_cheb_tile.cu
+++ b/adaptive-graph-convolutional-network_b200/csrc/agcn_cheb_tile.cu
@@ -1,39 +1,11 @@
 #include <algorithm>
 #include <mutex>
 
-#include "agcn_internal.cuh"
+#include "agcn_cheb_rows.cuh"
 
 namespace agcn {
 namespace ct {
 
-constexpr int CH = 32;
-constexpr int CPITCH = 144;
-
-__device__ __forceinline__ uint32_t smem_u32(const void* p) { return (uint32_t)__cvta_generic_to_shared(p); }
-__device__ __forceinline__ float4 lds128(uint32_t a) {
-  float4 v;
-  asm volatile("ld.shared.v4.f32 {%0,%1,%2,%3}, [%4];\n" : "=f"(v.x), "=f"(v.y), "=f"(v.z), "=f"(v.w) : "r"(a) : "memory");
-  return v;
-}
-__device__ __forceinline__ float lds32(uint32_t a) {
-  float v;
-  asm volatile("ld.shared.f32 %0, [%1];\n" : "=f"(v) : "r"(a) : "memory");
-  return v;
-}
-__device__ __forceinline__ void sts128(uint32_t a, float4 v) {
-  asm volatile("st.shared.v4.f32 [%0], {%1,%2,%3,%4};\n" ::"r"(a), "f"(v.x), "f"(v.y), "f"(v.z), "f"(v.w) : "memory");
-}
-__device__ __forceinline__ void sts32(uint32_t a, float v) {
-  asm volatile("st.shared.f32 [%0], %1;\n" ::"r"(a), "f"(v) : "memory");
-}
-__device__ __forceinline__ void cp_async4(uint32_t sdst, const float* gsrc) {
-  asm volatile("cp.async.ca.shared.global [%0], [%1], 4;\n" ::"r"(sdst), "l"(gsrc) : "memory");
-}
-__device__ __forceinline__ void cp_async16(uint32_t sdst, const float* gsrc) {
-  asm volatile("cp.async.cg.shared.global [%0], [%1], 16;\n" ::"r"(sdst), "l"(gsrc) : "memory");
-}
-__device__ __forceinline__ void cp_async_commit() { asm volatile("cp.async.commit_group;\n" ::: "memory"); }
-__device__ __forceinline__ void cp_async_wait_all() { asm volatile("cp.async.wait_group 0;\n" ::: "memory"); }
 
 struct CtArgs {
   const int4* tile_graphs;
@@ -79,14 +51,6 @@
   int pitch;
 };
 
-__device__ __forceinline__ void copy_matrix(const float* __restrict__ src, uint32_t dst, int n, int pitch) {
-  const int warp = threadIdx.x >> 5, lane = threadIdx.x & 31, nw = blockDim.x >> 5;
-  for (int i = warp; i < n; i += nw) {
-    const float* srow = src + (long long)i * n;
-    const uint32_t drow = dst + 4 * (i * pitch);
-    for (int j = lane; j < n; j += 32) cp_async4(drow + 4 * j, srow + j);
-  }
-}
 
 template <bool TILE>
 __device__ __forceinline__ Row prologue(const CtArgs& p, int tile, int r, uint32_t s_glist, uint32_t sL) {
@@ -121,7 +85,7 @@
         t.n = gz; t.r0 = gy; t.lbase = gw; t.i = r - gy; t.pitch = gz | 1;
       }
       const long long loff = (long long)(((unsigned long long)(unsigned)hi << 32) | (unsigned)lo);
-      copy_matrix(p.L + loff, sL + 4 * gw, gz, gz | 1);
+      copy_matrix(p.L + loff, sL + 4 * gw, gz, gz | 1, 0, nthreads >> 5);
     }
   } else {
     const int g = p.order[p.order_start + tile];
@@ -130,144 +94,12 @@
       t.grow = p.node_off[g] + r;
       t.n = n; t.i = r; t.pitch = pitch;
     }
-    copy_matrix(p.L + p.lap_off[g], sL, n, pitch);
+    copy_matrix(p.L + p.lap_off[g], sL, n, pitch, 0, nthreads >> 5);
   }
   cp_async_commit();
   return t;
 }
 
-template <int MW>
-struct Mask {
-  uint32_t w[MW];
-};
-
-template <int MW>
-__device__ __forceinline__ Mask<MW> nonzero_mask(uint32_t laddr, int lstride_bytes, int n) {
-  Mask<MW> m;
-#pragma unroll
-  for (int k = 0; k < MW; ++k) {
-    uint32_t bits = 0;
-    const int j0 = 32 * k;
-    if (j0 < n) {
-      const int cnt = min(32, n - j0);
-      uint32_t a = laddr + (uint32_t)(j0 * lstride_bytes);
-      int j = 0;
-      for (; j + 8 <= cnt; j += 8) {
-        uint32_t b8 = 0;
-#pragma unroll
-        for (int u = 0; u < 8; ++u) b8 |= (lds32(a + (uint32_t)(u * lstride_bytes)) != 0.f) ? (1u << u) : 0u;
-        bits |= b8 << j;
-        a += 8 * lstride_bytes;
-      }
-      for (; j < cnt; ++j) {
-        bits |= (lds32(a) != 0.f) ? (1u << j) : 0u;
-        a += lstride_bytes;
-      }
-    }
-    m.w[k] = bits;
-  }
-  return m;
-}
-template <int MW>
-__device__ __forceinline__ bool prefer_masked(const Mask<MW>& m, int n) {
-  int nnz = 0;
-#pragma unroll
-  for (int k = 0; k < MW; ++k) nnz += __popc(m.w[k]);
-  const unsigned dense_cost = __reduce_max_sync(0xffffffffu, (unsigned)(n * 3));
-  const unsigned masked_cost = __reduce_max_sync(0xffffffffu, (unsigned)(nnz * 4));
-  return masked_cost < dense_cost;
-}
-
-__device__ __forceinline__ void fma_row(float a, const float4 b[4], float acc[16]) {
-#pragma unroll
-  for (int g = 0; g < 4; ++g) {
-    acc[4 * g] = fmaf(a, b[g].x, acc[4 * g]);
-    acc[4 * g + 1] = fmaf(a, b[g].y, acc[4 * g + 1]);
-    acc[4 * g + 2] = fmaf(a, b[g].z, acc[4 * g + 2]);
-    acc[4 * g + 3] = fmaf(a, b[g].w, acc[4 * g + 3]);
-  }
-}
-__device__ __forceinline__ void lap_times_rows(uint32_t laddr, int lstride_bytes, uint32_t src, int r0, int n, int h,
-                                               float acc[16]) {
-  uint32_t ta = src + (uint32_t)(r0 * CPITCH + h * 64);
-  uint32_t la = laddr;
-  int j = 0;
-  for (; j < n; ++j) {
-    const float a = lds32(la);
-    float4 b[4];
-#pragma unroll
-    for (int g = 0; g < 4; ++g) b[g] = lds128(ta + 16 * g);
-    fma_row(a, b, acc);
-    la += lstride_bytes;
-    ta += CPITCH;
-  }
-}
-template <int MW>
-__device__ __forceinline__ void lap_times_rows_masked(uint32_t laddr, int lstride_bytes, uint32_t src, int r0,
-                                                      const Mask<MW>& m, int h, float acc[16]) {
-#pragma unroll
-  for (int k = 0; k < MW; ++k) {
-    uint32_t bits = m.w[k];
-    const uint32_t tbase = src + (uint32_t)((r0 + 32 * k) * CPITCH + h * 64);
-    const uint32_t lbase = laddr + (uint32_t)(32 * k * lstride_bytes);
-    while (bits) {
-      const int j = __ffs((int)bits) - 1;
-      bits &= bits - 1;
-      const float a = lds32(lbase + (uint32_t)(j * lstride_bytes));
-      float4 b[4];
-#pragma unroll
-      for (int g = 0; g < 4; ++g) b[g] = lds128(tbase + (uint32_t)(j * CPITCH + 16 * g));
-      fma_row(a, b, acc);
-    }
-  }
-}
-
-__device__ __forceinline__ uint32_t seg_addr(uint32_t buf, int row, int h) { return buf + (uint32_t)(row * CPITCH + h * 64); }
-__device__ __forceinline__ void read_seg(uint32_t buf, int row, int h, float v[16]) {
-#pragma unroll
-  for (int g = 0; g < 4; ++g) {
-    const float4 x = lds128(seg_addr(buf, row, h) + 16 * g);
-    v[4 * g] = x.x; v[4 * g + 1] = x.y; v[4 * g + 2] = x.z; v[4 * g + 3] = x.w;
-  }
-}
-__device__ __forceinline__ void write_seg(uint32_t buf, int row, int h, const float v[16]) {
-#pragma unroll
-  for (int g = 0; g < 4; ++g)
-    sts128(seg_addr(buf, row, h) + 16 * g, make_float4(v[4 * g], v[4 * g + 1], v[4 * g + 2], v[4 * g + 3]));
-}
-__device__ __forceinline__ void load_seg(const float* __restrict__ M, int F, int grow, int col0, bool vec, float v[16]) {
-  if (grow < 0) {
-#pragma unroll
-    for (int u = 0; u < 16; ++u) v[u] = 0.f;
-    return;
-  }
-  const float* src = M + (long long)grow * F + col0;
-  if (vec) {
-#pragma unroll
-    for (int g = 0; g < 4; ++g) {
-      float4 x = make_float4(0.f, 0.f, 0.f, 0.f);
-      if (col0 + 4 * g < F) x = __ldg(reinterpret_cast<const float4*>(src) + g);
-      v[4 * g] = x.x; v[4 * g + 1] = x.y; v[4 * g + 2] = x.z; v[4 * g + 3] = x.w;
-    }
-  } else {
-#pragma unroll
-    for (int u = 0; u < 16; ++u) v[u] = (col0 + u < F) ? __ldg(src + u) : 0.f;
-  }
-}
-__device__ __forceinline__ void store_seg(float* __restrict__ M, int F, int grow, int col0, bool vec, const float v[16]) {
-  if (grow < 0) return;
-  float* dst = M + (long long)grow * F + col0;
-  if (vec) {
-#pragma unroll
-    for (int g = 0; g < 4; ++g)
-      if (col0 + 4 * g < F)
-        reinterpret_cast<float4*>(dst)[g] = make_float4(v[4 * g], v[4 * g + 1], v[4 * g + 2], v[4 * g + 3]);
-  } else {
-#pragma unroll
-    for (int u = 0; u < 16; ++u)
-      if (col0 + u < F) dst[u] = v[u];
-  }
-}
 
 template <bool TILE, int MW>
 __global__ void __launch_bounds__(TILE ? 256 : 320, TILE ? 3 : 1) cheb_tile_fwd_kernel(CtArgs p) {
@@ -438,7 +270,8 @@
   return nullptr;
 }
 
-static int launch(const agcn_plan* plan, CtArgs a, bool forward, cudaStream_t st_small, cudaStream_t st_mid) {
+static int launch(const agcn_plan* plan, CtArgs a, bool forward, cudaStream_t st_small, cudaStream_t st_mid,
+                  bool small_tiles = true) {
   static std::once_flag once;
   static int once_rc = AGCN_OK;
   const size_t smem_tile = smem_bytes(128, AGCN_FUSE_LCAP, true);
@@ -470,7 +303,7 @@
     }
     AGCN_LAUNCH_CHECK();
   }
-  if (plan->ft_small_tiles > 0) {
+  if (small_tiles && plan->ft_small_tiles > 0) {
     CtArgs t = a;
     t.tile_graphs = reinterpret_cast<const int4*>(plan->d_ft_entries);
     t.tile_gstart = plan->d_ft_gstart;
@@ -488,7 +321,7 @@
     else
       cheb_tile_bwd_kernel<true, 2><<<grid, 256, smem_tile, st_small>>>(t);
   }
-  if (plan->ft_small_tiles > 0) AGCN_LAUNCH_CHECK();
+  if (small_tiles && plan->ft_small_tiles > 0) AGCN_LAUNCH_CHECK();
   return AGCN_OK;
 }
 
@@ -507,6 +340,15 @@
   return ct::launch(plan, a, true, st_small, st_mid);
 }
 
+int cheb_mid_forward(const agcn_plan* plan, const float* X, const float* L, int add_identity, int F, int K, float* T,
+                     cudaStream_t st_mid, int transL) {
+  if (K < 2) return AGCN_OK;
+  ct::CtArgs a = ct::base_args(plan, L, add_identity, F, K);
+  a.transL = transL;
+  a.X = X; a.T = T; a.tslice = (long long)plan->R * F;
+  return ct::launch(plan, a, true, st_mid, st_mid, false);
+}
+
 int cheb_tiles_backward(const agcn_plan* plan, const float* G, const float* L, int add_identity, int F, int K, float* dX,
                         cudaStream_t st_small, cudaStream_t st_mid) {
   if (K < 2) return AGCN_OK;
diff --git a/adaptive-graph-convolutional-network_b200/csrc/agcn_internal.cuh b/adaptive-graph-convolutional-network_b200/csrc/agcn_internal.cuh
--- a/adaptive-graph-convolutional-network_b200/csrc/agcn_internal.cuh
+++ b/adaptive-graph-convolutional-network_b200/csrc/agcn_internal.cuh
@@ -109,6 +109,8 @@
   int32_t* d_big_tile_start = nullptr;
   int ft_tiles = 0;
   int ft_small_tiles = 0;
+  int ft_lfloats = 0;
+  std::vector<int32_t> wide_row_tiles;
   std::vector<int32_t> ft_gstart, ft_entries;
   int32_t* d_ft_gstart = nullptr;
   int32_t* d_ft_entries = nullptr;
@@ -282,9 +284,18 @@
 int pre_backward(const agcn_plan* plan, int tile0, int ntiles, const float* dY, const float* Y, const float* wsplit, int F,
                  int Fo, int K, float* G, cudaStream_t st);
 
+void cheb_rows_enable(int on);
+int rows_forward_wide(const agcn_plan* plan, const float* X, const float* T, const float* wsplit, const float* bias, int act,
+                      int F, int Fo, int K, float* Y, cudaStream_t st);
+bool cheb_rows_supported(const agcn_plan* plan, int Fin, int Fout, int K, const float* X, const float* T);
+int cheb_rows_forward(const agcn_plan* plan, const float* X, const float* L, int add_identity, int transL, float* T,
+                      const float* wsplit, const float* bias, int act, int Fin, int Fout, int K, float* Out, cudaStream_t st);
+
 bool cheb_tiles_has_mid(const agcn_plan* plan);
 int cheb_tiles_forward(const agcn_plan* plan, const float* X, const float* L, int add_identity, int F, int K, float* T,
                        cudaStream_t st_small, cudaStream_t st_mid, int transL = 0);
+int cheb_mid_forward(const agcn_plan* plan, const float* X, const float* L, int add_identity, int F, int K, float* T,
+                     cudaStream_t st_mid, int transL);
 int cheb_tiles_backward(const agcn_plan* plan, const float* G, const float* L, int add_identity, int F, int K, float* dX,
                         cudaStream_t st_small, cudaStream_t st_mid);
 
diff --git a/adaptive-graph-convolutional-network_b200/csrc/agcn_plan.cu b/adaptive-graph-convolutional-network_b200/csrc/agcn_plan.cu
--- a/adaptive-graph-convolutional-network_b200/csrc/agcn_plan.cu
+++ b/adaptive-graph-convolutional-network_b200/csrc/agcn_plan.cu
@@ -451,6 +451,15 @@
   }
   build_fused_tiles(p->n, p->order, &p->ft_gstart, &p->ft_entries, &p->ft_small_tiles);
   p->ft_tiles = (int)p->ft_gstart.size() - 1;
+  for (int e = 0; e < (p->ft_small_tiles > 0 ? p->ft_gstart[p->ft_small_tiles] : 0); ++e) {
+    const int32_t* en = &p->ft_entries[4 * e];
+    p->ft_lfloats = std::max(p->ft_lfloats, en[3] + en[2] * (en[2] | 1));
+  }
+  for (int g = 0; g < B; ++g)
+    if (p->n[g] > AGCN_FUSE_MAX_N)
+      for (int t = p->node_off[g] / 128; t <= (p->node_off[g] + p->n[g] - 1) / 128; ++t) p->wide_row_tiles.push_back(t);
+  std::sort(p->wide_row_tiles.begin(), p->wide_row_tiles.end());
+  p->wide_row_tiles.erase(std::unique(p->wide_row_tiles.begin(), p->wide_row_tiles.end()), p->wide_row_tiles.end());
   const size_t T = (size_t)p->large_tiles;
   const size_t NB = p->big_tile_start.size();
   const size_t n32 = (size_t)B + (B + 1) + B + 2 * T + NB + p->ft_gstart.size();
diff --git a/adaptive-graph-convolutional-network_b200/csrc/agcn_pre_tile.cu b/adaptive-graph-convolutional-network_b200/csrc/agcn_pre_tile.cu
--- a/adaptive-graph-convolutional-network_b200/csrc/agcn_pre_tile.cu
+++ b/adaptive-graph-convolutional-network_b200/csrc/agcn_pre_tile.cu
@@ -1,9 +1,11 @@
 #include <cuda.h>
 
 #include <algorithm>
+#include <atomic>
+#include <cstdlib>
 #include <mutex>
 
-#include "agcn_internal.cuh"
+#include "agcn_cheb_rows.cuh"
 
 namespace agcn {
 namespace pt {
@@ -355,6 +357,8 @@
 
 constexpr int RG_THREADS = 96 + WORKERS;
 
+constexpr int RG_MAX_TILE_LIST = 64;
+
 struct RowsArgs {
   int R, Fin, Fout, K, N, nchunks;
   int NS, NA, NB;
@@ -367,6 +371,8 @@
   float* Out;
   long long out_slice;
   unsigned long long* dbg;
+  int ntl;
+  int tl[RG_MAX_TILE_LIST];
 };
 
 #define RG_STAMP(slot)                                                                  \
@@ -393,6 +399,11 @@
       "r"(__float_as_uint(v[12])), "r"(__float_as_uint(v[13])), "r"(__float_as_uint(v[14])), "r"(__float_as_uint(v[15]))
       : "memory");
 }
+__device__ __forceinline__ void tmem_st4(uint32_t taddr, const float v[4]) {
+  asm volatile("tcgen05.st.sync.aligned.32x32b.x4.b32 [%0], {%1,%2,%3,%4};\n" ::"r"(taddr), "r"(__float_as_uint(v[0])),
+               "r"(__float_as_uint(v[1])), "r"(__float_as_uint(v[2])), "r"(__float_as_uint(v[3]))
+               : "memory");
+}
 __device__ __forceinline__ void tmem_st_wait() { asm volatile("tcgen05.wait::st.sync.aligned;\n" ::: "memory"); }
 
 __device__ __forceinline__ float4 lds128(uint32_t a) {
@@ -404,7 +415,8 @@
 template <bool FWD>
 __global__ void __launch_bounds__(RG_THREADS, FWD ? 2 : 1)
 rows_gemm_kernel(const __grid_constant__ CUtensorMap tmBhi, const __grid_constant__ CUtensorMap tmBlo,
-                 const __grid_constant__ CUtensorMap tmIn, const __grid_constant__ CUtensorMap tmAux, RowsArgs p) {
+                 const __grid_constant__ CUtensorMap tmIn, const __grid_constant__ CUtensorMap tmAux,
+                 const __grid_constant__ RowsArgs p) {
   extern __shared__ uint8_t smem_raw[];
   uint8_t* base = reinterpret_cast<uint8_t*>((reinterpret_cast<uintptr_t>(smem_raw) + 1023) & ~(uintptr_t)1023);
   const uint32_t sbase = smem_u32(base);
@@ -424,7 +436,8 @@
 
   const int warp = threadIdx.x >> 5, lane = threadIdx.x & 31;
   const bool split = !FWD && (int)blockIdx.x >= p.full_tiles;
-  const int tile = split ? p.full_tiles + ((int)blockIdx.x - p.full_tiles) / K : (int)blockIdx.x;
+  const int tile = split ? p.full_tiles + ((int)blockIdx.x - p.full_tiles) / K
+                         : ((FWD && p.ntl > 0) ? p.tl[blockIdx.x] : (int)blockIdx.x);
   const int z0 = split ? ((int)blockIdx.x - p.full_tiles) % K : 0;
   const int items = FWD ? nc * K : nc;
   const int nb = FWD ? 1 : (split ? 1 : K);
@@ -631,6 +644,284 @@
   }
 }
 
+
+constexpr int CR_STAGE = TM * ct::CPITCH;
+
+struct ChebRowsArgs {
+  const int4* tile_graphs;
+  const int32_t* tile_gstart;
+  const float* L;
+  int add_identity, transL;
+  const float* X;
+  float* T;
+  long long tslice;
+  int F, Fout, K, N, nchunks, lfloats;
+  int NS, NA, NB;
+  int a_col0;
+  const float* bias;
+  int act;
+  float* Out;
+};
+
+__device__ __forceinline__ void bulk_load(uint32_t dst, const float* src, uint32_t bytes, uint64_t* bar) {
+  asm volatile("cp.async.bulk.shared::cluster.global.mbarrier::complete_tx::bytes [%0], [%1], %2, [%3];\n" ::"r"(dst),
+               "l"(src), "r"(bytes), "r"(smem_u32(bar))
+               : "memory");
+}
+
+__global__ void __maxnreg__(88)
+cheb_rows_kernel(const __grid_constant__ CUtensorMap tmBhi, const __grid_constant__ CUtensorMap tmBlo, ChebRowsArgs p) {
+  extern __shared__ uint8_t smem_raw[];
+  uint8_t* base = reinterpret_cast<uint8_t*>((reinterpret_cast<uintptr_t>(smem_raw) + 1023) & ~(uintptr_t)1023);
+  const uint32_t sbase = smem_u32(base);
+  const int NS = p.NS, NA = p.NA, NB = p.NB, N = p.N, K = p.K, nc = p.nchunks, F = p.F;
+  const int w_bytes = N * 128;
+  const uint32_t b_ring = sbase, s_ring = b_ring + (uint32_t)(NB * 2 * w_bytes);
+  const uint32_t sL = s_ring + (uint32_t)(NS * CR_STAGE), s_glist = sL + 4u * (uint32_t)p.lfloats;
+  uint64_t* bars = reinterpret_cast<uint64_t*>(base + (s_glist - sbase) + 128 * 32 + 16);
+  uint64_t* a_full = bars;
+  uint64_t* a_empty = bars + 4;
+  uint64_t* b_full = bars + 8;
+  uint64_t* b_empty = bars + 12;
+  uint64_t* s_full = bars + 16;
+  uint64_t* s_empty = bars + 20;
+  uint64_t* out_bar = bars + 24;
+  uint32_t* tmem_slot = reinterpret_cast<uint32_t*>(bars + 25);
+
+  const int warp = threadIdx.x >> 5, lane = threadIdx.x & 31;
+  const int tile = (int)blockIdx.x;
+  const int items = nc * K;
+
+  if (threadIdx.x == 0) {
+    for (int s = 0; s < 4; ++s) {
+      mbar_init(&a_full[s], WORKERS / 32);
+      mbar_init(&a_empty[s], 1);
+      mbar_init(&b_full[s], 1);
+      mbar_init(&b_empty[s], 1);
+      mbar_init(&s_full[s], 1);
+      mbar_init(&s_empty[s], WORKERS / 32);
+    }
+    mbar_init(out_bar, 1);
+    asm volatile("fence.mbarrier_init.release.cluster;\n" ::: "memory");
+  }
+  if (warp == 1) {
+    const uint32_t s = smem_u32(tmem_slot);
+    asm volatile("tcgen05.alloc.cta_group::1.sync.aligned.shared::cta.b32 [%0], 256;\n" ::"r"(s) : "memory");
+    asm volatile("tcgen05.relinquish_alloc_permit.cta_group::1.sync.aligned;\n" ::: "memory");
+  }
+  if (warp == 2) {
+    int gs = 0, ge = 0;
+    if (lane == 0) {
+      gs = __ldg(p.tile_gstart + tile);
+      ge = __ldg(p.tile_gstart + tile + 1);
+    }
+    gs = __shfl_sync(0xffffffffu, gs, 0);
+    ge = __shfl_sync(0xffffffffu, ge, 0);
+    for (int e = lane; e < 2 * (ge - gs); e += 32) {
+      const int4 v = __ldg(p.tile_graphs + 2 * gs + e);
+      asm volatile("st.shared.v4.s32 [%0], {%1,%2,%3,%4};\n" ::"r"(s_glist + 16 * e), "r"(v.x), "r"(v.y), "r"(v.z), "r"(v.w) : "memory");
+    }
+    if (lane == 0) asm volatile("st.shared.s32 [%0], %1;\n" ::"r"(s_glist + 128 * 32), "r"(ge - gs) : "memory");
+  }
+  tc_fence_before();
+  __syncthreads();
+  tc_fence_after();
+  const uint32_t tmem_base = *tmem_slot;
+  const int ng = ldsi32(s_glist + 128 * 32);
+  auto row_of = [&](int r, int& gy, int& gz, int& gw) {
+    int grow = -1;
+    for (int e = 0; e < ng; ++e) {
+      const int ey = ldsi32(s_glist + 32 * e + 4), ez = ldsi32(s_glist + 32 * e + 8);
+      if (r >= ey && r < ey + ez) {
+        grow = ldsi32(s_glist + 32 * e + 16) + (r - ey);
+        gy = ey; gz = ez; gw = ldsi32(s_glist + 32 * e + 12);
+      }
+    }
+    return grow;
+  };
+
+  if (warp == 0) {
+    if (lane == 0) {
+      int cc = 0, sl = 0;
+      for (int i = 0; i < items; ++i) {
+        const int slot = i % NB, u = i / NB;
+        if (u > 0) mbar_wait(&b_empty[slot], (uint32_t)((u - 1) & 1));
+        const uint32_t dst = b_ring + (uint32_t)(slot * 2 * w_bytes);
+        mbar_expect_tx(&b_full[slot], 2 * w_bytes);
+        tma_load_2d(dst, &tmBhi, &b_full[slot], cc * CH, sl * N);
+        tma_load_2d(dst + w_bytes, &tmBlo, &b_full[slot], cc * CH, sl * N);
+        if (++sl == K) { sl = 0; ++cc; }
+      }
+    }
+  } else if (warp == 2) {
+    int grow[4], d0, d1, d2;
+    int valid = 0;
+#pragma unroll
+    for (int m = 0; m < 4; ++m) {
+      grow[m] = row_of(lane + 32 * m, d0, d1, d2);
+      valid += grow[m] >= 0 ? 1 : 0;
+    }
+    valid = __reduce_add_sync(0xffffffffu, (unsigned)valid);
+    for (int c = 0; c < nc; ++c) {
+      const int slot = c % NS, u = c / NS;
+      if (lane == 0) {
+        if (u > 0) {
+          mbar_wait(&s_empty[slot], (uint32_t)((u - 1) & 1));
+          asm volatile("fence.proxy.async.shared::cta;\n" ::: "memory");
+        }
+        mbar_expect_tx(&s_full[slot], (uint32_t)(valid * CH * 4));
+      }
+      __syncwarp();
+      const uint32_t dst = s_ring + (uint32_t)(slot * CR_STAGE);
+#pragma unroll
+      for (int m = 0; m < 4; ++m)
+        if (grow[m] >= 0)
+          bulk_load(dst + (uint32_t)((lane + 32 * m) * ct::CPITCH), p.X + (long long)grow[m] * F + c * CH, CH * 4, &s_full[slot]);
+    }
+  } else if (warp == 1) {
+    if (lane == 0) {
+      const uint32_t idesc = (1u << 4) | (2u << 7) | (2u << 10) | ((uint32_t)(N >> 3) << 17) | ((uint32_t)(TM >> 4) << 24);
+      for (int i = 0; i < items; ++i) {
+        const int aslot = i % NA, slot = i % NB;
+        mbar_wait(&a_full[aslot], (uint32_t)((i / NA) & 1));
+        tc_fence_after();
+        const uint32_t ta_hi = tmem_base + (uint32_t)(p.a_col0 + aslot * 2 * CH), ta_lo = ta_hi + CH;
+        mbar_wait(&b_full[slot], (uint32_t)((i / NB) & 1));
+        tc_fence_after();
+        const uint32_t sw = b_ring + (uint32_t)(slot * 2 * w_bytes), sw_lo = sw + w_bytes;
+#pragma unroll
+        for (int k = 0; k < CH / UMMA_K; ++k) {
+          const uint32_t koff = k * UMMA_K * 4;
+          const uint64_t b_hi = make_desc(sw + koff), b_lo = make_desc(sw_lo + koff);
+          umma_ts(tmem_base, ta_lo + k * UMMA_K, b_hi, idesc, (i | k) != 0);
+          umma_ts(tmem_base, ta_hi + k * UMMA_K, b_lo, idesc, 1);
+          umma_ts(tmem_base, ta_hi + k * UMMA_K, b_hi, idesc, 1);
+        }
+        umma_commit(&b_empty[slot]);
+        umma_commit(&a_empty[aslot]);
+      }
+      umma_commit(out_bar);
+    }
+  } else {
+    const int wi = warp - 3, q = warp & 3, h = wi >> 2, r = q * 32 + lane;
+    int r0 = 0, n = 0, lbase = 0;
+    const int grow = row_of(r, r0, n, lbase);
+    const int i_me = r - r0, pitch = n | 1;
+    for (int e = 0; e < ng; ++e) {
+      const int ez = ldsi32(s_glist + 32 * e + 8), ew = ldsi32(s_glist + 32 * e + 12);
+      const long long loff =
+          (long long)(((unsigned long long)(unsigned)ldsi32(s_glist + 32 * e + 24) << 32) | (unsigned)ldsi32(s_glist + 32 * e + 20));
+      ct::copy_matrix(p.L + loff, sL + 4 * ew, ez, ez | 1, 3, WORKERS / 32);
+    }
+    ct::cp_async_commit();
+    ct::cp_async_wait_all();
+    worker_sync();
+    const uint32_t lrow = p.transL ? sL + 4 * (lbase + i_me) : sL + 4 * (lbase + i_me * pitch);
+    const int lstep = p.transL ? 4 * pitch : 4;
+    const ct::Mask<2> mask = ct::nonzero_mask<2>(lrow, lstep, grow >= 0 ? n : 0);
+    const bool masked = ct::prefer_masked<2>(mask, grow >= 0 ? n : 0);
+    const int nn = grow >= 0 ? n : 0;
+    auto put = [&](int i, const float v[16]) {
+      const int aslot = i % NA;
+      if (lane == 0 && i >= NA) mbar_wait(&a_empty[aslot], (uint32_t)((i / NA - 1) & 1));
+      __syncwarp();
+      const uint32_t ta = tmem_base + ((uint32_t)(q * 32) << 16) + (uint32_t)(p.a_col0 + aslot * 2 * CH + 16 * h);
+#pragma unroll
+      for (int g = 0; g < 4; ++g) {
+        float hi[4], lo[4];
+#pragma unroll
+        for (int e = 0; e < 4; ++e) {
+          hi[e] = tf32_rn(v[4 * g + e]);
+          lo[e] = tf32_rn(v[4 * g + e] - hi[e]);
+        }
+        tmem_st4(ta + 4 * g, hi);
+        tmem_st4(ta + CH + 4 * g, lo);
+      }
+      tmem_st_wait();
+      tc_fence_before();
+      __syncwarp();
+      if (lane == 0) mbar_arrive(&a_full[aslot]);
+    };
+    const bool save = p.T != nullptr;
+#pragma unroll 1
+    for (int c = 0; c < nc; ++c) {
+      const int sslot = c % NS;
+      const uint32_t buf = s_ring + (uint32_t)(sslot * CR_STAGE);
+      if (lane == 0) mbar_wait(&s_full[sslot], (uint32_t)((c / NS) & 1));
+      __syncwarp();
+      const int col0 = c * CH + 16 * h;
+      float tm1[16], tm2[16];
+      if (grow >= 0) {
+        ct::read_seg(buf, r, h, tm1);
+      } else {
+#pragma unroll
+        for (int u = 0; u < 16; ++u) tm1[u] = 0.f;
+      }
+#pragma unroll
+      for (int u = 0; u < 16; ++u) tm2[u] = 0.f;
+      put(c * K, tm1);
+#pragma unroll 1
+      for (int s = 1; s < K; ++s) {
+        if (s >= 2) worker_sync();
+        float t[16];
+#pragma unroll
+        for (int u = 0; u < 16; ++u) t[u] = p.add_identity ? tm1[u] : 0.f;
+        if (masked)
+          ct::lap_times_rows_masked<2>(lrow, lstep, buf, r0, mask, h, t);
+        else
+          ct::lap_times_rows(lrow, lstep, buf, r0, nn, h, t);
+        if (s >= 2) {
+#pragma unroll
+          for (int u = 0; u < 16; ++u) t[u] = 2.f * t[u] - tm2[u];
+        }
+        if (save) ct::store_seg(p.T + (long long)(s - 1) * p.tslice, F, grow, col0, true, t);
+        put(c * K + s, t);
+        if (s + 1 < K) {
+          worker_sync();
+          ct::write_seg(buf, r, h, t);
+        }
+#pragma unroll
+        for (int u = 0; u < 16; ++u) { tm2[u] = tm1[u]; tm1[u] = t[u]; }
+      }
+      __syncwarp();
+      if (lane == 0) mbar_arrive(&s_empty[sslot]);
+    }
+    if (lane == 0) mbar_wait(out_bar, 0);
+    __syncwarp();
+    tc_fence_after();
+    const int Fout = p.Fout;
+    const bool vecO = ((Fout & 3) == 0) && ((reinterpret_cast<uintptr_t>(p.Out) & 15) == 0);
+    for (int c0 = 16 * h; c0 < N && c0 < Fout; c0 += 32) {
+      float v[16];
+      tmem_ld16(tmem_base + ((uint32_t)(q * 32) << 16) + (uint32_t)c0, v);
+      if (grow < 0) continue;
+#pragma unroll
+      for (int u = 0; u < 16; ++u) {
+        float o = v[u] + ((p.bias && c0 + u < Fout) ? __ldg(p.bias + c0 + u) : 0.f);
+        if (p.act == AGCN_ACT_RELU) o = fmaxf(o, 0.f);
+        v[u] = o;
+      }
+      float* dst = p.Out + (long long)grow * Fout + c0;
+#pragma unroll
+      for (int g = 0; g < 4; ++g) {
+        if (c0 + 4 * g >= Fout) continue;
+        if (vecO && c0 + 4 * g + 3 < Fout) {
+          *reinterpret_cast<float4*>(dst + 4 * g) = make_float4(v[4 * g], v[4 * g + 1], v[4 * g + 2], v[4 * g + 3]);
+        } else {
+#pragma unroll
+          for (int e = 0; e < 4; ++e)
+            if (c0 + 4 * g + e < Fout) dst[4 * g + e] = v[4 * g + e];
+        }
+      }
+    }
+  }
+  tc_fence_before();
+  __syncthreads();
+  if (warp == 1) {
+    asm volatile("tcgen05.dealloc.cta_group::1.sync.aligned.b32 %0, 256;\n" ::"r"(tmem_base) : "memory");
+  }
+}
+
 typedef CUresult (*EncodeTiledFn)(CUtensorMap*, CUtensorMapDataType, cuuint32_t, void*, const cuuint64_t*,
                                   const cuuint64_t*, const cuuint32_t*, const cuuint32_t*, CUtensorMapInterleave,
                                   CUtensorMapSwizzle, CUtensorMapL2promotion, CUtensorMapFloatOOBfill);
@@ -683,7 +974,7 @@
 }
 
 static int launch_rows(const agcn_plan* plan, const PreArgs& a, const CUtensorMap& mhi, const CUtensorMap& mlo, const char* name,
-                       cudaStream_t st) {
+                       cudaStream_t st, const std::vector<int32_t>* tiles = nullptr) {
   RowsArgs r{};
   r.R = (int)plan->R; r.Fin = a.Fin; r.Fout = a.Fout; r.K = a.K; r.N = a.N; r.nchunks = a.Fin / CH;
   r.acc_stride = a.N <= 32 ? 32 : (a.N <= 64 ? 64 : 128);
@@ -712,6 +1003,10 @@
   r.NB = std::max(1, std::min(4, (budget - r.NS * stage_bytes) / w2));
   const int smem = r.NB * w2 + r.NS * stage_bytes + 256 + 1024;
   int ntiles = (int)((plan->R + TM - 1) / TM);
+  if (tiles) {
+    r.ntl = ntiles = (int)tiles->size();
+    std::copy(tiles->begin(), tiles->end(), r.tl);
+  }
   r.full_tiles = ntiles;
   if (!a.forward && a.K > 1) {
     int sms = 148;
@@ -738,6 +1033,36 @@
   AGCN_LAUNCH_CHECK();
   return AGCN_OK;
 }
+
+
+static int launch_cheb_rows(const agcn_plan* plan, ChebRowsArgs r, const float* wsplit, const char* name, cudaStream_t st) {
+  CUtensorMap mhi, mlo;
+  int rc;
+  const long long half = (long long)r.K * r.N * r.F;
+  if ((rc = make_map(&mhi, wsplit, (uint64_t)r.K * r.N, (uint64_t)r.F, (uint32_t)r.N))) return rc;
+  if ((rc = make_map(&mlo, wsplit + half, (uint64_t)r.K * r.N, (uint64_t)r.F, (uint32_t)r.N))) return rc;
+  r.tile_graphs = reinterpret_cast<const int4*>(plan->d_ft_entries);
+  r.tile_gstart = plan->d_ft_gstart;
+  r.nchunks = r.F / CH;
+  r.lfloats = (plan->ft_lfloats + 3) & ~3;
+  r.a_col0 = r.N <= 32 ? 32 : (r.N <= 64 ? 64 : 128);
+  r.NA = std::min(3, (256 - r.a_col0) / (2 * CH));
+  r.NS = 2;
+  const int w2 = 2 * r.N * 128;
+  const int fixed = r.NS * CR_STAGE + 4 * r.lfloats + 128 * 32 + 16 + 256 + 1024;
+  r.NB = std::max(1, std::min(4, (112 * 1024 - fixed) / w2));
+  const int smem = r.NB * w2 + fixed;
+  static std::once_flag once;
+  std::call_once(once, [] { cudaFuncSetAttribute(cheb_rows_kernel, cudaFuncAttributeMaxDynamicSharedMemorySize, 227 * 1024); });
+  {
+    ProfScope prof(name, st);
+    cheb_rows_kernel<<<plan->ft_small_tiles, RG_THREADS, smem, st>>>(mhi, mlo, r);
+  }
+  AGCN_LAUNCH_CHECK();
+  return AGCN_OK;
+}
+
+static std::atomic<int> g_cheb_rows_on{-1};
 
 static int launch(const agcn_plan* plan, int tile0, int ntiles, PreArgs& a, const float* wsplit, int Kp, const char* name,
                   cudaStream_t st) {
@@ -778,6 +1103,33 @@
 
 void rows_debug_set(void* d_buf) { pt::g_rows_dbg = d_buf; }
 
+void cheb_rows_enable(int on) { pt::g_cheb_rows_on.store(on ? 1 : 0); }
+
+bool cheb_rows_supported(const agcn_plan* plan, int Fin, int Fout, int K, const float* X, const float* T) {
+  int on = pt::g_cheb_rows_on.load();
+  if (on < 0) {
+    const char* e = ab_env("AGCN_FUSED_LAYER");
+    on = (e && atoi(e) == 0) ? 0 : 1;
+    int expect = -1;
+    pt::g_cheb_rows_on.compare_exchange_strong(expect, on);
+    on = pt::g_cheb_rows_on.load();
+  }
+  auto al = [](const void* q) { return (reinterpret_cast<uintptr_t>(q) & 15) == 0; };
+  return on && plan->large_tiles == 0 && plan->ft_small_tiles > 0 && K >= 2 && Fin % pt::CH == 0 && Fout >= 1 &&
+         Fout <= 128 && al(X) && (!T || al(T)) && plan->wide_row_tiles.size() <= (size_t)pt::RG_MAX_TILE_LIST;
+}
+
+int cheb_rows_forward(const agcn_plan* plan, const float* X, const float* L, int add_identity, int transL, float* T,
+                      const float* wsplit, const float* bias, int act, int Fin, int Fout, int K, float* Out, cudaStream_t st) {
+  if (plan->ft_small_tiles <= 0) return AGCN_OK;
+  pt::ChebRowsArgs r{};
+  r.L = L; r.add_identity = add_identity; r.transL = transL;
+  r.X = X; r.T = T; r.tslice = (long long)plan->R * Fin;
+  r.F = Fin; r.Fout = Fout; r.K = K; r.N = pt::pad16(Fout);
+  r.bias = bias; r.act = act; r.Out = Out;
+  return pt::launch_cheb_rows(plan, r, wsplit, transL ? "pt::cheb_rows_kernel(bwd)" : "pt::cheb_rows_kernel(fwd)", st);
+}
+
 int pre_forward(const agcn_plan* plan, int tile0, int ntiles, const float* X, const float* T, const float* wsplit,
                 const float* bias, int act, int F, int Fo, int K, float* Y, cudaStream_t st) {
   if (ntiles <= 0 && tile0 >= 0) return AGCN_OK;
@@ -788,6 +1140,26 @@
   return pt::launch(plan, tile0, ntiles, a, wsplit, pt::pad32(F), "pt::pre_tile_kernel(fwd)", st);
 }
 
+int rows_forward_wide(const agcn_plan* plan, const float* X, const float* T, const float* wsplit, const float* bias, int act,
+                      int F, int Fo, int K, float* Y, cudaStream_t st) {
+  if (plan->wide_row_tiles.empty()) return AGCN_OK;
+  pt::PreArgs a{};
+  a.Fin = F; a.Fout = Fo; a.K = K; a.N = pt::pad16(Fo);
+  a.In = X; a.Mask = nullptr; a.T = T; a.t_slice = (long long)plan->R * F;
+  a.bias = bias; a.act = act; a.Out = Y; a.out_slice = 0; a.forward = 1;
+  if (plan->wide_row_tiles.size() > (size_t)pt::RG_MAX_TILE_LIST || !pt::rows_fast(a)) {
+    set_error("rows_forward_wide: shape not supported by the row-tile contraction");
+    return AGCN_ERR_INVALID;
+  }
+  const int Kp = pt::pad32(F);
+  const long long half = (long long)K * a.N * Kp;
+  CUtensorMap mhi, mlo;
+  int rc;
+  if ((rc = pt::make_map(&mhi, wsplit, (uint64_t)K * a.N, (uint64_t)Kp, (uint32_t)a.N))) return rc;
+  if ((rc = pt::make_map(&mlo, wsplit + half, (uint64_t)K * a.N, (uint64_t)Kp, (uint32_t)a.N))) return rc;
+  return pt::launch_rows(plan, a, mhi, mlo, "pt::rows_gemm_kernel(fwd, wide rows)", st, &plan->wide_row_tiles);
+}
+
 int pre_backward(const agcn_plan* plan, int tile0, int ntiles, const float* dY, const float* Y, const float* wsplit, int F,
                  int Fo, int K, float* G, cudaStream_t st) {
   if (ntiles <= 0 && tile0 >= 0) return AGCN_OK;
diff --git a/include/agcn_sgcll.h b/include/agcn_sgcll.h
--- a/include/agcn_sgcll.h
+++ b/include/agcn_sgcll.h
@@ -62,6 +62,8 @@
 int agcn_profile_read(char* buf, size_t cap, size_t* needed);
 int agcn_profile_timeline(char* buf, size_t cap, size_t* needed);
 int agcn_probe_fp32_fma(float* d_sink, int32_t iters, void* stream);
+
+int agcn_fused_layer(int enable);
 
 int agcn_fused_debug_set(void* d_buf);
 
```

Result: slower. 1.286 million (median of 6 runs) (-21.9%).
